# thowell/CALIPSO.jl

Hardware: AMD Instinct MI355X
Metric: Newton steps/sec (n~5k KKT) (higher is better)
Workload: dtype f64; 1 GPU; C3 synthetic dense conic QP: nx=2500 ne=1500 nc=1000 (400 R+ + 200 x SOC3), n=5000 condensed, N=8500 unreduced; ONE system per GPU stepped sequentially (replicas at N > 1); 1 LDL^T factorisation, 6 refinement round(s) per step; refinement_rounds=6

## Files before the change

calipso.jl_amd/__init__.py:

```python
import ctypes as C

import numpy as np

from ._lib import CALLBACK_FN, EVAL_FN, CalipsoHipError, lib

__all__ = ["Solver", "Group", "LDLSolver", "SmallBatch", "Comm", "ordering", "symbolic", "Options", "initialize_b", "solve_b", "CalipsoHipError", "FLAGS", "splitmix_uniform",
           "mfma_f64_peak"]

FLAGS = dict(
    objective=1 << 0, objective_gradient_variables=1 << 1, objective_jacobian_variables_variables=1 << 2,
    equality_constraint=1 << 3, equality_jacobian_variables=1 << 4, equality_dual_jacobian_variables=1 << 5,
    equality_dual_jacobian_variables_variables=1 << 6, cone_constraint=1 << 7, cone_jacobian_variables=1 << 8,
    cone_dual_jacobian_variables=1 << 9, cone_dual_jacobian_variables_variables=1 << 10,
    objective_jacobian_variables_parameters=1 << 11, equality_jacobian_parameters=1 << 12,
    equality_dual_jacobian_variables_parameters=1 << 13, cone_jacobian_parameters=1 << 14,
    cone_dual_jacobian_variables_parameters=1 << 15)
CONE_BARRIER, CONE_BARRIER_GRADIENT, CONE_PRODUCT, CONE_JACOBIAN, CONE_TARGET = 1, 2, 4, 8, 16

STATUS_TEXT = {-1: "inertia correction failure", -2: "cone search failure", -3: "evaluation callback failed",
               -4: "bad argument", -5: "HIP error", -6: "cone layout not supported"}


def _pd(a):
    return a.ctypes.data_as(C.POINTER(C.c_double))
# ... 373 lines not shown
    def set_callbacks(self, inner=None, outer=None):
        self._cbi = CALLBACK_FN(lambda u, h: inner(self)) if inner else None
        self._cbo = CALLBACK_FN(lambda u, h: outer(self)) if outer else None
        ci = C.cast(self._cbi, C.c_void_p) if self._cbi else None
        co = C.cast(self._cbo, C.c_void_p) if self._cbo else None
        self._check(self._L.calipso_hip_set_callbacks(self._h, ci, co, None), "set_callbacks")

    def stats(self):
        out = np.zeros(8, dtype=np.int64)
        self._L.calipso_hip_stats(self._h, _pi(out))
        return dict(total_iterations=int(out[0]), outer=int(out[1]), factorizations=int(out[2]), refinement_failures=int(out[3]),
                    max_refinement_rounds=int(out[4]), fallbacks=int(out[5]), last_refinement_rounds=int(out[6]), newton_steps=int(out[7]))

    def qp_attach(self, P, q, A, b, G, h, objective_scale=0.5):
        f = lambda M: np.ascontiguousarray(np.asarray(M, dtype=np.float64).T).reshape(-1)
        v = lambda a: np.ascontiguousarray(np.asarray(a, dtype=np.float64))
        Pc, Ac, Gc = f(P), f(A) if self.ne else np.zeros(1), f(G) if self.nc else np.zeros(1)
        qv, bv, hv = v(q), v(b) if self.ne else np.zeros(1), v(h) if self.nc else np.zeros(1)
        self._check(self._L.calipso_hip_qp_attach(self._h, _pd(Pc), _pd(qv), _pd(Ac), _pd(bv), _pd(Gc), _pd(hv), objective_scale), "qp_attach")

    def qp_evaluate(self, flags, which=0):
        self._check(self._L.calipso_hip_qp_evaluate(self._h, which, int(flags)), "qp_evaluate")

    def newton_step(self, advance=False):
        info = np.zeros(6)
        rc = self._check(self._L.calipso_hip_newton_step(self._h, int(advance), _pd(info)), "newton_step")
        return dict(status=rc, step_size=info[0], step_size_cone_slack_dual=info[1], refinement_rounds=int(info[2]),
                    factorizations=int(info[3]), merit_candidate=info[4], violation_candidate=info[5])

    def newton_steps(self, count, advance=False):
        info = np.zeros(6 * max(int(count), 1))
        status = np.zeros(max(int(count), 1), dtype=np.int32)
        self._check(self._L.calipso_hip_newton_steps(self._h, int(count), int(advance), _pd(info), status.ctypes.data_as(C.POINTER(C.c_int32))), "newton_steps")
        I = info.reshape(-1, 6)
        return [dict(status=int(status[k]), step_size=I[k, 0], step_size_cone_slack_dual=I[k, 1], refinement_rounds=int(I[k, 2]), factorizations=int(I[k, 3]),
                     merit_candidate=I[k, 4], violation_candidate=I[k, 5]) for k in range(int(count))]

    def phase_times(self):
        out = np.zeros(9)
        self._L.calipso_hip_phase_times(self._h, _pd(out))
        return out

    def kernel_times(self):
        out = np.zeros(8)
        self._L.calipso_hip_kernel_times(self._h, _pd(out))
        return out

    def structure_work(self):
        out = np.zeros(8)
        self._check(self._L.calipso_hip_structure_work(self._h, _pd(out)), "structure_work")
        return dict(schur_flops=out[0], packed_doubles=out[1], segment_pairs=int(out[2]), factor_flops=out[3], factor_nnz=out[4], order=int(out[5]), structured=bool(out[6]))

    def schedule_info(self):
        out = np.zeros(4)
        self._check(self._L.calipso_hip_schedule_info(self._h, _pd(out)), "schedule_info")
        return dict(prologue_ahead_steps=int(out[0]), last_prologue_mode=int(out[1]), ahead_undone=int(out[2]))

    def padded_nx(self):
        return int(self.kernel_times()[2])

    def device_bytes(self):
        return int(self.kernel_times()[3])

    def analyze_structure(self):
        out = np.zeros(4, dtype=np.int64)
        self._check(self._L.calipso_hip_analyze_structure(self._h, _pi(out)), "analyze_structure")
        return dict(half_bandwidth=int(out[0]), band_blocks=int(out[1]), equality_rows_per_group=int(out[2]), cone_rows_per_group=int(out[3]))

    def clear_structure(self):
        self._check(self._L.calipso_hip_clear_structure(self._h), "clear_structure")

    def set_stage_parallel(self, on=True, batch=1):
        out = np.zeros(4, dtype=np.int64)
        self._check(self._L.calipso_hip_set_stage_parallel(self._h, 1 if on else 0, int(batch), _pi(out)), "set_stage_parallel")
        return dict(levels=int(out[0]), largest_front=int(out[1]), nnz_upper=int(out[2]))

    def set_stage_blocks(self, on=True):
        out = np.zeros(4, dtype=np.int64)
        self._check(self._L.calipso_hip_set_stage_blocks(self._h, 1 if on else 0, _pi(out)), "set_stage_blocks")
        return dict(z_blocks=int(out[0]), hessian_blocks=int(out[1]), segments=int(out[2]), packed_doubles=int(out[3]))

    def synchronize(self):
        self._check(self._L.calipso_hip_synchronize(self._h), "synchronize")

    def streams_concurrent(self, other):
        out = np.zeros(6)
        self._check(self._L.calipso_hip_streams_concurrent(self._h, other._h, _pd(out)), "streams_concurrent")
        return bool(out[0]), float(out[1]), float(out[2]), float(out[3]), float(out[4]), float(out[5])

    def rebind_stream(self, priority_class=-1):
        self._check(self._L.calipso_hip_rebind_stream(self._h, int(priority_class)), "rebind_stream")


class Group:

    def __init__(self, solvers):
        import ctypes as C
        self.solvers = list(solvers)
        self._L = self.solvers[0]._L
        arr = (C.c_void_p * len(self.solvers))(*[s._h for s in self.solvers])
        h = C.c_void_p()
        rc = self._L.calipso_hip_group_create(arr, len(self.solvers), C.byref(h))
        if rc != 0:
            raise CalipsoHipError("group_create failed (%d): %s" % (rc, self._L.calipso_hip_last_error(self.solvers[0]._h).decode()))
        self._g = h

    def newton_step(self, advance=False):
        import ctypes as C
        B = len(self.solvers)
# ... 782 lines not shown
```

calipso.jl_amd/csrc/api.hip:

```cpp
#include <algorithm>
#include <array>
#include <atomic>
#include <cmath>
#include <mutex>
#include <cstdio>
#include <cstdlib>
#include <cstring>

#include "internal.hpp"
#include "device_utils.hpp"
#include "host_logic.hpp"

using namespace calipso;

namespace calipso {
int check(H* s, hipError_t e, const char* what) {
    char buf[512];
    snprintf(buf, sizeof buf, "%s: %s", what, hipGetErrorString(e));
    if (s) s->err = buf;
    return CALIPSO_ERR_HIP;
}
bool lds_attribute(const void* kernel, int bytes) {
    static std::mutex mu;
    static std::map<std::pair<const void*, int>, std::pair<int, int>> done;
// ... 560 lines not shown

}

__global__ __launch_bounds__(128) void k_publish_words(const unsigned* __restrict__ src, int words, unsigned* __restrict__ hdst, unsigned long long* __restrict__ hseq,
                                                        unsigned long long seq) {
    if ((int)threadIdx.x < words) hdst[threadIdx.x] = src[threadIdx.x];
    __threadfence_system();
    __syncthreads();
    if (threadIdx.x == 0) __hip_atomic_store(hseq, seq, __ATOMIC_RELEASE, __HIP_MEMORY_SCOPE_SYSTEM);
}
static int wait_published(H* s, unsigned long long seq);
static int publish_and_wait(H* s, const void* dsrc, void* hdst_dev, int words) {
    const unsigned long long seq = ++s->pub_seq;
    hipLaunchKernelGGL(k_publish_words, dim3(1), dim3(128), 0, s->stream, static_cast<const unsigned*>(dsrc), words, static_cast<unsigned*>(hdst_dev), s->hseq_dev, seq);
    return wait_published(s, seq);
}
static int wait_published(H* s, unsigned long long seq) {
    if (launch_errors(s, "a kernel launch of this phase was refused")) return CALIPSO_ERR_HIP;
    hipError_t q = hipSuccess;
    const bool ok = host_wait([&] { return __atomic_load_n(s->hseq, __ATOMIC_ACQUIRE) >= seq; },
                              [&] { q = hipStreamQuery(s->stream); return q == hipErrorNotReady; });
    if (ok) return 0;
    if (q != hipSuccess && q != hipErrorNotReady) return calipso::check(s, q, "publish_and_wait");
    s->err = "scalar read-back did not arrive";
    return CALIPSO_ERR_HIP;
}
static int wait_published_side(H* s, unsigned long long seq) {
    hipError_t q = hipSuccess;
    const bool ok = host_wait([&] { return __atomic_load_n(s->hseq + 1, __ATOMIC_ACQUIRE) >= seq; },
                              [&] { q = hipStreamQuery(s->stream2); return q == hipErrorNotReady; });
    if (ok) return 0;
    if (q != hipSuccess && q != hipErrorNotReady) return calipso::check(s, q, "wait_published_side");
    s->err = "scalar read-back of the second stream did not arrive";
    return CALIPSO_ERR_HIP;
}
static int read_scalars(H* s, int first, int count) { return publish_and_wait(s, s->dscal + first, s->hscal_dev + first, 2 * count); }
static int read_icount(H* s, int first, int count) { return publish_and_wait(s, s->icount + first, s->hicount_dev + first, count); }
static double* point_of(H* s, int which) { return which == 0 ? s->solution : s->candidate; }

static void factor_times(H* s) {
    if (!s->factor_times_pending) return;
    s->factor_times_pending = false;
    if (hipEventSynchronize(s->ev[13]) != hipSuccess) return;
    float ms = 0.f;
    (void)hipEventElapsedTime(&ms, s->ev[10], s->ev[11]); s->phase_ms[1] = ms;
    (void)hipEventElapsedTime(&ms, s->ev[11], s->ev[12]); s->phase_ms[7] = ms;
    (void)hipEventElapsedTime(&ms, s->ev[12], s->ev[13]); s->phase_ms[3] = ms;
    s->kernel_ms[0] = hipEventElapsedTime(&ms, s->ev[12], s->ev[14]) == hipSuccess ? ms : 0.0;
}

static int do_factorize(H* s, int64_t inertia[3], bool rhs_ahead_ok = false) {
    factor_times(s);
    (void)hipEventRecord(s->ev[10], s->stream);
    launch_cone_weights(s);
    s->rhs_ahead = false; s->rhs_joined = false;
    if (rhs_ahead_ok) {
        hipStream_t st2 = calipso::ldl_rhs_stream(s);
        if (st2 && s->side_work) s->rhs_ahead = true;
        else if (st2) {
            (void)hipEventRecord(s->ev_side[6], s->stream);
            (void)hipStreamWaitEvent(st2, s->ev_side[6], 0);
            hipStream_t keep = s->stream;
            s->stream = st2;
            launch_residual_symmetric(s, s->residual);
            if (s->d.m) calipso::gemv_t(s, s->d.m, s->d.nx, s->Z, s->d.m, s->t1, s->xbuf, 1.0, 1.0, calipso::SP_Z);
            s->stream = keep;
            s->rhs_ahead = true;
        }
    }
    launch_scale_rows(s);
    calipso::inject_refused_launch(s->stream);
    (void)hipEventRecord(s->ev[11], s->stream);
    launch_schur(s);
    (void)hipEventRecord(s->ev[12], s->stream);
    s->side_ran = false;
    launch_ldl(s);
    if (s->side_work && s->rhs_ahead && !s->side_ran) s->side_work(s);
    (void)hipEventRecord(s->ev[13], s->stream);
    s->factor_times_pending = true;
    if (s->ldl_failed) { s->ldl_failed = false; SYNC(); return CALIPSO_ERR_HIP; }
    if (s->ldl_pub_seq) {
        if (wait_published(s, s->ldl_pub_seq)) return CALIPSO_ERR_HIP;
    } else {
        if (launch_errors(s, "a kernel launch of the factorisation was refused")) return CALIPSO_ERR_HIP;
        CK(hipMemcpyAsync(s->hicount, s->icount, sizeof(int) * 6, hipMemcpyDeviceToHost, s->stream));
        SYNC();
        factor_times(s);
    }
    s->stats.factorizations += 1;
    s->phase_ms[8] += 1.0;
    const int64_t pos = s->hicount[0] + s->hicount[3], nonpos = s->hicount[1] + s->hicount[4], zero = s->hicount[2] + s->hicount[5];
    inertia[0] = pos; inertia[1] = nonpos; inertia[2] = zero;
    if (zero > 0) { inertia[0] = -1; return CALIPSO_WARN_ZERO_PIVOT; }
    return CALIPSO_OK;
}

static int do_inertia_correction(H* s, int64_t* nfact, bool rhs_ahead_ok = false, const int64_t* first_in = nullptr, int first_rc = 0) {
    const Options& o = s->opt; const Dims& d = s->d;
    int64_t in[3];
    ic_begin(o, s->sc);
    int rc;
    if (first_in) { in[0] = first_in[0]; in[1] = first_in[1]; in[2] = first_in[2]; rc = first_rc; }
    else rc = do_factorize(s, in, rhs_ahead_ok);
    for (int64_t count = 1;; ++count) {
        if (rc < 0) return rc;
        const IcVerdict v = ic_after(o, s->sc, in, d.nx, d.ne + d.nc, count == 1);
        if (v != IC_AGAIN) {
            if (nfact) *nfact = count;
            if (v == IC_DONE) return CALIPSO_OK;
            s->err = "inertia correction failure";
            return CALIPSO_ERR_INERTIA;
        }
        rc = do_factorize(s, in, rhs_ahead_ok);
    }
}

static void do_sds(H* s, int which, double* accumulate = nullptr, bool refine_follows = false, bool use_ahead = false) {
    const double* res = which == 0 ? s->residual : s->residual_error;
    double* st = which == 0 ? s->step : s->step_correction;
    if (which == 0 && s->rhs_ahead && !s->rhs_joined && s->stream2 && s->ev_side[7]) {
        (void)hipEventRecord(s->ev_side[7], s->stream2);
        (void)hipStreamWaitEvent(s->stream, s->ev_side[7], 0);
        s->rhs_joined = true;
    }
    const bool ready = use_ahead && which == 0 && s->rhs_ahead && s->rhs_joined;
    s->rhs_ahead = false;
    if (!ready) launch_residual_symmetric(s, res);
    const bool tail = which == 0 && !accumulate && s->d.m > 0;
    linear_solve_device(s, !tail, ready);
    if (tail && launch_solve_tail(s, 0, false, refine_follows)) return;
    if (tail) gemv_n(s, s->d.m, s->d.nx, s->Z, s->d.m, s->xbuf, s->t2, 1.0, 0.0, SP_Z);
    launch_recover(s, st, res, accumulate, which == 0 ? 1 : 0);
}

static void refine_residual(H* s, bool publish = false) {
    const Dims& d = s->d;
    launch_refine_local(s);
    const int nchunk = gemv_refine_pair(s, s->step + d.oy(), s->t1, s->w1, s->w2, s->step, s->lxv, true);
    if (nchunk > 0) launch_refine_x_fused(s, publish, nchunk); else launch_refine_x(s, publish);
}
static void refine_solve(H* s) {
    const Dims& d = s->d;
    launch_trsv(s, s->xbuf);
    if (d.m && launch_solve_tail(s, 1, true, true)) return;
    if (d.m) gemv_n(s, d.m, d.nx, s->Z, d.m, s->xbuf, s->t2, 1.0, 0.0, SP_Z);
    launch_recover(s, s->step_correction, s->residual_error, s->step, 2);
}

static bool spec_refinement_ok(H* s) {
    static const bool env = [] { const char* e = getenv("CALIPSO_HIP_SPEC_REFINE"); return !e || atoi(e) != 0; }();
    return env && !s->cur && s->gate && s->d.m > 0 && !s->compact && !s->blocks.on && !(s->stage_parallel && s->spS) && wform_on(s) && solve_tail_available(s) &&
           s->opt.max_iterative_refinement >= 1;
}
static int refinement_loop(H* s, double norm, double norm0, int it, int* rounds, double* final_norm, bool* ran_more);
static int do_refinement(H* s, int* rounds, double* final_norm, bool zsx_valid = false) {
    const Options& o = s->opt; const Dims& d = s->d;
    if (!zsx_valid && d.m) gemv_n(s, d.m, d.nx, s->Z, d.m, s->step, s->zsx, 1.0, 0.0, SP_Z);
    double norm, norm0;
    int it = 0;
    if (spec_refinement_ok(s)) {
        const int spec = (int)std::min<calipso::i64>(o.max_iterative_refinement, std::max<calipso::i64>(1, s->stats.last_refine > 0 ? s->stats.last_refine : o.min_iterative_refinement));
        if (++s->gate_counter == 0) s->gate_counter = 1;
        s->gate_epoch = s->gate_counter;
        for (int k = 0; k <= spec; ++k) {
            if (k > 0) {
                launch_trsv_direct(s, s->xbuf);
                (void)launch_solve_tail(s, 1, true, true);
            }
            launch_refine_local(s);
            const int nchunk = gemv_refine_pair(s, s->step + d.oy(), s->t1, s->w1, s->w2, s->step, s->lxv, true);
            launch_refine_x_fused(s, true, nchunk, k, k == spec);
        }
        s->gate_epoch = 0;
        if (s->refine_defer) { s->refine_pending = true; if (rounds) *rounds = -1; return CALIPSO_OK; }
        if (wait_published(s, s->pub_seq)) return CALIPSO_ERR_HIP;
        norm = s->hscal[7]; norm0 = s->hscal[20]; it = (int)s->hscal[21];
    } else {
        refine_residual(s, true);
        if (wait_published(s, s->pub_seq)) return CALIPSO_ERR_HIP;
        norm = s->hscal[7];
        norm0 = norm;
    }
// ... 648 lines not shown
    EV(8);
    int rc = inner_iteration(s, nullptr, nullptr, ev, cv, info, &ev, &cv, !last);
    EV(9);
    if (rc < 0) return rc;
    if (!advance) {
        copy_step_state(s, false);
        launch_cone(s, s->solution, CALIPSO_CONE_PRODUCT);
        s->filter_theta = ft; s->filter_merit = fm; s->filter_index = fi;
        restore_scalars_keeping_regularization(s->sc, saved_sc);
    }
    if (info_out) {
        info_out[0] = info.step_size; info_out[1] = info.step_size_t; info_out[2] = info.rounds; info_out[3] = (double)info.nfact;
        info_out[4] = info.Mh; info_out[5] = info.thetah;
    }
    if (!last) return rc;
    SYNC();
    float ms = 0.f;
    if (info.exit_kind == 0) {
        (void)hipEventElapsedTime(&ms, s->ev[0], s->ev[1]); s->phase_ms[0] = ms;
        (void)hipEventElapsedTime(&ms, s->ev[2], s->ev[3]); s->phase_ms[2] = ms;
        (void)hipEventElapsedTime(&ms, s->ev[3], s->ev[4]); s->phase_ms[5] = ms;
    }
    (void)hipEventElapsedTime(&ms, s->ev[8], s->ev[9]); s->phase_ms[6] = ms;
    return rc;
}

}

extern "C" {

int32_t calipso_hip_phase_times(H* s, double out[9]) {
    if (!s || !out) return CALIPSO_ERR_ARGUMENT;
    factor_times(s);
    for (int i = 0; i < 9; ++i) out[i] = s->phase_ms[i];
    return CALIPSO_OK;
}

int32_t calipso_hip_kernel_times(H* s, double out[8]) {
    if (!s || !out) return CALIPSO_ERR_ARGUMENT;
    for (int i = 0; i < 8; ++i) out[i] = 0.0;
    factor_times(s);
    out[0] = s->kernel_ms[0];
    out[1] = (double)s->ldl_step_launches;
    out[2] = (double)s->d.NP;
    out[3] = (double)(s->slab_doubles * sizeof(double) + s->scratch_bytes);
    { double lf[8]; calipso::lfac_describe(s, lf); out[6] = s->lfac_last ? 1.0 : (s->lfac_failed ? -1.0 : 0.0); out[7] = lf[5]; }
    if (s->matvec_timed && hipEventSynchronize(s->ev[6]) == hipSuccess) {
        float ms = 0.f;
        if (hipEventElapsedTime(&ms, s->ev[5], s->ev[6]) == hipSuccess) { out[4] = ms; out[5] = 8.0 * ((double)s->d.m * s->d.nx + (double)s->d.nx * s->d.nx); }
    }
    return CALIPSO_OK;
}

int32_t calipso_hip_schedule_info(H* s, double out[4]) {
    if (!s || !out) return CALIPSO_ERR_ARGUMENT;
    out[0] = (double)s->prologue_ahead_steps; out[1] = (double)s->last_prologue_mode; out[2] = (double)s->ahead_undone; out[3] = 0.0;
    return CALIPSO_OK;
}

int32_t calipso_hip_structure_work(H* s, double out[8]) {
    if (!s || !out) return CALIPSO_ERR_ARGUMENT;
    for (int i = 0; i < 8; ++i) out[i] = 0.0;
    if (s->blocks.on) { out[0] = s->blocks.schur_flops; out[1] = (double)s->blocks.packed; out[2] = (double)s->blocks.npairs; }
    if (s->stage_parallel && s->spS) { double w[3]; calipso::sparse_work(s->spS, w); out[3] = w[0]; out[4] = w[1]; out[5] = w[2]; }
    out[6] = s->compact ? 1.0 : 0.0;
    return CALIPSO_OK;
}

int32_t calipso_hip_splitmix_uniform(uint64_t problem_id, uint64_t stream_id, double lo, double hi, int64_t count, double* out) {
    if (!out && count > 0) return CALIPSO_ERR_ARGUMENT;
    uint64_t state = 0xCA11B50000000000ULL + 4096ULL * problem_id + stream_id;
    for (int64_t i = 0; i < count; ++i) {
        state += 0x9E3779B97F4A7C15ULL;
        uint64_t z = state;
        z = (z ^ (z >> 30)) * 0xBF58476D1CE4E5B9ULL;
        z = (z ^ (z >> 27)) * 0x94D049BB133111EBULL;
        z = z ^ (z >> 31);
        out[i] = lo + (hi - lo) * ((double)(z >> 11) * (1.0 / 9007199254740992.0));
    }
    return CALIPSO_OK;
}

}
```

calipso.jl_amd/csrc/device_utils.hpp:

```cpp
#pragma once
#include <hip/hip_runtime.h>

#include "../../include/calipso_wave.hpp"

namespace calipso {

template <typename... P> __device__ __forceinline__ void inst_shift(const Batch& b, P&... p) {
    const long long o = b.delta[blockIdx.z];
    ((p += o), ...);
}
template <typename... P> __device__ __forceinline__ void inst_shift_i(const Batch& b, P&... p) {
    const long long o = 2 * b.delta[blockIdx.z];
    ((p += o), ...);
}

__device__ __forceinline__ size_t column_shift(const Batch& b, size_t per_member) { return (size_t)b.slot[blockIdx.z] * per_member; }

__device__ __forceinline__ double from_lane63(double v) {
    return __hiloint2double(__builtin_amdgcn_readlane(__double2hiint(v), 63), __builtin_amdgcn_readlane(__double2loint(v), 63));
}
__device__ __forceinline__ double wave_sum(double v) { return from_lane63(wave_sum_l63(v)); }
__device__ __forceinline__ double wave_max(double v) { return from_lane63(wave_max_l63(v)); }
__device__ __forceinline__ int wave_sum_i(int v) {
#pragma unroll
    for (int off = 32; off > 0; off >>= 1) v += __shfl_down(v, off, 64);
    return v;
}

__device__ __forceinline__ double block_sum(double v, double* sm) {
    const int lane = threadIdx.x & 63, w = threadIdx.x >> 6, nw = (blockDim.x + 63) >> 6;
    v = wave_sum(v);
    __syncthreads();
    if (lane == 0) sm[w] = v;
    __syncthreads();
    double r = 0.0;
    if (threadIdx.x == 0) for (int i = 0; i < nw; ++i) r += sm[i];
    return r;
}
__device__ __forceinline__ double block_max(double v, double* sm) {
    const int lane = threadIdx.x & 63, w = threadIdx.x >> 6, nw = (blockDim.x + 63) >> 6;
    v = wave_max(v);
    __syncthreads();
    if (lane == 0) sm[w] = v;
    __syncthreads();
    double r = 0.0;
    if (threadIdx.x == 0) for (int i = 0; i < nw; ++i) r = fmax(r, sm[i]);
    return r;
}

__device__ __forceinline__ void arrow_inverse(int n, const double* u, const double* x, double* out) {
    double uu = 0.0;
    for (int i = 1; i < n; ++i) uu += u[i] * u[i];
    const double alpha = -1.0 / (u[0] * u[0]) * uu;
    const double beta = 1.0 / (1.0 + alpha);
    double d0 = 0.0;
    for (int i = 1; i < n; ++i) d0 += (u[i] / u[0]) * x[i];
    const double x0_1 = x[0] - d0;
    double d1 = 0.0;
    for (int i = 1; i < n; ++i) {
        const double v = x[i] - beta * ((u[i] / u[0]) * x0_1);
        out[i] = v;
        d1 += (u[i] / u[0]) * v;
    }
    const double x2_1 = x[0] - d1;
    out[0] = 1.0 / u[0] * x2_1;
    for (int i = 1; i < n; ++i) out[i] = 1.0 / u[0] * out[i];
}


template <int MAXD>
__device__ __forceinline__ void arrow_inverse_small(int n, const double (&u)[MAXD], const double (&x)[MAXD], double (&out)[MAXD]) {
    double uu = 0.0;
#pragma unroll
    for (int i = 1; i < MAXD; ++i) if (i < n) uu += u[i] * u[i];
    const double alpha = -1.0 / (u[0] * u[0]) * uu;
    const double beta = 1.0 / (1.0 + alpha);
    double d0 = 0.0;
#pragma unroll
    for (int i = 1; i < MAXD; ++i) if (i < n) d0 += (u[i] / u[0]) * x[i];
    const double x0_1 = x[0] - d0;
    double d1 = 0.0;
#pragma unroll
    for (int i = 1; i < MAXD; ++i) if (i < n) {
        const double v = x[i] - beta * ((u[i] / u[0]) * x0_1);
        out[i] = v;
        d1 += (u[i] / u[0]) * v;
    }
    const double x2_1 = x[0] - d1;
    out[0] = 1.0 / u[0] * x2_1;
#pragma unroll
    for (int i = 1; i < MAXD; ++i) if (i < n) out[i] = 1.0 / u[0] * out[i];
}

template <int MAXD>
__device__ __forceinline__ void arrow_inverse_t_small(int n, const double (&u)[MAXD], const double (&y)[MAXD], double (&out)[MAXD]) {
    double uu = 0.0;
#pragma unroll
    for (int i = 1; i < MAXD; ++i) if (i < n) uu += u[i] * u[i];
    const double alpha = -1.0 / (u[0] * u[0]) * uu;
    const double beta = 1.0 / (1.0 + alpha);
// ... 16 lines not shown
```

calipso.jl_amd/csrc/gemv.hip:

```cpp
#include "internal.hpp"
#include "device_utils.hpp"

namespace calipso {

struct BlockRanges { int b0, b1, b2, b3; };
__device__ __forceinline__ BlockRanges column_blocks(const Sparsity& sp, int col, int rows) {
    BlockRanges r = {0, (rows + 63) / 64, 0, 0};
    if (sp.kind == SP_DENSE) return r;
    if (sp.kind == SP_LXX) { r.b0 = max(0, col - sp.hb) / 64; r.b1 = (min(rows, col + sp.hb + 1) + 63) / 64; return r; }
    const int* k = sp.kr + 4 * (col / 16);
    const int elo = k[0], ehi = k[1], clo = k[2], chi = k[3];
    if (sp.kind == SP_GX) { r.b0 = elo / 64; r.b1 = ehi > elo ? (ehi + 63) / 64 : r.b0; return r; }
    if (sp.kind == SP_HX) { r.b0 = clo / 64; r.b1 = chi > clo ? (chi + 63) / 64 : r.b0; return r; }
    r.b0 = elo / 64; r.b1 = ehi > elo ? (ehi + 63) / 64 : r.b0;
    r.b2 = (sp.ne + clo) / 64; r.b3 = chi > clo ? (sp.ne + chi + 63) / 64 : r.b2;
    return r;
}
__device__ __forceinline__ bool block_active(const BlockRanges& r, int b) { return (b >= r.b0 && b < r.b1) || (b >= r.b2 && b < r.b3); }

template <int NV>
__device__ __forceinline__ void structured_column(const BlockRanges& br, int rows, int lane, const double* __restrict__ a, const double* const (&x)[NV],
                                                  double (&acc0)[NV], double (&acc1)[NV]) {
#pragma unroll
    for (int pass = 0; pass < 2; ++pass) {
        const int lo = pass ? max(br.b2, br.b1) : br.b0, hi = pass ? br.b3 : br.b1;
        for (int w0 = lo; w0 < hi; w0 += 16) {
            double v[16];
#pragma unroll
            for (int q = 0; q < 16; ++q) { const int b = w0 + q, i = b * 64 + lane; v[q] = (b < hi && i < rows) ? a[i] : 0.0; }
#pragma unroll
            for (int q = 0; q < 16; ++q) {
                const int b = w0 + q, i = b * 64 + lane;
                const bool in = b < hi && i < rows;
                const bool odd = ((b % 24) & 1) != 0;
#pragma unroll
                for (int n = 0; n < NV; ++n) {
                    const double xv = in ? x[n][i] : 0.0;
                    acc0[n] = odd ? acc0[n] : fma(v[q], xv, acc0[n]);
                    acc1[n] = odd ? fma(v[q], xv, acc1[n]) : acc1[n];
                }
            }
        }
    }
}

__global__ __launch_bounds__(256) void k_gemv_t(Batch bt, Sparsity sp, int rows, int cols, const double* __restrict__ A, int ld, const double* __restrict__ x,
                                                 double* __restrict__ y, double alpha, double beta, const double* __restrict__ add = nullptr) {
    inst_shift(bt, A, x, y);
    if (add) inst_shift(bt, add);
    if (sp.kr) inst_shift_i(bt, sp.kr);
    const int lane = threadIdx.x & 63;
    const int col = blockIdx.x * 4 + (threadIdx.x >> 6);
    if (col >= cols) return;
    const double* a = A + (size_t)col * ld;
    const BlockRanges br = column_blocks(sp, col, rows);
    double acc0 = 0.0, acc1 = 0.0;
    if (sp.kind != SP_DENSE) {
        const double* const xs[1] = {x};
        double a0[1] = {0.0}, a1[1] = {0.0};
        structured_column<1>(br, rows, lane, a, xs, a0, a1);
        acc0 = a0[0]; acc1 = a1[0];
    } else
    for (int base = 0; base < rows; base += 64 * 24) {
        if (sp.kind != SP_DENSE && !(base / 64 < max(br.b1, br.b3) && base / 64 + 24 > min(br.b0, br.b2 < br.b3 ? br.b2 : br.b0))) continue;
        double v[24];
#pragma unroll
        for (int q = 0; q < 24; ++q) { const int i = base + lane + 64 * q; v[q] = (i < rows && block_active(br, base / 64 + q)) ? a[i] : 0.0; }
#pragma unroll
        for (int q = 0; q < 24; q += 2) {
            const int i = base + lane + 64 * q;
            acc0 = fma(v[q], i < rows ? x[i] : 0.0, acc0);
            acc1 = fma(v[q + 1], i + 64 < rows ? x[i + 64] : 0.0, acc1);
        }
    }
    const double r = wave_sum(acc0 + acc1);
    if (lane == 0) y[col] = add ? alpha * r + add[col] : ((beta == 0.0) ? alpha * r : alpha * r + beta * y[col]);
}

__device__ __forceinline__ void gemv_t2_body(Batch bt, Sparsity sp, int bx, int rows, int cols, const double* __restrict__ A, int ld, const double* __restrict__ x1,
                                             const double* __restrict__ x2, double* __restrict__ y1, double* __restrict__ y2) {
    inst_shift(bt, A, x1, x2, y1, y2);
    if (sp.kr) inst_shift_i(bt, sp.kr);
    const int lane = threadIdx.x & 63;
    const int col = bx * 4 + (threadIdx.x >> 6);
    if (col >= cols) return;
    const double* a = A + (size_t)col * ld;
    const BlockRanges br = column_blocks(sp, col, rows);
    double p0 = 0.0, p1 = 0.0, q0 = 0.0, q1 = 0.0;
    if (sp.kind != SP_DENSE) {
        const double* const xs[2] = {x1, x2};
        double a0[2] = {0.0, 0.0}, a1[2] = {0.0, 0.0};
        structured_column<2>(br, rows, lane, a, xs, a0, a1);
        p0 = a0[0]; p1 = a1[0]; q0 = a0[1]; q1 = a1[1];
    } else
    for (int base = 0; base < rows; base += 64 * 24) {
        if (sp.kind != SP_DENSE && !(base / 64 < max(br.b1, br.b3) && base / 64 + 24 > min(br.b0, br.b2 < br.b3 ? br.b2 : br.b0))) continue;
        double v[24];
#pragma unroll
        for (int q = 0; q < 24; ++q) { const int i = base + lane + 64 * q; v[q] = (i < rows && block_active(br, base / 64 + q)) ? a[i] : 0.0; }
#pragma unroll
        for (int q = 0; q < 24; q += 2) {
            const int i = base + lane + 64 * q;
            const bool in0 = i < rows, in1 = i + 64 < rows;
            p0 = fma(v[q], in0 ? x1[i] : 0.0, p0); p1 = fma(v[q + 1], in1 ? x1[i + 64] : 0.0, p1);
            q0 = fma(v[q], in0 ? x2[i] : 0.0, q0); q1 = fma(v[q + 1], in1 ? x2[i + 64] : 0.0, q1);
        }
    }
    const double r1 = wave_sum(p0 + p1), r2 = wave_sum(q0 + q1);
    if (lane == 0) { y1[col] = r1; y2[col] = r2; }
}
__device__ __forceinline__ void gemv_t2_dense_lds(Batch bt, int bx, int rows, int cols, const double* __restrict__ A, int ld, const double* __restrict__ x1,
                                                  const double* __restrict__ x2, double* __restrict__ y1, double* __restrict__ y2, double* __restrict__ xs) {
    inst_shift(bt, A, x1, x2, y1, y2);
    const int lane = threadIdx.x & 63;
    const int col = bx * 4 + (threadIdx.x >> 6);
    const bool valid = col < cols;
    const double* a = A + (size_t)(valid ? col : 0) * ld;
    double v[24];
#pragma unroll
    for (int q = 0; q < 24; ++q) { const int i = lane + 64 * q; v[q] = (valid && i < rows) ? a[i] : 0.0; }
    for (int i = threadIdx.x; i < rows; i += 256) { xs[i] = x1[i]; xs[rows + i] = x2[i]; }
    __syncthreads();
    if (!valid) return;
    double p0 = 0.0, p1 = 0.0, q0 = 0.0, q1 = 0.0;
    for (int base = 0; base < rows; base += 64 * 24) {
        if (base) {
#pragma unroll
            for (int q = 0; q < 24; ++q) { const int i = base + lane + 64 * q; v[q] = i < rows ? a[i] : 0.0; }
        }
// ... 52 lines not shown
    const int i = bx * GN_ROWS + threadIdx.x;
    const int c0 = by * chunk;
    const int c1 = min(cols, c0 + chunk);
    const bool xb = c1 - c0 <= 64;
    const int ln = threadIdx.x & 63;
    double xr = (xb && c0 + ln < c1) ? x[c0 + ln] : 0.0;
    asm volatile("" : "+v"(xr));
    const bool inrow = i < rows;
    int jlo = 0, jhi = cols;
    if (inrow) {
        if (sp.kind == SP_LXX) { jlo = i - sp.hb; jhi = i + sp.hb + 1; }
        else if (sp.kind != SP_DENSE) { jlo = sp.rowrange[2 * (row_off + i)]; jhi = sp.rowrange[2 * (row_off + i) + 1]; }
    } else { jlo = 0; jhi = 0; }
    const bool any = inrow && !(sp.kind != SP_DENSE && (c1 <= jlo || c0 >= jhi));
    double acc0 = 0.0, acc1 = 0.0;
    auto xat = [&](int j) -> double {
        if (!xb) return x[j];
        const int l = j - c0;
        return __hiloint2double(__builtin_amdgcn_readlane(__double2hiint(xr), l), __builtin_amdgcn_readlane(__double2loint(xr), l));
    };
    for (int j0 = c0; j0 < c1; j0 += 24) {
        const bool batch_in = any && (sp.kind == SP_DENSE || !(j0 + 24 <= jlo || j0 >= jhi));
        double v[24];
#pragma unroll
        for (int q = 0; q < 24; ++q) { const int j = j0 + q; v[q] = (batch_in && j < c1 && j >= jlo && j < jhi) ? A[i + (size_t)j * ld] : 0.0; }
#pragma unroll
        for (int q = 0; q < 24; q += 2) {
            const double x0 = j0 + q < c1 ? xat(j0 + q) : 0.0, x1 = j0 + q + 1 < c1 ? xat(j0 + q + 1) : 0.0;
            if (batch_in) { acc0 += v[q] * x0; acc1 += v[q + 1] * x1; }
        }
    }
    if (inrow) partial[(size_t)by * rows + i] = acc0 + acc1;
}
__global__ __launch_bounds__(GN_ROWS) void k_gemv_n_partial(Batch bt, Sparsity sp, int row_off, int rows, int cols, int chunk, const double* __restrict__ A, int ld,
                                                             const double* __restrict__ x, double* __restrict__ partial) {
    gemv_n_partial_body(bt, sp, blockIdx.x, blockIdx.y, row_off, rows, cols, chunk, A, ld, x, partial);
}
__global__ __launch_bounds__(256) void k_gemv_t2_and_n(Batch bt, Sparsity spz, int rowsz, int colsz, const double* __restrict__ Z, int ldz, const double* __restrict__ x1,
                                                        const double* __restrict__ x2, double* __restrict__ y1, double* __restrict__ y2, int nt2, Sparsity spl, int rb,
                                                        int rowsl, int colsl, int chunk, const double* __restrict__ L, int ldl, const double* __restrict__ xl,
                                                        double* __restrict__ partial, const int* __restrict__ gate = nullptr, int gate_epoch = 0, int lds_x = 0) {
    static_assert(GN_ROWS == 256, "one block size for both bodies");
    if (gate && gate[0] == gate_epoch) return;
    extern __shared__ __attribute__((aligned(16))) double t2_lds[];
    const int b = blockIdx.x;
    if (b < nt2 && lds_x && spz.kind == SP_DENSE) {
        gemv_t2_dense_lds(bt, b, rowsz, colsz, Z, ldz, x1, x2, y1, y2, t2_lds);
        return;
    }
    if (b < nt2) gemv_t2_body(bt, spz, b, rowsz, colsz, Z, ldz, x1, x2, y1, y2);
    else gemv_n_partial_body(bt, spl, (b - nt2) % rb, (b - nt2) / rb, 0, rowsl, colsl, chunk, L, ldl, xl, partial);
}

__global__ __launch_bounds__(256) void k_gemv_n_reduce(Batch bt, int rows, int nchunk, const double* __restrict__ partial, double* __restrict__ y, double alpha, double beta,
                                                       const double* __restrict__ add = nullptr) {
    __shared__ double part[4][64];
    inst_shift(bt, partial, y);
    if (add) inst_shift(bt, add);
    const int r = threadIdx.x & 63, p = threadIdx.x >> 6;
    const int i = blockIdx.x * 64 + r;
    double acc = 0.0;
    if (i < rows) {
        static_assert(GN_MAXCHUNK <= 64, "16 partials per thread");
        for (int c0 = p; c0 < nchunk; c0 += 64) {
            double v[16];
#pragma unroll
            for (int u = 0; u < 16; ++u) { const int c = c0 + 4 * u; v[u] = c < nchunk ? partial[(size_t)c * rows + i] : 0.0; }
#pragma unroll
            for (int u = 0; u < 16; ++u) if (c0 + 4 * u < nchunk) acc += v[u];
        }
    }
    part[p][r] = acc;
    __syncthreads();
    if (threadIdx.x < 64 && i < rows) {
        const double v = (part[0][r] + part[1][r]) + (part[2][r] + part[3][r]);
        y[i] = add ? alpha * v + add[i] : ((beta == 0.0) ? alpha * v : alpha * v + beta * y[i]);
    }
}

constexpr int BOTH_RQ = 16;
constexpr int BOTH_CW = 16;
__global__ __launch_bounds__(256) void k_gemv_both(Batch bt, Sparsity sp, int rows, int cols, int cw, const double* __restrict__ A, int ld, const double* __restrict__ x,
                                                    const double* __restrict__ u, double* __restrict__ part_n, double* __restrict__ part_t) {
    inst_shift(bt, A, x, u, part_n, part_t);
    if (sp.kr) inst_shift_i(bt, sp.kr);
    const int lane = threadIdx.x & 63;
    const int cg = blockIdx.x * 4 + (threadIdx.x >> 6);
    const int c0 = cg * cw;
    if (c0 >= cols) return;
    const int r0 = blockIdx.y * 64 * BOTH_RQ;
    double uu[BOTH_RQ], acc[BOTH_RQ];
#pragma unroll
    for (int q = 0; q < BOTH_RQ; ++q) { const int i = r0 + lane + 64 * q; uu[q] = i < rows ? u[i] : 0.0; acc[q] = 0.0; }
    const int c1 = min(cols, c0 + cw);
    const BlockRanges br = column_blocks(sp, c0, rows);
    unsigned active = 0;
#pragma unroll
    for (int q = 0; q < BOTH_RQ; ++q) if (block_active(br, r0 / 64 + q)) active |= 1u << q;
    for (int j = c0; j < c1; ++j) {
        const double* a = A + (size_t)j * ld;
        double z[BOTH_RQ];
#pragma unroll
        for (int q = 0; q < BOTH_RQ; ++q) { const int i = r0 + lane + 64 * q; z[q] = (i < rows && ((active >> q) & 1u)) ? a[i] : 0.0; }
        const double xj = x[j];
        double t0 = 0.0, t1 = 0.0;
#pragma unroll
        for (int q = 0; q < BOTH_RQ; q += 2) {
            t0 += z[q] * uu[q]; t1 += z[q + 1] * uu[q + 1];
            acc[q] += z[q] * xj; acc[q + 1] += z[q + 1] * xj;
        }
        const double t = wave_sum(t0 + t1);
        if (lane == 0) part_t[(size_t)blockIdx.y * cols + j] = t;
    }
#pragma unroll
    for (int q = 0; q < BOTH_RQ; ++q) { const int i = r0 + lane + 64 * q; if (i < rows) part_n[(size_t)cg * rows + i] = acc[q]; }
}

void gemv_both(calipso_hip_solver* s, int rows, int cols, const double* A, int ld, const double* x, const double* u, double* yn, double* yt, double beta_t, int kind) {
    if (rows == 0 || cols == 0) return;
    if (s->compact) { s->err = "internal: a dense mat-vec was requested on a structured handle"; s->ldl_failed = true; return; }
    const BatchSc B = batch_of(s);
    const int cw = BOTH_CW;
    const int ncg = (cols + cw - 1) / cw, nrr = (rows + 64 * BOTH_RQ - 1) / (64 * BOTH_RQ);
    double* part_n = s->gemv_partial;
    double* part_t = s->gemv_partial + (size_t)ncg * rows;
    hipLaunchKernelGGL(k_gemv_both, dim3((ncg + 3) / 4, nrr, B.b.n), dim3(256), 0, s->stream, B.b, sparsity_of(s, kind), rows, cols, cw, A, ld, x, u, part_n, part_t);
    hipLaunchKernelGGL(k_gemv_n_reduce, dim3((rows + 63) / 64, 1, B.b.n), dim3(256), 0, s->stream, B.b, rows, ncg, part_n, yn, 1.0, 0.0);
    hipLaunchKernelGGL(k_gemv_n_reduce, dim3((cols + 63) / 64, 1, B.b.n), dim3(256), 0, s->stream, B.b, cols, nrr, part_t, yt, 1.0, beta_t);
}

static void gemv_n_chunks(int rows, int cols, int& rb, int& nchunk, int& chunk) {
    rb = (rows + GN_ROWS - 1) / GN_ROWS;
    nchunk = (768 + rb - 1) / rb;
    if (nchunk > GN_MAXCHUNK) nchunk = GN_MAXCHUNK;
    if (nchunk > (cols + 15) / 16) nchunk = (cols + 15) / 16;
    if (nchunk < 1) nchunk = 1;
    chunk = (cols + nchunk - 1) / nchunk;
    nchunk = (cols + chunk - 1) / chunk;
    if (cols == 0) nchunk = 0;
}

int gemv_refine_pair(calipso_hip_solver* s, const double* x1, const double* x2, double* y1, double* y2, const double* xl, double* yl, bool defer_reduce) {
    const Dims& d = s->d;
    if (d.m == 0 || s->blocks.on || s->compact) {
        if (d.m) gemv_t2(s, d.m, d.nx, s->Z, d.m, x1, x2, y1, y2, SP_Z);
        gemv_n(s, d.nx, d.nx, s->Lxx, d.nx, xl, yl, 1.0, 0.0, SP_LXX);
        return 0;
    }
    int rb, nchunk, chunk;
    gemv_n_chunks(d.nx, d.nx, rb, nchunk, chunk);
    const int nt2 = (d.nx + 3) / 4;
    const BatchSc B = batch_of(s);
    const bool timed = s->time_matvec && !s->cur;
    if (timed) (void)hipEventRecord(s->ev[5], s->stream);
    const size_t xbytes = 2 * sizeof(double) * (size_t)d.m;
    const int lds_x = gemv_lds_x(xbytes);
    hipLaunchKernelGGL(k_gemv_t2_and_n, dim3(nt2 + rb * nchunk, 1, B.b.n), dim3(256), lds_x ? xbytes : 0, s->stream, B.b, sparsity_of(s, SP_Z), d.m, d.nx, s->Z, d.m, x1, x2, y1, y2, nt2,
                       sparsity_of(s, SP_LXX), rb, d.nx, d.nx, chunk, s->Lxx, d.nx, xl, s->gemv_partial, s->gate_epoch ? s->gate : (const int*)nullptr, s->gate_epoch, lds_x);
    if (timed) { (void)hipEventRecord(s->ev[6], s->stream); s->time_matvec = false; s->matvec_timed = true; }
    if (defer_reduce) return nchunk;
    hipLaunchKernelGGL(k_gemv_n_reduce, dim3((d.nx + 63) / 64, 1, B.b.n), dim3(256), 0, s->stream, B.b, d.nx, nchunk, s->gemv_partial, yl, 1.0, 0.0);
    return 0;
}

void gemv_n(calipso_hip_solver* s, int rows, int cols, const double* A, int ld, const double* x, double* y, double alpha, double beta, int kind, const double* add) {
    if (rows == 0) return;
    if (blocks_gemv_n(s, kind, x, y, alpha, beta)) { if (add) launch_add(s, y, add, rows); return; }
    if (s->compact) { s->err = "internal: a dense mat-vec was requested on a structured handle"; s->ldl_failed = true; return; }
    int rb, nchunk, chunk;
    gemv_n_chunks(rows, cols, rb, nchunk, chunk);
    const BatchSc B = batch_of(s);
    if (nchunk > 0)
        hipLaunchKernelGGL(k_gemv_n_partial, dim3(rb, nchunk, B.b.n), dim3(GN_ROWS), 0, s->stream, B.b, sparsity_of(s, kind), kind == SP_HX ? s->d.ne : 0, rows, cols, chunk, A, ld,
                           x, s->gemv_partial);
    hipLaunchKernelGGL(k_gemv_n_reduce, dim3((rows + 63) / 64, 1, B.b.n), dim3(256), 0, s->stream, B.b, rows, nchunk, s->gemv_partial, y, alpha, beta, add);
}

}
```

calipso.jl_amd/csrc/internal.hpp:

```cpp
#pragma once
#include <hip/hip_runtime.h>
#include <stdint.h>

#include <map>
#include <string>
#include <vector>

#include "../../include/calipso_hip.h"
#include "../../include/calipso_options.hpp"
#include "step_decisions.hpp"
#include "sensitivity_columns.hpp"

namespace calipso {

constexpr int TILE = 128;
constexpr int NB = 64;
constexpr int MAX_SOC_DIM = 1024;
constexpr int TRSV_BLOCK = 2048;
inline int trsv_block(int NP, int limit = TRSV_BLOCK) {
    if (NP <= 512) return NP;
    int tb = 512;
    while (2 * tb <= limit && 2 * tb <= NP) tb *= 2;
    for (;; tb /= 2) { const int rem = NP % tb; if (tb == 512 || (rem & (rem - 1)) == 0) return tb; }
}
inline size_t tinv_doubles(int NP) {
    size_t most = 0;
    for (int limit : {512, 1024, 2048}) { const size_t tb = (size_t)trsv_block(NP, limit); const size_t n = ((size_t)NP + tb - 1) / tb * tb * tb; most = n > most ? n : most; }
    return most;
}
inline bool wform_layout_ok(int NP, int tb) { return NP > tb && NP <= 4096; }
inline size_t wform_offset(int NP, int tb, int kb) {
    size_t off = 0;
    for (int b = 0; b < kb; ++b) { const int k0 = b * tb, w = tb < NP - k0 ? tb : NP - k0; off += (size_t)(NP - k0 - w) * (size_t)w; }
    return off;
}
constexpr int MAX_BATCH = 128;
struct Batch {
    int n = 1;
    long long delta[MAX_BATCH] = {0};
    int slot[MAX_BATCH] = {0};
};
struct BatchSc {
    Batch b;
    const Scalars* sctab = nullptr;
    Scalars sc1;
    __host__ __device__ const Scalars& scal(int z) const { return sctab ? sctab[z] : sc1; }
};

enum { SP_DENSE = 0, SP_Z = 1 , SP_GX = 2 , SP_HX = 3 , SP_LXX = 4  };
struct Sparsity {
    int kind = SP_DENSE;
    int hb = 0;
    int ne = 0;
    const int* kr = nullptr;
    const int* rowrange = nullptr;
};

struct Dims {
    int nx, np, ne, nc, n, N, m;
    int q;
    int n_soc;
    int max_dim;
    int n_wide;
    int NP;
    __host__ __device__ int orr() const { return nx; }
    __host__ __device__ int os() const { return nx + ne; }
    __host__ __device__ int oy() const { return nx + ne + nc; }
    __host__ __device__ int oz() const { return nx + ne + nc + ne; }
    __host__ __device__ int ot() const { return nx + ne + nc + ne + nc; }
};

struct ConeDev {
    int* soc_start = nullptr;
    int* soc_dim = nullptr;
    int* soc_woff = nullptr;
    int* entry_soc = nullptr;
    int* wide = nullptr;
};

struct ZBlock { int row0, nrows, col0, ncols; long long off_c, off_r; };
struct LBlock { int c0, n; long long off_c, off_r; };
struct Segment { int c0, nc, first, count; };
struct SegPair { int a, b, first, count, lblock; long long soff; };
struct StageBlocks {
    bool on = false;
    int nblk = 0, nlb = 0, nseg = 0, npairs = 0, max_lb = 0;
    size_t packed = 0;
    unsigned long long signature = 0;
    ZBlock* d_blk = nullptr; LBlock* d_lblk = nullptr; Segment* d_seg = nullptr; int* d_segblk = nullptr; SegPair* d_pairs = nullptr; int* d_pairblk = nullptr;
    int* d_colrange = nullptr;
    std::vector<calipso_device_block> h_jdesc, h_hdesc;
    calipso_device_block *d_jdesc = nullptr, *d_hdesc = nullptr;
    int* d_rowcov = nullptr;
    double schur_flops = 0.0;
    std::vector<ZBlock> h_blk; std::vector<LBlock> h_lblk; std::vector<SegPair> h_pairs; std::vector<Segment> h_seg; std::vector<int> h_seg_of_col;
};
struct BlockPlan {
    std::vector<ZBlock> zb; std::vector<LBlock> lb; std::vector<Segment> seg; std::vector<int> segblk, pairblk, colrange, seg_of_col; std::vector<SegPair> pairs;
    size_t packed = 0, spacked = 0; int max_lb = 0; unsigned long long signature = 0;
};

struct QpEval {
    bool attached = false;
    double scale = 0.5;
    double *q = nullptr, *bh = nullptr;
};

struct ColumnWorkspace {
    double* d = nullptr; size_t doubles = 0;
    int* active = nullptr; size_t ints = 0;
    std::vector<double> norms;
    SensitivityColumns cols;
    double info[4] = {0, 0, 0, 0};
};

struct Stats {
    i64 total_iterations = 0, outer = 0, factorizations = 0, refine_fail = 0, refine_max = 0, fallbacks = 0, last_refine = 0, newton_steps = 0;
};

}

struct calipso_hip_solver {
    calipso::Dims d;
    calipso::Options opt;
    calipso::Scalars sc;
    calipso::ConeDev cone;
    calipso::QpEval qp;
    calipso::Stats stats;
    struct calipso_hip_group* owner = nullptr;
    const calipso::BatchSc* cur = nullptr;
    double* slab = nullptr; size_t slab_doubles = 0;
    int device = 0;
    hipStream_t stream = nullptr;
    std::string err;
    calipso_callback_fn cb_inner = nullptr, cb_outer = nullptr;
    void* cb_user = nullptr;
    calipso_device_eval_fn dev_eval = nullptr;
    void* dev_eval_user = nullptr;
    calipso_device_block_eval_fn dev_block_eval = nullptr;
    void* dev_block_eval_user = nullptr;
    size_t scratch_bytes = 0;
    int last_prologue_mode = 0;
    bool prologue_pending = false, side_ran = false;
    int prologue_rc = 0;
    void (*side_work)(calipso_hip_solver*) = nullptr;
    unsigned long long pub_seq2 = 0;
    long long prologue_ahead_steps = 0;
    long long ahead_undone = 0;
    bool rhs_ahead = false, rhs_joined = false;
    double *evalL = nullptr, *evalZ = nullptr;
    std::map<std::string, double*> optd;
    std::vector<int> h_soc_start, h_soc_dim, h_soc_woff;
    std::vector<int64_t> h_nonneg, h_soc_ptr, h_soc_idx;
    double* Lxx = nullptr;
    double* Z = nullptr;
    double *gx = nullptr, *hx = nullptr;
    double* Lsym = nullptr;
    bool hessian_dirty = true;
    double *fx = nullptr, *gyx = nullptr, *hzx = nullptr;
    double* gh = nullptr;
    double *g = nullptr, *hc = nullptr;
    double *cone_product = nullptr, *cone_target = nullptr, *barrier_gradient = nullptr;
    double* dscal = nullptr;
    double* hscal = nullptr;
    double* hscal_dev = nullptr;
    unsigned long long* hseq = nullptr;
    unsigned long long* hseq_dev = nullptr;
    unsigned long long pub_seq = 0;
    double *jacobian_parameters = nullptr, *solution_sensitivity = nullptr;
    double *solution = nullptr, *candidate = nullptr, *lambda = nullptr, *parameters = nullptr;
    double *residual = nullptr, *residual_error = nullptr, *step = nullptr, *step_correction = nullptr, *saved_point = nullptr;
    double *residual_symmetric = nullptr, *step_symmetric = nullptr, *merit_gradient = nullptr;
    bool pad_done = false;
    double* Kdense = nullptr;
    double* S = nullptr;
    double* Dx = nullptr;
    double* refpart = nullptr;
    int refparts = 0;
    int* zgrp = nullptr; int n_zgrp = 0;
    int* gate = nullptr; int gate_epoch = 0; int gate_counter = 0;
    bool refine_defer = false, refine_pending = false;
    bool spec_ahead_ok = false;
    bool refine_local_done = false;
    double* Ypanel = nullptr;
    double* Tinv = nullptr;
    double* Ttmp = nullptr;
    double* zf2 = nullptr;
    double* Wfac = nullptr;
    double* WH = nullptr;
    double* wz = nullptr;
    double* kzz = nullptr;
    double* Wsoc = nullptr;
    double* Bsoc = nullptr;
    double* socwork = nullptr;
    int schur_nj = 8;
    int half_bandwidth = 0, band64 = 0;
    std::vector<int> h_reach;
    std::vector<int> h_zrow, h_lreach;
    calipso::StageBlocks blocks;
    bool blocks_effective = true;
    size_t blocks_zero_cell = 0;
    bool compact = false;
    calipso_hip_sparse* spS = nullptr;
    long long* spS_src = nullptr;
    bool spS_values_current = false;
    int* spS_inv = nullptr;
    int* d_reach = nullptr;
    bool stage_parallel = false;
    calipso::i64 structure_resets = 0;
    int* krange = nullptr;
    int* zrow = nullptr;
    int* icount = nullptr;
    int* hicount = nullptr;
    int* hicount_dev = nullptr;
    double* gemv_partial = nullptr;
    double* vtmp = nullptr;
    double *xbuf = nullptr, *zf = nullptr, *t1 = nullptr, *t2 = nullptr;
    double *zsx = nullptr;
    double *w1 = nullptr, *w2 = nullptr, *lxv = nullptr;
    double *saved_g = nullptr, *saved_h = nullptr;
    double *lgp = nullptr, *gp = nullptr, *hp = nullptr;
    std::vector<double> hparams;
    calipso::ColumnWorkspace fwd, rev;
    bool group_columns = false;
    int group_tile = 0;
// ... 26 lines not shown
    bool graph_ldl_tried = false, graph_ldl_fin_tried = false, graph_trsv_tried = false, use_graphs = true;
    calipso::i64 solve_block = 1024;
    calipso::i64 solve_wform = 1;
    bool time_matvec = false, matvec_timed = false;
    double kernel_ms[4] = {0};
    double phase_ms[9] = {0};
    std::vector<double> filter_theta, filter_merit, cache_theta, cache_merit;
    calipso::i64 filter_index = 0;
    std::vector<double> hpoint, hstage;
};

namespace calipso {

void launch_cone(calipso_hip_solver* s, const double* point, int flags);
void launch_cone_search(calipso_hip_solver* s, unsigned long long publish_seq = 0);
void launch_cone_candidate(calipso_hip_solver* s, double a_s, double a_t);
void launch_cone_candidate_batch(calipso_hip_solver* s, const double* a_s, const double* a_t);
void launch_cone_violation_host(calipso_hip_solver* s, const double* xhat_dev, const double* x_dev, double tau);
void launch_residual(calipso_hip_solver* s);
void launch_violations(calipso_hip_solver* s, int pub_first = 0, int pub_count = 0);
void launch_residual_symmetric(calipso_hip_solver* s, const double* res);
void launch_recover(calipso_hip_solver* s, double* step, const double* res, double* accumulate, int zsx_mode = 0);
void launch_refine_local(calipso_hip_solver* s);
bool launch_solve_tail(calipso_hip_solver* s, int which, bool accumulate, bool with_refine);
bool solve_tail_available(const calipso_hip_solver* s);
void solve_tail_plan(const Dims& d, const std::vector<int>& soc_start, const std::vector<int>& soc_dim, std::vector<int>& grp);
void launch_refine_x(calipso_hip_solver* s, bool publish = false);
void launch_refine_x_fused(calipso_hip_solver* s, bool publish, int nchunk, int it = -1, bool last_queued = false);
void launch_trsv_direct(calipso_hip_solver* s, double* x);
void launch_axpy_points(calipso_hip_solver* s, double step_size, int with_s);
void launch_accept(calipso_hip_solver* s, double step_size);
void launch_axpy_points_batch(calipso_hip_solver* s, const double* step_size, int with_s);
void launch_accept_batch(calipso_hip_solver* s, const double* step_size);
void launch_merit(calipso_hip_solver* s, const double* point);
void launch_merit_gradient(calipso_hip_solver* s);
void launch_merit_and_gradient(calipso_hip_solver* s);
void launch_first_candidate(calipso_hip_solver* s, double a_s, double a_t);
void launch_first_candidate_batch(calipso_hip_solver* s, const double* a_s, const double* a_t);
void launch_first_candidate_from_masks(calipso_hip_solver* s);
void launch_constraint_violation(calipso_hip_solver* s, const double* point, int pub_first = 0, int pub_count = 0);
void launch_merit_and_constraint(calipso_hip_solver* s, const double* point, int pub_first, int pub_count);
void launch_violations_and_constraint(calipso_hip_solver* s, int pub_first = 0, int pub_count = 0, bool side = false);
void launch_dot_merit(calipso_hip_solver* s);
void launch_Hmul(calipso_hip_solver* s, const double* v, double* out);
void launch_residual_error(calipso_hip_solver* s, const double* step);
void launch_add(calipso_hip_solver* s, double* y, const double* x, int len);
void launch_assemble_K(calipso_hip_solver* s);
void gemv_n(calipso_hip_solver* s, int rows, int cols, const double* A, int ld, const double* x, double* y, double alpha, double beta, int kind = SP_DENSE,
            const double* add = nullptr);
void gemv_t(calipso_hip_solver* s, int rows, int cols, const double* A, int ld, const double* x, double* y, double alpha, double beta, int kind = SP_DENSE,
            const double* add = nullptr);
void gemv_t2(calipso_hip_solver* s, int rows, int cols, const double* A, int ld, const double* x1, const double* x2, double* y1, double* y2, int kind = SP_DENSE);
int gemv_refine_pair(calipso_hip_solver* s, const double* x1, const double* x2, double* y1, double* y2, const double* xl, double* yl, bool defer_reduce = false);
void gemv_both(calipso_hip_solver* s, int rows, int cols, const double* A, int ld, const double* x, const double* u, double* yn, double* yt, double beta_t,
               int kind = SP_DENSE);
void launch_cone_weights(calipso_hip_solver* s);
void launch_cone_weights_wide(calipso_hip_solver* s);
void launch_residual_symmetric_wide(calipso_hip_solver* s, const double* res, int p, double* rsym, double* t1, bool regions);
void launch_recover_wide(calipso_hip_solver* s, const double* res, int p, const double* rsym, const double* t2, double* dsym, double* step, double* accumulate, int zsx_mode, bool regions);
void launch_refine_local_wide(calipso_hip_solver* s, int part0);
void launch_scale_rows(calipso_hip_solver* s);
void launch_schur(calipso_hip_solver* s);
void launch_symmetrize(calipso_hip_solver* s);
void schur_plan(calipso_hip_solver* s);
void launch_pad_identity(calipso_hip_solver* s);
void blocks_release(calipso_hip_solver* s);
void blocks_pack(calipso_hip_solver* s, bool z, bool l);
int blocks_pack_from(calipso_hip_solver* s, const double* L, const double* Z, bool l, bool zg, bool zh);
int blocks_descriptors(calipso_hip_solver* s);
void blocks_mirror(calipso_hip_solver* s, bool l, bool zg, bool zh);
bool blocks_gemv_n(calipso_hip_solver* s, int kind, const double* x, double* y, double alpha, double beta);
bool blocks_gemv_t(calipso_hip_solver* s, int kind, const double* u1, const double* u2, double* y1, double* y2, double alpha, double beta);
bool blocks_schur(calipso_hip_solver* s);
bool blocks_gemm_l(calipso_hip_solver* s, const double* X, long long ldx, double* Y, long long ldy, int p, bool transposed = false);
bool blocks_gemm_n(calipso_hip_solver* s, const double* X, long long ldx, double* Y, long long ldy, int p);
bool blocks_gemm_t(calipso_hip_solver* s, const double* U, long long ldu, double* Y, long long ldy, int p, double beta);
bool blocks_plan(const Dims& d, const std::vector<int>& zrow, const std::vector<int>& lreach, BlockPlan& P, std::string& err);
int blocks_install(calipso_hip_solver* s, const BlockPlan& P);
int blocks_unpack_dense(calipso_hip_solver* s, double** Lxx, double** Z);
int blocks_upload_dense(calipso_hip_solver* s, int which, const double* data, double scale);
int blocks_download_dense(calipso_hip_solver* s, int which, double* data);
bool blocks_entry_offsets(const calipso_hip_solver* s, int which, int row, int col, long long* off_c, long long* off_r);
void launch_ldl(calipso_hip_solver* s);
void ldl_drop_graphs(calipso_hip_solver* s);
void launch_trsv(calipso_hip_solver* s, double* x);
bool lastblock_sym_on(const calipso_hip_solver* s);
bool wform_on(const calipso_hip_solver* s);
bool lfac_on(const calipso_hip_solver* s);
bool lfac_ready(calipso_hip_solver* s);
int lfac_enqueue(calipso_hip_solver* s, unsigned long long* hprog, unsigned long long epoch);
double* lfac_factor_buffer(calipso_hip_solver* s);
void lfac_release(calipso_hip_solver* s);
void lfac_describe(calipso_hip_solver* s, double out[8]);
void launch_copy_pad(calipso_hip_solver* s, const double* src, int n, double* dst, int npad);
void launch_init_point(calipso_hip_solver* s);
void launch_lambda_update(calipso_hip_solver* s);
void launch_jacobian_parameters(calipso_hip_solver* s);
void launch_negate_copy(calipso_hip_solver* s, const double* src, double* dst, int n);
void linear_solve_device(calipso_hip_solver* s, bool with_t2 = true, bool rhs_ready = false);
hipStream_t ldl_rhs_stream(calipso_hip_solver* s);
void launch_solve_from_b(calipso_hip_solver* s);
void gemm(calipso_hip_solver* s, int M, int N, int K, double alpha, const double* A, int lda, bool transA, const double* B, int ldb, double beta,
          double* C, int ldc);
void gemm_columns(calipso_hip_solver* s, int M, int N, int K, double alpha, const double* A, int lda, bool transA, const double* B, int ldb, double beta,
                  double* C, int ldc);
void trsm_multi(calipso_hip_solver* s, double* X, int p, double* U, double* Zm);
void launch_residual_symmetric_multi(calipso_hip_solver* s, const double* res, int p, double* rsym, double* xbuf, double* t1);
void launch_recover_multi(calipso_hip_solver* s, const double* res, int p, const double* rsym, const double* xbuf, const double* t2, double* dsym, double* step, double scale);
int refine_multi_parts(const calipso_hip_solver* s);
void launch_refine_rows_multi(calipso_hip_solver* s, const double* X, const double* R, const double* zx, int p, double* E, double* part, bool transposed = false);
void launch_refine_x_multi(calipso_hip_solver* s, const double* X, const double* R, const double* hx, long long ldh, int p, double* E, const double* part, double* norms);
void launch_accumulate_masked(calipso_hip_solver* s, const int* active, const double* C, int p, double* X, double* Xsave);
void launch_restore_masked(calipso_hip_solver* s, const int* restore, const double* Xsave, int p, double* X);
void launch_scale_into(calipso_hip_solver* s, const double* x, double* y, size_t n, double a);
int differentiate_columns(calipso_hip_solver* s);
int differentiate_columns_group(calipso_hip_solver* s, ColumnWorkspace& ws, int count, int tile);
int differentiate_columns_t(calipso_hip_solver* s, int p, const double* cotangent, bool with_theta, const double** lam, const double** grad_theta);
int differentiate_columns_t_group(calipso_hip_solver* s, ColumnWorkspace& ws, int count, int p, const double* cotangent, bool with_theta, const double** lam, const double** grad_theta);
int reserve_device(calipso_hip_solver* s, void** buf, size_t* have, size_t want, size_t elem, size_t uncounted, const char* caller, const char* what);
void launch_recover_t_multi(calipso_hip_solver* s, const double* V, int p, double* lam, double* g, double* xbuf);
void launch_residual_symmetric_t_multi(calipso_hip_solver* s, int p, const double* g, const double* xbuf, const double* t1, double* lam);
void launch_recover_t_wide(calipso_hip_solver* s, const double* V, int p, double* lam, double* g);
void launch_residual_symmetric_t_wide(calipso_hip_solver* s, int p, const double* g, const double* t1, double* lam);
void launch_qp_data_gradients(calipso_hip_solver* s, const double* lam, int p, double* const out[6], double scale);
int nonsymmetric_solve(calipso_hip_solver* s, const double* res, double* step);
void nonsymmetric_release(calipso_hip_solver* s);
void group_member_destroyed(struct calipso_hip_group* g, calipso_hip_solver* s);
void scatter_release(calipso_hip_solver* s);
void ldlsolver_release(calipso_hip_solver* s);
int structure_validate(calipso_hip_solver* s, int which);
bool csc_pattern_ok(i64 n, const i64* colptr, const i64* rowval);
inline bool structure_active(const calipso_hip_solver* s) { return s->band64 > 0 || s->stage_parallel || s->blocks.on; }
constexpr uint32_t PARAMETER_JACOBIANS = CALIPSO_EVAL_OBJECTIVE_JACOBIAN_PARAMETERS | CALIPSO_EVAL_EQUALITY_JACOBIAN_PARAMETERS | CALIPSO_EVAL_EQUALITY_DUAL_JACOBIAN_PARAMETERS |
                                         CALIPSO_EVAL_CONE_JACOBIAN_PARAMETERS | CALIPSO_EVAL_CONE_DUAL_JACOBIAN_PARAMETERS;
void launch_qp_evaluate(calipso_hip_solver* s, const double* point, uint32_t flags);

int check(calipso_hip_solver* s, hipError_t e, const char* what);
void inject_refused_launch(hipStream_t stream);
bool lds_attribute(const void* kernel, int bytes);
int evaluate_point(calipso_hip_solver* s, calipso_eval_fn eval, void* user, int which, uint32_t flags);
inline BatchSc batch_of(const calipso_hip_solver* s) {
    if (s->cur) return *s->cur;
    BatchSc b;
    b.b.n = 1; b.b.delta[0] = 0; b.sctab = nullptr; b.sc1 = s->sc;
    return b;
}
bool sparse_is_multifrontal(const calipso_hip_sparse* sp);
void sparse_borrow_stream(calipso_hip_sparse* sp, hipStream_t st);
int sparse_batch(const calipso_hip_sparse* sp);
int sparse_factor_from_dense(calipso_hip_sparse* sp, hipStream_t st, const Batch& bt, const double* S, const long long* src, int* icount, bool values_in_place = false);
void sparse_values(calipso_hip_sparse* sp, double** values, long long* stride);
int sparse_solve_inplace(calipso_hip_sparse* sp, hipStream_t st, const Batch& bt, double* x);
// ... 18 lines not shown
```

calipso.jl_amd/csrc/ldl.hip:

```cpp
#include "internal.hpp"
#define LDL_TRACE_OWNER
#include "ldl_device.hpp"
#include "host_logic.hpp"

#include <algorithm>
#include <array>
#include <chrono>
#include <mutex>

namespace calipso {


__global__ __launch_bounds__(DIAG_THREADS) void k_ldl_diag(Batch bt, int NP, int nx, int k0, int tb, double* __restrict__ S, double* __restrict__ Dx,
                                                            double* __restrict__ Tinv, double* __restrict__ Minv, int* __restrict__ icount) {
    __shared__ double smem[DIAG_LDS_DOUBLES];
    inst_shift(bt, S, Dx, Tinv, Minv);
    inst_shift_i(bt, icount);
    const int lane = threadIdx.x & 63, w = threadIdx.x >> 6, R = w >> 2, C = w & 3, fr = lane & 15, fk = lane >> 4;
    v4d acc = (v4d){0.0, 0.0, 0.0, 0.0};
    if (R >= C) {
#pragma unroll
        for (int q = 0; q < 4; ++q) acc[q] = S[(k0 + 16 * R + fr) + (size_t)(k0 + 16 * C + fk + 4 * q) * NP];
    }
    diag_block(smem, acc, NP, nx, k0, tb, S, Dx, Tinv, Minv, icount);
// ... 388 lines not shown
}
static bool side_stream(calipso_hip_solver* s) {
    if (s->stream2) return s->hprog_dev != nullptr && s->ev_side[7] != nullptr;
    int least = 0, greatest = 0;
    if (hipDeviceGetStreamPriorityRange(&least, &greatest) != hipSuccess) return false;
    hipStream_t st = nullptr;
    if (hipStreamCreateWithPriority(&st, hipStreamNonBlocking, least) != hipSuccess) return false;
    bool ok = true;
    if (!s->hprog) {
        if (hipHostMalloc((void**)&s->hprog, 4 * sizeof(unsigned long long), hipHostMallocMapped) != hipSuccess) { s->hprog = nullptr; ok = false; }
        else {
            s->hprog[0] = 0; s->hprog[1] = 0;
            if (hipHostGetDevicePointer((void**)&s->hprog_dev, s->hprog, 0) != hipSuccess) { s->hprog_dev = nullptr; ok = false; }
        }
    }
    for (auto& e : s->ev_side)
        if (ok && !e && hipEventCreateWithFlags(&e, hipEventDisableTiming) != hipSuccess) { e = nullptr; ok = false; }
    if (!ok) { (void)hipStreamDestroy(st); return false; }
    s->stream2 = st;
    return true;
}
static void enqueue_finish_feed(calipso_hip_solver* s, hipStream_t stream, int f);
static void enqueue_wform(calipso_hip_solver* s, hipStream_t stream, int kb);
static void enqueue_feed(calipso_hip_solver* s, hipStream_t stream, int i, bool beside);
static int wform_rows(const calipso_hip_solver* s, int rb);
static void enqueue_lastblock_sym(calipso_hip_solver* s, hipStream_t stream);
static void ldl_plan_ranges(calipso_hip_solver* s);
static bool ldl_overlap(calipso_hip_solver* s) {
    static const int env = [] { const char* e = getenv("CALIPSO_HIP_LDL_OVERLAP"); return e ? atoi(e) : 1; }();
    if (!env || graph_ldl_requested() || s->cur || s->band64 > 0) return false;
    const int NP = s->d.NP, tb = trsv_block(NP, (int)s->solve_block);
    if (NP < 1024 || NP > 8192 || tb < 256) return false;
    return true;
}

static void enqueue_ldl_steps(calipso_hip_solver* s) {
    const int NP = s->d.NP, nblk = NP / NB, tb = trsv_block(NP, (int)s->solve_block);
    const Batch bt = batch_of(s).b;
    const unsigned nz = bt.n;
    double* Minv = s->Ypanel;
    const bool lfac = lfac_ready(s);
    if (!lfac) hipLaunchKernelGGL(k_ldl_diag, dim3(1, 1, nz), dim3(DIAG_THREADS), 0, s->stream, bt, NP, s->d.nx, 0, tb, s->S, s->Dx, s->Tinv, Minv, s->icount);
    const int band = s->band64 > 0 ? s->band64 : nblk;
    const int resident = std::max(2, 248 / (int)nz);
    const bool pairs = s->band64 == 0 && nz >= 4;
    auto grid = [&](int tiles) { const int workers = std::min(std::max(tiles - 1, 0), resident) * (int)nz; return dim3(nz + (workers ? (workers + 7) / 8 * 8 + 7 : 0)); };
    const bool overlap = ldl_overlap(s) && side_stream(s);
    s->ldl_overlap_on = overlap;
    if (overlap) ldl_plan_ranges(s);
    int launches = 1;
    unsigned long long* const hprog = overlap ? s->hprog_dev : (unsigned long long*)nullptr;
    const unsigned long long epoch = s->ldl_epoch << 16;
    s->lfac_last = lfac;
    if (lfac) launches = lfac_enqueue(s, hprog, epoch);
    for (int kb = 0; !lfac && kb + 1 < nblk;) {
        const int k0 = kb * NB;
        const int rows = std::min(NP - k0 - NB, band * NB);
        const int ntr = rows / TT;
        if (pairs && kb + 2 < nblk) {
            hipLaunchKernelGGL((k_ldl_step<1>), grid(ntr), dim3(TR_THREADS), 0, s->stream, bt, NP, s->d.nx, k0, ntr, tb, s->S, Minv, s->Dx,
                               s->Tinv, s->icount, hprog, epoch | (unsigned long long)kb);
            const int ntr2 = ntr - 1, ntiles2 = ntr2 * (ntr2 + 1) / 2;
            hipLaunchKernelGGL((k_ldl_step<2>), grid(ntiles2), dim3(TR_THREADS), 0, s->stream, bt, NP, s->d.nx, k0, ntiles2, tb, s->S, Minv,
                               s->Dx, s->Tinv, s->icount);
            kb += 2; launches += 2;
        } else {
            const int ntiles = ntr * (ntr + 1) / 2;
            hipLaunchKernelGGL((k_ldl_step<0>), grid(ntiles), dim3(TR_THREADS), 0, s->stream, bt, NP, s->d.nx, k0, ntiles, tb, s->S, Minv, s->Dx, s->Tinv, s->icount,
                               hprog, epoch | (unsigned long long)kb);
            kb += 1; launches += 1;
        }
    }
    s->ldl_step_launches = launches;
    int forks = 0;
    if (overlap) while (3 * forks < (int)s->ldl_feeds.size() && s->ldl_feeds[3 * forks] <= nblk - 2) ++forks;
    s->ldl_forks = forks;
    if (s->ldl_publish && nz == 1) {
        s->ldl_pub_seq = ++s->pub_seq;
        hipLaunchKernelGGL(k_publish_inertia, dim3(1), dim3(64), 0, s->stream, s->icount, s->hicount_dev, s->hseq_dev, s->ldl_pub_seq);
    }
}

static void enqueue_ldl_finish(calipso_hip_solver* s) {
    const int NP = s->d.NP, nblk = NP / NB, tb = trsv_block(NP, (int)s->solve_block);
    const Batch bt = batch_of(s).b;
    const unsigned nz = bt.n;
    const int band = s->band64 > 0 ? s->band64 : nblk;
    {
        if (s->ldl_overlap_on) {
            if (s->ldl_forks || s->rhs_ahead) {
                (void)hipEventRecord(s->ev_side[7], s->stream2);
                (void)hipStreamWaitEvent(s->stream, s->ev_side[7], 0);
                s->rhs_joined = true;
            }
            for (int f = s->ldl_forks; 3 * f < (int)s->ldl_feeds.size(); ++f) enqueue_feed(s, s->stream, f, false);
            enqueue_lastblock_sym(s, s->stream);
            return;
        }
    }
    if (nblk > 1) {
        const int maxrows = std::min(NP - NB, band * NB);
        hipLaunchKernelGGL(k_ldl_scale, dim3(maxrows / 64, nblk - 1, nz), dim3(1024), 0, s->stream, bt, NP, tb, band * NB, 0, s->S, s->Lf, s->Dx, s->Tinv);
    }
    for (int level = 1; level <= 5; ++level) {
        const int half = 32 << level, tiles = half / 64, pairs = NP / (2 * half);
        if (2 * half > tb) break;
        for (int phase = 0; phase < 2; ++phase)
            hipLaunchKernelGGL(k_tinv_merge32, dim3(pairs * tiles * tiles * 4, 1, nz), dim3(256), 0, s->stream, bt, NP, tb, half, phase, 0, s->Lf, s->Tinv, s->Ttmp);
    }
    if (wform_on(s)) for (int kb = 0; kb * tb < NP; ++kb) enqueue_wform(s, s->stream, kb);
    enqueue_lastblock_sym(s, s->stream);
}

constexpr int FEED = 256;
static size_t merge_scratch(int NP, int half) { return (size_t)NP * (size_t)(half - 64) / 2; }
static void enqueue_merge(calipso_hip_solver* s, hipStream_t stream, int half, int phase, int pair0, int pairs) {
    const int NP = s->d.NP, tb = trsv_block(NP, (int)s->solve_block), tiles = half / 32;
    const Batch bt = batch_of(s).b;
    hipLaunchKernelGGL(k_tinv_merge32, dim3(pairs * tiles * tiles, 1, bt.n), dim3(256), 0, stream, bt, NP, tb, half, phase, pair0, s->Lf, s->Tinv, s->Ttmp + merge_scratch(NP, half));
}
constexpr int WFORM_WGS = 128;
static void ldl_plan_ranges(calipso_hip_solver* s) {
    const int NP = s->d.NP, nblk = NP / NB, tb = trsv_block(NP, (int)s->solve_block);
    s->ldl_ranges.clear();
    s->ldl_feeds.clear();
    const bool wf = wform_on(s);
    std::vector<std::array<int, 3>> feeds;
    for (int b0 = 0; b0 < NP; b0 += tb) {
        const int wblk = std::min(tb, NP - b0), wr = std::min(FEED, wblk);
        for (int c = b0; c < b0 + wblk; c += wr) {
            feeds.push_back({(c + wr) / NB, 0, (int)s->ldl_ranges.size() / 2});
            s->ldl_ranges.push_back(c); s->ldl_ranges.push_back(wr);
        }
// ... 251 lines not shown
    const int tid = threadIdx.x, r = tid % ROWS, p = tid / ROWS;
    const int row = blockIdx.x * ROWS + r;
    const double* M = Msym + row;
    double acc = 0.0;
    for (int c0 = 0; c0 < w; c0 += W) {
        double v[CPT];
#pragma unroll
        for (int q = 0; q < CPT; ++q) { const int c = c0 + p + PARTS * q; v[q] = (c < w) ? M[(size_t)c * w] : 0.0; }
        if (c0) __syncthreads();
        for (int i = tid; i < W; i += ROWS * PARTS) bs[i] = c0 + i < w ? in[k0 + c0 + i] : 0.0;
        __syncthreads();
#pragma unroll
        for (int q = 0; q < CPT; ++q) acc += v[q] * bs[p + PARTS * q];
    }
    part[p][r] = acc;
    __syncthreads();
    if (tid < ROWS) {
        double s = 0.0;
#pragma unroll
        for (int q = 0; q < PARTS; ++q) s += part[q][tid];
        x[k0 + blockIdx.x * ROWS + tid] = s;
    }
}

bool wform_on(const calipso_hip_solver* s) {
    const int NP = s->d.NP, tb = trsv_block(NP, (int)s->solve_block);
    return s->solve_wform != 0 && !s->compact && !(s->stage_parallel && s->spS) && wform_layout_ok(NP, tb);
}
static const int LASTSYM = [] { const char* e = getenv("CALIPSO_HIP_LASTBLOCK_SYM"); return e ? atoi(e) : 1; }();
bool lastblock_sym_on(const calipso_hip_solver* s) {
    if (!LASTSYM || !wform_on(s)) return false;
    const int NP = s->d.NP, tb = trsv_block(NP, (int)s->solve_block), nb = (NP + tb - 1) / tb;
    return nb >= 2;
}
static void enqueue_lastblock_sym(calipso_hip_solver* s, hipStream_t stream) {
    if (!lastblock_sym_on(s)) return;
    const int NP = s->d.NP, tb = trsv_block(NP, (int)s->solve_block), nb = (NP + tb - 1) / tb;
    const int k0 = (nb - 1) * tb, w = NP - k0;
    const Batch bt = batch_of(s).b;
    hipLaunchKernelGGL(k_lastblock_sym, dim3((w / 32) * (w / 32), 1, bt.n), dim3(256), 0, stream, bt, tb, nb - 1, w, s->Tinv, s->Dx, s->Wfac + wform_offset(NP, tb, nb - 1));
}
static int wform_rows(const calipso_hip_solver* s, int rb) {
    if (s->band64 <= 0) return rb;
    return std::min(rb, ((s->half_bandwidth + 63) / 64) * 64);
}
static void enqueue_wform(calipso_hip_solver* s, hipStream_t stream, int kb) {
    const int NP = s->d.NP, tb = trsv_block(NP, (int)s->solve_block);
    const int k0 = kb * tb, w = std::min(tb, NP - k0), rb = NP - k0 - w;
    if (rb <= 0) return;
    const Batch bt = batch_of(s).b;
    const int rows = wform_rows(s, rb);
    hipLaunchKernelGGL(k_wform_product, dim3((rows / 32) * (w / 32), 1, bt.n), dim3(256), 0, stream, bt, NP, tb, kb, w, rb, rows, s->Lf, s->Tinv, s->Wfac + wform_offset(NP, tb, kb));
}
static void enqueue_trsv_wform(calipso_hip_solver* s, double* x) {
    const int NP = s->d.NP, tb = trsv_block(NP, (int)s->solve_block), nb = (NP + tb - 1) / tb;
    double* u = s->zf;
    double* z = s->zf2;
    const Batch bt = batch_of(s).b;
    const unsigned nz = bt.n;
    const int* gate = s->gate_epoch ? s->gate : (const int*)nullptr;
    const int ge = s->gate_epoch;
    const bool sym = lastblock_sym_on(s);
    for (int kb = 0; kb < nb - (sym ? 1 : 0); ++kb) {
        const int k0 = kb * tb, w = std::min(tb, NP - k0), rb = NP - k0 - w;
        const double* Wb = s->Wfac + wform_offset(NP, tb, kb);
        const int rows = wform_rows(s, rb);
        const int snap = (sym && kb == nb - 2) ? 1 + rows : 0;
        const int grows = snap ? rb : rows;
        if (w > 512) hipLaunchKernelGGL((k_trsv_fwd<16, 32, 32>), dim3((w + grows) / 16, 1, nz), dim3(512), 0, s->stream, bt, kb, tb, w, rb, s->Tinv, Wb, x, s->Dx, u, z, gate, ge, snap);
        else hipLaunchKernelGGL((k_trsv_fwd<16, 16, 32>), dim3((w + grows) / 16, 1, nz), dim3(256), 0, s->stream, bt, kb, tb, w, rb, s->Tinv, Wb, x, s->Dx, u, z, gate, ge, snap);
    }
    if (sym) {
        const int k0 = (nb - 1) * tb, w = NP - k0;
        const double* Msym = s->Wfac + wform_offset(NP, tb, nb - 1);
        if (w > 512) hipLaunchKernelGGL((k_block_sym<16, 32, 32>), dim3(w / 16, 1, nz), dim3(512), 0, s->stream, bt, k0, w, Msym, u, x, gate, ge);
        else hipLaunchKernelGGL((k_block_sym<16, 16, 32>), dim3(w / 16, 1, nz), dim3(256), 0, s->stream, bt, k0, w, Msym, u, x, gate, ge);
    }
    for (int kb = nb - 1 - (sym ? 1 : 0); kb >= 0; --kb) {
        const int k0 = kb * tb, w = std::min(tb, NP - k0), rb = NP - k0 - w;
        const double* Wb = s->Wfac + wform_offset(NP, tb, kb);
        const int rows = wform_rows(s, rb), nch = (w + rows + 63) / 64;
        if (nch <= 8) launch_trsv_bwd<8>(s->stream, nz, bt, kb, tb, w, rb, rows, s->Tinv, Wb, z, x, gate, ge);
        else if (nch <= 16) launch_trsv_bwd<16>(s->stream, nz, bt, kb, tb, w, rb, rows, s->Tinv, Wb, z, x, gate, ge);
        else if (nch <= 24) launch_trsv_bwd<24>(s->stream, nz, bt, kb, tb, w, rb, rows, s->Tinv, Wb, z, x, gate, ge);
        else if (nch <= 32) launch_trsv_bwd<32>(s->stream, nz, bt, kb, tb, w, rb, rows, s->Tinv, Wb, z, x, gate, ge);
        else if (nch <= 40) launch_trsv_bwd<40>(s->stream, nz, bt, kb, tb, w, rb, rows, s->Tinv, Wb, z, x, gate, ge);
        else if (nch <= 48) launch_trsv_bwd<48>(s->stream, nz, bt, kb, tb, w, rb, rows, s->Tinv, Wb, z, x, gate, ge);
        else launch_trsv_bwd<64>(s->stream, nz, bt, kb, tb, w, rb, rows, s->Tinv, Wb, z, x, gate, ge);
    }
}

static void enqueue_trsv(calipso_hip_solver* s, double* x) {
    if (wform_on(s)) { enqueue_trsv_wform(s, x); return; }
    const int NP = s->d.NP, tb = trsv_block(NP, (int)s->solve_block), nb = (NP + tb - 1) / tb;
    double* u = s->zf;
    double* z = s->zf2;
    const Batch bt = batch_of(s).b;
    const unsigned nz = bt.n;
    for (int kb = 0; kb < nb; ++kb) {
        const int k0 = kb * tb, w = std::min(tb, NP - k0);
        int rest = NP - (k0 + w);
        if (s->band64 > 0) rest = std::min(rest, ((s->half_bandwidth + 31) / 32) * 32);
        if (w > 512) {
            hipLaunchKernelGGL((k_trsv_block_n<16, 32, 32>), dim3(w / 16, 1, nz), dim3(512), 0, s->stream, bt, kb, tb, w, s->Tinv, x, s->Dx, u, z);
            if (rest > 0) hipLaunchKernelGGL((k_trsv_update_n<16, 32, 32>), dim3(rest / 16, 1, nz), dim3(512), 0, s->stream, bt, NP, k0, w, s->Lf, u, x);
        } else {
            hipLaunchKernelGGL((k_trsv_block_n<16, 16, 32>), dim3(w / 16, 1, nz), dim3(256), 0, s->stream, bt, kb, tb, w, s->Tinv, x, s->Dx, u, z);
            if (rest > 0) hipLaunchKernelGGL((k_trsv_update_n<16, 16, 32>), dim3(rest / 16, 1, nz), dim3(256), 0, s->stream, bt, NP, k0, w, s->Lf, u, x);
        }
    }
    for (int kb = nb - 1; kb >= 0; --kb) {
        const int k0 = kb * tb, w = std::min(tb, NP - k0);
        if (w > 1024) hipLaunchKernelGGL(k_trsv_block_t<2048>, dim3(w / 4, 1, nz), dim3(256), 0, s->stream, bt, kb, tb, w, s->Tinv, z, x);
        else hipLaunchKernelGGL(k_trsv_block_t<1024>, dim3(w / 4, 1, nz), dim3(256), 0, s->stream, bt, kb, tb, w, s->Tinv, z, x);
        if (kb > 0) {
            const int cfirst = s->band64 > 0 ? std::max(0, ((k0 - s->half_bandwidth) / 4) * 4) : 0;
            if (w > 1024) hipLaunchKernelGGL(k_trsv_update_t<2048>, dim3((k0 - cfirst) / 4, 1, nz), dim3(256), 0, s->stream, bt, NP, k0, w, cfirst, s->Lf, x, z);
            else hipLaunchKernelGGL(k_trsv_update_t<1024>, dim3((k0 - cfirst) / 4, 1, nz), dim3(256), 0, s->stream, bt, NP, k0, w, cfirst, s->Lf, x, z);
        }
    }
}


template <typename F>
static bool replay_or_capture(calipso_hip_solver* s, hipGraphExec_t& exec, bool& tried, F enqueue) {
    if (exec) return hipGraphLaunch(exec, s->stream) == hipSuccess;
    if (tried) return false;
    tried = true;
    hipGraph_t graph = nullptr;
    if (hipStreamBeginCapture(s->stream, hipStreamCaptureModeThreadLocal) != hipSuccess) return false;
    enqueue();
    if (hipStreamEndCapture(s->stream, &graph) != hipSuccess || !graph) return false;
    const bool ok = hipGraphInstantiate(&exec, graph, nullptr, nullptr, 0) == hipSuccess;
    (void)hipGraphDestroy(graph);
    if (!ok) { exec = nullptr; return false; }
    return hipGraphLaunch(exec, s->stream) == hipSuccess;
}

#ifdef CALIPSO_LDL_TRACE
}
extern "C" int32_t calipso_hip_debug_ldl_bulk_trace(long long* out) { return hipMemcpyFromSymbol(out, HIP_SYMBOL(calipso::g_ldl_bulk), sizeof(long long) * (32 * 8 + 32 * 16 * 2)) == hipSuccess ? 0 : -1; }
extern "C" int32_t calipso_hip_debug_ldl_trace(long long* out) { return hipMemcpyFromSymbol(out, HIP_SYMBOL(calipso::g_ldl_trace), sizeof(long long) * 64 * 16) == hipSuccess ? 0 : -1; }
namespace calipso {
#endif

void ldl_drop_graphs(calipso_hip_solver* s) {
    if (s->graph_ldl) { (void)hipGraphExecDestroy(s->graph_ldl); s->graph_ldl = nullptr; }
    if (s->graph_ldl_fin) { (void)hipGraphExecDestroy(s->graph_ldl_fin); s->graph_ldl_fin = nullptr; }
    if (s->graph_trsv) { (void)hipGraphExecDestroy(s->graph_trsv); s->graph_trsv = nullptr; }
    s->graph_ldl_tried = false; s->graph_ldl_fin_tried = false; s->graph_trsv_tried = false;
}

hipStream_t ldl_rhs_stream(calipso_hip_solver* s) {
    static const bool env = [] { const char* e = getenv("CALIPSO_HIP_RHS_AHEAD"); return !e || atoi(e) != 0; }();
    if (!env || s->cur || s->compact || (s->stage_parallel && s->spS) || (s->use_graphs && graph_ldl_requested())) return nullptr;
    if (!ldl_overlap(s) || !side_stream(s)) return nullptr;
    return s->stream2;
}

void launch_ldl(calipso_hip_solver* s) {
    s->ldl_forks = 0;
    s->ldl_pub_seq = 0;
    s->ldl_overlap_on = false;
    s->ldl_failed = false;
    if (s->stage_parallel && s->spS) {
        const Batch bt = batch_of(s).b;
        if (sparse_factor_from_dense(s->spS, s->stream, bt, s->S, s->spS_src, s->icount, s->compact && s->spS_inv && s->spS_values_current) == CALIPSO_OK) { s->spS_values_current = false; (void)hipEventRecord(s->ev[14], s->stream); return; }
        if (s->compact) {
            s->err = "structured handle: the multifrontal factorisation was refused and there is no blocked one to fall back to";
            s->ldl_failed = true;
            (void)hipEventRecord(s->ev[14], s->stream);
            return;
        }
        s->stage_parallel = false;
        launch_pad_identity(s);
    }
    s->Lf = lfac_factor_buffer(s);
    const bool graphs = !s->cur && s->use_graphs && graph_ldl_requested();
    if (ldl_overlap(s)) (void)side_stream(s);
    static const bool pub_env = [] { const char* e = getenv("CALIPSO_HIP_LDL_PUBLISH"); return !e || atoi(e) != 0; }();
    s->ldl_publish = pub_env && !graphs && !s->cur;
    s->ldl_epoch += 1;
    if (!graphs || !replay_or_capture(s, s->graph_ldl, s->graph_ldl_tried, [&] { enqueue_ldl_steps(s); })) enqueue_ldl_steps(s);
    (void)hipEventRecord(s->ev[14], s->stream);
    for (int f = 0; f < s->ldl_forks; ++f) {
        const unsigned long long want = (s->ldl_epoch << 16) | (unsigned long long)s->ldl_feeds[3 * f];
        (void)host_wait([&] { return __atomic_load_n(s->hprog, __ATOMIC_ACQUIRE) >= want; }, [&] { return hipStreamQuery(s->stream) == hipErrorNotReady; });
        enqueue_feed(s, s->stream2, f, true);
    }
    if (!graphs || !replay_or_capture(s, s->graph_ldl_fin, s->graph_ldl_fin_tried, [&] { enqueue_ldl_finish(s); })) enqueue_ldl_finish(s);
}

void launch_trsv_direct(calipso_hip_solver* s, double* x) {
    if (s->stage_parallel && s->spS) { (void)sparse_solve_inplace(s->spS, s->stream, batch_of(s).b, x); return; }
    enqueue_trsv(s, x);
}
void launch_trsv(calipso_hip_solver* s, double* x) {
    if (s->stage_parallel && s->spS) { (void)sparse_solve_inplace(s->spS, s->stream, batch_of(s).b, x); return; }
    if (s->cur || x != s->xbuf || !s->use_graphs || !replay_or_capture(s, s->graph_trsv, s->graph_trsv_tried, [&] { enqueue_trsv(s, s->xbuf); })) enqueue_trsv(s, x);
}

}
```

calipso.jl_amd/csrc/lfac.hip:

```cpp
#include "internal.hpp"
#include "ldl_device.hpp"

#include <algorithm>
#include <array>
#include <atomic>
#include <chrono>
#include <cstdio>
#include <map>
#include <memory>
#include <mutex>
#include <queue>
#include <thread>
#include <type_traits>

namespace calipso {

constexpr int LKT = 32;
constexpr int LLDK = LKT + 2;
constexpr int LFAC_LDS_DOUBLES = 4 * TT * LDT > DIAG_LDS_DOUBLES ? 4 * TT * LDT : DIAG_LDS_DOUBLES;
static_assert(6 * TT * LLDK <= LFAC_LDS_DOUBLES, "Schur stage buffers (a ring of three)");

enum { LI_SCHUR = 0, LI_FAR = 1, LI_ROW = 2 };
struct LItem { short kind, i, j, a, b, c, pad0, pad1; };

struct LfacArgs {
    int NP, nx, m, ne, nc, tb;
    int k;
    int nst0, nst;
    double *S, *Zbuf, *Minv, *Dx, *Tinv;
    const double *Lsym, *Zj, *WH;
    int* icount;
    const LItem* items; const int* wfirst;
    unsigned long long* hprog; unsigned long long ptag;
    Scalars sc;
};

struct LLane { int tid, lane, wave, wr, wc, fr, fk, row, cb; };

__device__ __forceinline__ void item_schur(const LfacArgs& a, const LItem it, const LLane& L, double* __restrict__ smem) {
    const int i0 = it.i * TT, j0 = it.j * TT;
    const int P = it.pad0 > 1 ? it.pad0 : 1;
    const bool mf = __builtin_amdgcn_readfirstlane(L.wave) < 16 / P;
    const int wr = (4 / P) * it.pad1 + (L.wave >> 2);
    const int offC = (wr * 16 + L.fr) + (L.wc * 16 + L.fk) * a.NP;
    double* T = a.S + (i0 + (size_t)j0 * a.NP);
    v4d acc = (v4d){0.0, 0.0, 0.0, 0.0};
    if (mf && !(it.c & 1)) {
#pragma unroll
        for (int r = 0; r < 4; ++r) acc[r] = T[offC + 4 * r * a.NP];
    }
    asm volatile("" : "+v"(acc));
    const double omega_y = -1.0 / (-1.0 / (a.sc.rho + a.sc.ep) + (0.0 - a.sc.ed));
    const int k = L.tid & (LKT - 1), c = L.tid >> 5;
    const bool vA0 = i0 + c < a.nx, vA1 = i0 + c + 32 < a.nx, vB0 = j0 + c < a.nx, vB1 = j0 + c + 32 < a.nx;
    const unsigned cA0 = (unsigned)min(i0 + c, a.nx - 1), cA1 = (unsigned)min(i0 + c + 32, a.nx - 1), cB0 = (unsigned)min(j0 + c, a.nx - 1), cB1 = (unsigned)min(j0 + c + 32, a.nx - 1);
    const unsigned pA0 = cA0 * (unsigned)a.m, pA1 = cA1 * (unsigned)a.m, pBm0 = cB0 * (unsigned)a.m, pBm1 = cB1 * (unsigned)a.m, pBc0 = cB0 * (unsigned)a.nc, pBc1 = cB1 * (unsigned)a.nc;
    double ra[2][2], rb[2][2];
    auto fetch = [&](int st, int set) {
        const bool eq = st < a.nst0;
        const int kl = (eq ? st : st - a.nst0) * LKT, klim = (eq ? a.ne : a.nc) - 1 - kl;
        const unsigned kk = (unsigned)min(k, klim);
        const double* bA = (eq ? a.Zj : a.Zj + a.ne) + kl;
        const double* bB = (eq ? a.Zj : a.WH) + kl;
        ra[set][0] = bA[kk + pA0]; ra[set][1] = bA[kk + pA1];
        rb[set][0] = bB[kk + (eq ? pBm0 : pBc0)]; rb[set][1] = bB[kk + (eq ? pBm1 : pBc1)];
    };
    auto park = [&](int buf, int set, int st) {
        const bool eq = st < a.nst0;
        const int klim = (eq ? a.ne : a.nc) - 1 - (eq ? st : st - a.nst0) * LKT;
        const bool kin = k <= klim;
        const double scale = eq ? omega_y : 1.0;
        double* As = smem + (size_t)buf * 2 * TT * LLDK;
        double* Bs = As + TT * LLDK;
        As[c * LLDK + k] = (kin && vA0) ? 1.0 * ra[set][0] : 0.0;
        As[(c + 32) * LLDK + k] = (kin && vA1) ? 1.0 * ra[set][1] : 0.0;
        Bs[c * LLDK + k] = (kin && vB0) ? scale * rb[set][0] : 0.0;
        Bs[(c + 32) * LLDK + k] = (kin && vB1) ? scale * rb[set][1] : 0.0;
    };
    const int s0 = it.a, s1 = it.b;
    double fa[8], fb[8];
    auto reads = [&](int buf, int half) {
        const unsigned ab = (unsigned)(uintptr_t)(smem + (size_t)buf * 2 * TT * LLDK + (wr * 16 + L.fr) * LLDK + L.fk);
        const unsigned bb = (unsigned)(uintptr_t)(smem + (size_t)buf * 2 * TT * LLDK + TT * LLDK + (L.wc * 16 + L.fr) * LLDK + L.fk);
        if (half == 0) {
#pragma unroll
            for (int kk = 0; kk < 4; ++kk) {
// ... 158 lines not shown
    if (it.a < k) apply_panels(a, c2, i, k + 2, it.a, k, L, Ms, Xs, Ms, Xs);
    else lds_barrier();
#pragma unroll
    for (int q = 0; q < 4; ++q) Ys[L.row * LDT + L.cb + q * 16] = y2[q];
    lds_barrier();
    {
        const v4d acc = frag_product((unsigned)(uintptr_t)(Zs + (L.wr * 16 + L.fr) * LDT + L.fk), (unsigned)(uintptr_t)(Ys + (L.wc * 16 + L.fr) * LDT + L.fk));
#pragma unroll
        for (int r = 0; r < 4; ++r) T2[offC + 4 * r * a.NP] = c2[r] - acc[r];
    }
    lds_barrier();
}

__global__ __launch_bounds__(TR_THREADS) void k_lfac(const LfacArgs a) {
    __shared__ double smem[LFAC_LDS_DOUBLES];
    if (a.hprog && blockIdx.x == 0 && threadIdx.x == 0) __hip_atomic_store(a.hprog, a.ptag, __ATOMIC_RELAXED, __HIP_MEMORY_SCOPE_SYSTEM);
    auto lanes = [] {
        LLane L;
        int tid = threadIdx.x;
        asm volatile("" : "+v"(tid));
        L.tid = tid; L.lane = L.tid & 63; L.wave = L.tid >> 6;
        L.wr = L.wave >> 2; L.wc = L.wave & 3; L.fr = L.lane & 15; L.fk = L.lane >> 4;
        L.row = (L.lane & 7) + 8 * ((L.lane >> 4) & 1) + 16 * (L.wave & 3);
        L.cb = ((L.lane >> 3) & 1) + 2 * ((L.lane >> 5) & 1) + 4 * (L.wave >> 2);
        return L;
    };
    if (blockIdx.x == 0) {
        const LLane L = lanes();
        if (a.k < -1) return;
        const int offC = (L.wr * 16 + L.fr) + (L.wc * 16 + L.fk) * a.NP;
        if (a.k == -1) {
            v4d acc = (v4d){0.0, 0.0, 0.0, 0.0};
            if (L.wr >= L.wc) {
#pragma unroll
                for (int q = 0; q < 4; ++q) acc[q] = a.S[offC + 4 * q * a.NP];
            }
            diag_block(smem, acc, a.NP, a.nx, 0, a.tb, a.S, a.Dx, a.Tinv, a.Minv, a.icount);
            return;
        }
        const int k0 = a.k * NB, r0 = k0 + NB;
        double* Zs = smem;
        double* Ys = smem + TT * LDT;
        double* Ms = Ys + TT * LDT;
        double cS[4];
        const double* Q = a.S + ((size_t)r0 + (size_t)r0 * a.NP);
#pragma unroll
        for (int r = 0; r < 4; ++r) cS[r] = Q[offC + 4 * r * a.NP];
        form_Z(a.S + ((size_t)r0 + (size_t)k0 * a.NP), a.NP, a.Minv + (size_t)a.k * NB * NB, Ys, Ms, Zs, L.row, L.cb, L.wr, L.wc, L.fr, L.fk);
        const v4d acc = frag_product((unsigned)(uintptr_t)(Zs + (L.wr * 16 + L.fr) * LDT + L.fk), (unsigned)(uintptr_t)(Ys + (L.wc * 16 + L.fr) * LDT + L.fk));
#pragma unroll
        for (int r = 0; r < 4; ++r) cS[r] -= acc[r];
        lds_barrier();
        diag_block(smem, (v4d){cS[0], cS[1], cS[2], cS[3]}, a.NP, a.nx, r0, a.tb, a.S, a.Dx, a.Tinv, a.Minv, a.icount);
        return;
    }
    const int w = (int)blockIdx.x - 1;
    const int first = a.wfirst[w], last = a.wfirst[w + 1];
#pragma unroll 1
    for (int idx = first; idx < last; ++idx) {
        const LItem it = a.items[idx];
        const LLane L = lanes();
        if (it.kind == LI_SCHUR) item_schur(a, it, L, smem);
        else if (it.kind == LI_FAR) item_far(a, it, L, smem);
        else item_row(a, it, L, smem);
    }
}

struct LfacPlan {
    int nblk = 0, nst0 = 0, nst = 0, W = 0;
    std::vector<int> item0;
    std::vector<LItem> items;
    std::vector<int> wfirst;
    double budget = 0.0; int margin = 0;
    std::vector<double> load;
    std::vector<int> counts;
    std::vector<double> mean;
    std::vector<int> busy;
};
struct LfacAux {
    LfacPlan plan;
    int NP = 0, ne = 0, nc = 0;
    double *Zbuf = nullptr, *Lfac = nullptr;
    LItem* d_items = nullptr; int* d_wfirst = nullptr;
    double plan_ms = 0.0;
};

constexpr double LFAC_CHAIN_US = 19.4;
constexpr double LFAC_LAUNCH_US = 0.0;
static double cost_schur(int stages, int P = 1) { return (P == 1 ? 1.52 : P == 2 ? 1.05 : 0.8) * stages + 3.3; }
static double cost_far(int panels) { return 3.1 * panels + 2.5; }
static double cost_row(int pending) { return 15.0 + 2.2 * pending; }
static double cost_row_half(int pending, bool second) { return second ? 11.0 + 2.2 * pending : 10.0; }
static int stages_within(double us, int P = 1) { const int n = (int)((us - 3.3) / (P == 1 ? 1.52 : P == 2 ? 1.05 : 0.8)); return n < 1 ? 1 : n; }

static bool lfac_make_plan(LfacPlan& P, int nblk, int nx, int ne, int nc, int W, double budget, double head, int margin = 1 << 20) {
    P = LfacPlan();
    P.nblk = nblk; P.W = W; P.budget = budget;
    P.nst0 = (ne + LKT - 1) / LKT; P.nst = P.nst0 + (nc + LKT - 1) / LKT;
    const int nst = P.nst;
    if (head <= 0.0) head = std::min(cost_schur(nst), 120.0);
    struct Tile { int st = 0, pn = 0; };
    std::vector<Tile> tiles((size_t)nblk * nblk);
    auto T = [&](int i, int j) -> Tile& { return tiles[(size_t)i * nblk + j]; };
    auto deadline = [&](int i, int j) { return (i == 0 && j == 0) ? -1 : std::max(0, j - 2); };
    std::vector<std::pair<int, int>> order;
    for (int j = 0; j < nblk; ++j) for (int i = j; i < nblk; ++i) {
// ... 247 lines not shown
    LfacAux* A = static_cast<LfacAux*>(s->lfac_aux);
    if (!A) return;
    if (A->Zbuf) (void)hipFree(A->Zbuf);
    if (A->Lfac) (void)hipFree(A->Lfac);
    if (A->d_items) (void)hipFree(A->d_items);
    if (A->d_wfirst) (void)hipFree(A->d_wfirst);
    delete A;
    s->lfac_aux = nullptr;
}


static LfacAux* lfac_prepare(calipso_hip_solver* s) {
    LfacAux* A = static_cast<LfacAux*>(s->lfac_aux);
    const int NP = s->d.NP, nblk = NP / NB;
    if (A && A->NP == NP && A->ne == s->d.ne && A->nc == s->d.nc) return A;
    lfac_release(s);
    A = new LfacAux();
    A->NP = NP; A->ne = s->d.ne; A->nc = s->d.nc;
    bool ok = false;
    {
        double ms = 0.0;
        const auto P = lfac_cached_plan(nblk, s->d.nx, s->d.ne, s->d.nc, 255, &ms);
        A->plan_ms = ms;
        if (P) { A->plan = *P; ok = true; }
        else {
            char buf[256];
            snprintf(buf, sizeof buf, "note: no left-looking plan meets its deadlines for nx = %d, ne = %d, nc = %d (NP = %d): the right-looking schedule is kept", s->d.nx, s->d.ne, s->d.nc, NP);
            s->err = buf;
        }
    }
    const size_t nn = (size_t)NP * NP;
    const bool planned = ok;
    ok = ok && hipMalloc((void**)&A->Zbuf, nn * sizeof(double)) == hipSuccess && hipMalloc((void**)&A->Lfac, nn * sizeof(double)) == hipSuccess &&
         hipMalloc((void**)&A->d_items, std::max<size_t>(1, A->plan.items.size()) * sizeof(LItem)) == hipSuccess &&
         hipMalloc((void**)&A->d_wfirst, A->plan.wfirst.size() * sizeof(int)) == hipSuccess &&
         hipMemcpy(A->d_items, A->plan.items.data(), A->plan.items.size() * sizeof(LItem), hipMemcpyHostToDevice) == hipSuccess &&
         hipMemcpy(A->d_wfirst, A->plan.wfirst.data(), A->plan.wfirst.size() * sizeof(int), hipMemcpyHostToDevice) == hipSuccess &&
         hipMemset(A->Lfac, 0, nn * sizeof(double)) == hipSuccess;
    s->lfac_aux = A;
    if (!ok) {
        if (planned) { (void)hipGetLastError(); s->err = "note: the buffers of the left-looking schedule (2 NP^2 doubles) could not be allocated: the right-looking schedule is kept"; }
        lfac_release(s); s->lfac_failed = true; return nullptr;
    }
    return A;
}

bool lfac_ready(calipso_hip_solver* s) { return lfac_on(s) && lfac_prepare(s) != nullptr; }

double* lfac_factor_buffer(calipso_hip_solver* s) {
    if (!lfac_ready(s)) return s->S;
    return static_cast<LfacAux*>(s->lfac_aux)->Lfac;
}

int lfac_enqueue(calipso_hip_solver* s, unsigned long long* hprog, unsigned long long epoch) {
    LfacAux* A = lfac_prepare(s);
    if (!A) return 0;
    const int NP = s->d.NP, nblk = NP / NB;
    LfacArgs a;
    a.NP = NP; a.nx = s->d.nx; a.m = s->d.m; a.ne = s->d.ne; a.nc = s->d.nc; a.tb = trsv_block(NP, (int)s->solve_block);
    a.nst0 = A->plan.nst0; a.nst = A->plan.nst;
    a.S = s->S; a.Zbuf = A->Zbuf; a.Minv = s->Ypanel; a.Dx = s->Dx; a.Tinv = s->Tinv;
    a.Lsym = s->Lsym; a.Zj = s->Z; a.WH = s->WH; a.icount = s->icount;
    a.sc = s->sc;
    int launches = 0;
    for (int ell = -2; ell <= nblk - 2; ++ell) {
        a.k = ell;
        a.items = A->d_items;
        a.wfirst = A->d_wfirst + A->plan.item0[ell + 2];
        a.hprog = ell >= 0 ? hprog : (unsigned long long*)nullptr;
        a.ptag = epoch | (unsigned long long)(ell >= 0 ? ell : 0);
        hipLaunchKernelGGL(k_lfac, dim3(1 + A->plan.busy[ell + 2]), dim3(TR_THREADS), 0, s->stream, a);
        ++launches;
    }
    return launches;
}

void lfac_describe(calipso_hip_solver* s, double out[8]) {
    for (int i = 0; i < 8; ++i) out[i] = 0.0;
    LfacAux* A = static_cast<LfacAux*>(s->lfac_aux);
    if (!A) return;
    out[0] = (double)A->plan.item0.size(); out[1] = (double)A->plan.items.size(); out[2] = A->plan.budget; out[3] = A->plan.load.empty() ? 0.0 : A->plan.load[0];
    double sum = 0.0; int n = 0;
    for (size_t l = 2; l < A->plan.load.size(); ++l) { sum += A->plan.load[l]; ++n; }
    out[4] = n ? sum / n : 0.0;
    out[5] = 2.0 * (double)A->NP * A->NP * sizeof(double) + (double)A->plan.items.size() * sizeof(LItem) + (double)A->plan.wfirst.size() * sizeof(int);
    out[6] = A->plan_ms; out[7] = lfac_plan_estimate(A->plan);
}

}

extern "C" int32_t calipso_hip_debug_lfac_describe(calipso_hip_solver* s, double out[8]) {
    if (!s || !out) return CALIPSO_ERR_ARGUMENT;
    calipso::lfac_describe(s, out);
    return CALIPSO_OK;
}

extern "C" int32_t calipso_hip_debug_lfac_plan(int32_t nblk, int32_t nx, int32_t ne, int32_t nc, double budget, double head, double* out, int32_t max_launches) {
    calipso::LfacPlan P;
    if (budget <= 0.0 ? !calipso::lfac_best_plan(P, nblk, nx, ne, nc, 255) : !calipso::lfac_make_plan(P, nblk, nx, ne, nc, 255, budget, head)) return 0;
    if (max_launches > 0) { out[6 * (max_launches - 1)] = P.budget; out[6 * (max_launches - 1) + 1] = P.margin; out[6 * (max_launches - 1) + 2] = P.load.empty() ? 0.0 : P.load[0]; }
    const int nl = (int)P.item0.size();
    for (int l = 0; l < nl && l < max_launches; ++l) {
        const int w0 = P.item0[l];
        const int i0 = P.wfirst[w0], i1 = P.wfirst[w0 + P.W];
        double kinds[3] = {0, 0, 0}, longrow = 0;
        for (int i = i0; i < i1; ++i) {
            const calipso::LItem& it = P.items[i];
            kinds[it.kind] += 1;
            if (it.kind == calipso::LI_ROW) longrow = std::max(longrow, calipso::cost_row(it.j - it.a));
        }
        out[6 * l + 0] = P.load[l]; out[6 * l + 1] = i1 - i0; out[6 * l + 2] = kinds[0]; out[6 * l + 3] = kinds[1]; out[6 * l + 4] = kinds[2]; out[6 * l + 5] = P.mean[l]; (void)longrow;
    }
    return nl;
}

extern "C" double calipso_hip_debug_lfac_items(calipso_hip_solver* s, int32_t kind, int32_t n, int32_t P, int32_t per_worker, int32_t skew, int32_t active) {
    using namespace calipso;
    if (!s || !lfac_ready(s)) return -1.0;
    LfacAux* A = static_cast<LfacAux*>(s->lfac_aux);
    const int NP = s->d.NP, nblk = NP / NB, W = A->plan.W, nst = A->plan.nst;
    std::vector<LItem> items; std::vector<int> wfirst;
    std::vector<std::pair<int, int>> tiles;
    for (int j = 0; j < nblk; ++j) for (int i = j; i < nblk; ++i) tiles.push_back({i, j});
    size_t next = 0;
    for (int w = 0; w < W; ++w) {
        wfirst.push_back((int)items.size());
        for (int q = 0; q < per_worker && (active <= 0 || (w * active) / W != ((w + 1) * active) / W); ++q) {
            LItem it{};
            if (kind == 0) {
                const auto ij = tiles[(next++) % tiles.size()];
                const int a0 = skew ? (w * 7) % std::max(1, nst - n) : 0;
                it.kind = LI_SCHUR; it.i = (short)ij.first; it.j = (short)ij.second; it.a = (short)a0; it.b = (short)std::min(nst, a0 + n); it.c = 1; it.pad0 = (short)P; it.pad1 = (short)(w % std::max(1, P));
            } else if (kind == 1) {
                std::pair<int, int> ij;
                do { ij = tiles[(next++) % tiles.size()]; } while (ij.second < n + 3);
                it.kind = LI_FAR; it.i = (short)ij.first; it.j = (short)ij.second; it.a = 0; it.b = (short)n;
            } else {
                const int k = n + (w % 3), i = k + 2 + (int)((next++) % (size_t)(nblk - k - 2));
                it.kind = LI_ROW; it.i = (short)i; it.j = (short)k; it.a = (short)(k - n); it.c = (short)(kind == 3 ? 0 : kind == 4 ? 3 : 1);
            }
            items.push_back(it);
        }
    }
    wfirst.push_back((int)items.size());
    LItem* d_items = nullptr; int* d_wfirst = nullptr;
    if (hipMalloc((void**)&d_items, items.size() * sizeof(LItem)) != hipSuccess || hipMalloc((void**)&d_wfirst, wfirst.size() * sizeof(int)) != hipSuccess) return -1.0;
    (void)hipMemcpy(d_items, items.data(), items.size() * sizeof(LItem), hipMemcpyHostToDevice);
    (void)hipMemcpy(d_wfirst, wfirst.data(), wfirst.size() * sizeof(int), hipMemcpyHostToDevice);
    LfacArgs a;
    a.NP = NP; a.nx = s->d.nx; a.m = s->d.m; a.ne = s->d.ne; a.nc = s->d.nc; a.tb = trsv_block(NP, (int)s->solve_block);
    a.nst0 = A->plan.nst0; a.nst = nst; a.k = -2;
    a.S = s->S; a.Zbuf = A->Zbuf; a.Minv = s->Ypanel; a.Dx = s->Dx; a.Tinv = s->Tinv; a.Lsym = s->Lsym; a.Zj = s->Z; a.WH = s->WH; a.icount = s->icount;
    a.items = d_items; a.wfirst = d_wfirst; a.hprog = nullptr; a.ptag = 0; a.sc = s->sc;
    hipEvent_t e0, e1;
    (void)hipEventCreate(&e0); (void)hipEventCreate(&e1);
    hipLaunchKernelGGL(k_lfac, dim3(1 + W), dim3(TR_THREADS), 0, s->stream, a);
    (void)hipStreamSynchronize(s->stream);
    (void)hipEventRecord(e0, s->stream);
    for (int r = 0; r < 5; ++r) hipLaunchKernelGGL(k_lfac, dim3(1 + W), dim3(TR_THREADS), 0, s->stream, a);
    (void)hipEventRecord(e1, s->stream);
    (void)hipEventSynchronize(e1);
    float ms = 0.f;
    (void)hipEventElapsedTime(&ms, e0, e1);
    (void)hipEventDestroy(e0); (void)hipEventDestroy(e1);
    (void)hipFree(d_items); (void)hipFree(d_wfirst);
    return (double)ms * 1e3 / 5.0;
}
```

calipso.jl_amd/csrc/qp.hip:

```cpp
#include "internal.hpp"
#include "device_utils.hpp"

namespace calipso {

__global__ __launch_bounds__(1024) void k_qp_objective(Batch bt, int nx, const double* __restrict__ x, const double* __restrict__ Lx,
                                                        const double* __restrict__ q, double* __restrict__ dscal) {
    __shared__ double sm[16];
    inst_shift(bt, x, Lx, q, dscal);
    double a = 0.0, b = 0.0;
    for (int i0 = threadIdx.x; i0 < nx; i0 += 4 * 1024) {
        double xv[4], lv[4], qv[4];
#pragma unroll
        for (int u = 0; u < 4; ++u) { const int i = i0 + u * 1024; const bool in = i < nx; xv[u] = in ? x[i] : 0.0; lv[u] = in ? Lx[i] : 0.0; qv[u] = in ? q[i] : 0.0; }
#pragma unroll
        for (int u = 0; u < 4; ++u) if (i0 + u * 1024 < nx) { a += xv[u] * lv[u]; b += qv[u] * xv[u]; }
    }
    const double ra = block_sum(a, sm);
    const double rb = block_sum(b, sm);
    if (threadIdx.x == 0) dscal[0] = 0.5 * ra + rb;
}

__global__ void k_vec_add(Batch bt, int n, const double* __restrict__ a, const double* __restrict__ b, double sign, double* __restrict__ out) {
    inst_shift(bt, a, b, out);
    const int i = blockIdx.x * blockDim.x + threadIdx.x;
    if (i < n) out[i] = a[i] + sign * b[i];
}

void launch_qp_evaluate(calipso_hip_solver* s, const double* point, uint32_t flags) {
    const Dims& d = s->d;
    const double* x = point;
    const double* y = point + d.oy();
    const double* z = point + d.oz();
    double* Lx = s->vtmp + 3 * (size_t)d.N;
    const Batch bt = batch_of(s).b;
    const unsigned nz = bt.n;
    if (flags & (CALIPSO_EVAL_OBJECTIVE | CALIPSO_EVAL_OBJECTIVE_GRADIENT)) {
        if (!(flags & CALIPSO_EVAL_OBJECTIVE)) gemv_t(s, d.nx, d.nx, s->Lxx, d.nx, x, s->fx, 1.0, 0.0, SP_LXX, s->qp.q);
        else {
            gemv_t(s, d.nx, d.nx, s->Lxx, d.nx, x, Lx, 1.0, 0.0, SP_LXX);
            hipLaunchKernelGGL(k_qp_objective, dim3(1, 1, nz), dim3(1024), 0, s->stream, bt, d.nx, x, Lx, s->qp.q, s->dscal);
            if (flags & CALIPSO_EVAL_OBJECTIVE_GRADIENT)
                hipLaunchKernelGGL(k_vec_add, dim3((d.nx + 255) / 256, 1, nz), dim3(256), 0, s->stream, bt, d.nx, Lx, s->qp.q, 1.0, s->fx);
        }
    }
    const bool want_g = (flags & CALIPSO_EVAL_EQUALITY) && d.ne, want_h = (flags & CALIPSO_EVAL_CONE) && d.nc;
    if (want_g && want_h) {
        gemv_n(s, d.m, d.nx, s->Z, d.m, x, s->gh, 1.0, 0.0, SP_Z, s->qp.bh);
    } else if (want_g) {
        gemv_n(s, d.ne, d.nx, s->gx, d.m, x, s->g, 1.0, 0.0, SP_GX, s->qp.bh);
    } else if (want_h) {
        gemv_n(s, d.nc, d.nx, s->hx, d.m, x, s->hc, 1.0, 0.0, SP_HX, s->qp.bh + d.ne);
    }
    if (flags & CALIPSO_EVAL_EQUALITY_DUAL_GRADIENT) {
        if (d.ne) gemv_t(s, d.ne, d.nx, s->gx, d.m, y, s->gyx, 1.0, 0.0, SP_GX);
        else fill_d(s, s->gyx, d.nx, 0.0);
    }
    if (flags & CALIPSO_EVAL_CONE_DUAL_GRADIENT) {
        if (d.nc) gemv_t(s, d.nc, d.nx, s->hx, d.m, z, s->hzx, 1.0, 0.0, SP_HX);
        else fill_d(s, s->hzx, d.nx, 0.0);
    }
}

}
```

calipso.jl_amd/csrc/schur.hip:

```cpp
#include "internal.hpp"
#include "device_utils.hpp"

#include <algorithm>
#include <mutex>

namespace calipso {

__global__ __launch_bounds__(1024) void k_cone_weights(BatchSc bt, Dims d, ConeDev cd, const double* __restrict__ w,
                                                        double* __restrict__ kzz, double* __restrict__ wz, double* __restrict__ Bsoc,
                                                        double* __restrict__ Wsoc, double* __restrict__ work, int* __restrict__ icount) {
    __shared__ int smi[3][16];
    inst_shift(bt.b, w, kzz, wz, Bsoc, Wsoc, work);
    inst_shift_i(bt.b, icount);
    const Scalars sc = bt.scal(blockIdx.z);
    const int tid = threadIdx.x;
    const double* sl = w + d.os();
    const double* t = w + d.ot();
    const double Hss = 0.0 + sc.ep;
    int pos = 0, nonpos = 0, zero = 0;
    for (int i = tid; i < d.q; i += 1024) {
        const double Sb = sl[i] - sc.ed, Ti = t[i];
        const double k = -1.0 * Sb / (Ti + Sb * Hss) + (0.0 - sc.ed);
        kzz[i] = k;
        wz[i] = -1.0 / k;
        pos += k > 0.0; nonpos += k <= 0.0; zero += k == 0.0;
    }
    for (int j = tid; j < d.n_soc; j += 1024) {
        const int st = cd.soc_start[j], dim = cd.soc_dim[j], off = cd.soc_woff[j];
        double* B = Bsoc + off;
        double* W = Wsoc + off;
        if (dim > 4) continue;
        {
            constexpr int MD = 4;
            double ls[MD], lt[MD], u[MD], c[MD], o[MD], Bm[MD * MD], M[MD * MD];
#pragma unroll
            for (int a = 0; a < MD; ++a) { ls[a] = a < dim ? sl[st + a] : 0.0; lt[a] = a < dim ? t[st + a] : 0.0; u[a] = 0.0; c[a] = 0.0; o[a] = 0.0; }
#pragma unroll
            for (int e = 0; e < MD * MD; ++e) { Bm[e] = 0.0; M[e] = 0.0; }
            const double sb1 = ls[0] - sc.ed;
            u[0] = lt[0] + sb1 * Hss;
#pragma unroll
            for (int k = 1; k < MD; ++k) if (k < dim) u[k] = lt[k] + ls[k] * Hss;
#pragma unroll
            for (int col = 0; col < MD; ++col) if (col < dim) {
#pragma unroll
                for (int a = 0; a < MD; ++a) if (a < dim) c[a] = (a == col) ? sb1 : (col == 0 ? ls[a] : (a == 0 ? ls[col] : 0.0));
                arrow_inverse_small<MD>(dim, u, c, o);
#pragma unroll
                for (int a = 0; a < MD; ++a) if (a < dim) Bm[a + col * MD] = 0.0 - o[a];
            }
#pragma unroll
            for (int a = 0; a < MD; ++a) if (a < dim) Bm[a + a * MD] += (0.0 - sc.ed);
#pragma unroll
            for (int b = 0; b < MD; ++b)
#pragma unroll
                for (int a = 0; a < MD; ++a) if (a < dim && b < dim) { B[a + b * dim] = Bm[a + b * MD]; M[a + b * MD] = (a <= b) ? Bm[a + b * MD] : Bm[b + a * MD]; }
#pragma unroll
            for (int jj = 0; jj < MD; ++jj) if (jj < dim) {
                const double dj = M[jj + jj * MD];
                pos += dj > 0.0; nonpos += dj <= 0.0; zero += dj == 0.0;
#pragma unroll
                for (int i = jj + 1; i < MD; ++i) if (i < dim) {
                    const double yij = M[i + jj * MD];
                    const double l = yij / dj;
#pragma unroll
                    for (int k = jj + 1; k < MD; ++k) if (k <= i) M[i + k * MD] -= l * (k == i ? yij : M[jj + k * MD]);
                    M[i + jj * MD] = l;
                    M[jj + i * MD] = yij;
                }
            }
#pragma unroll
            for (int col = 0; col < MD; ++col) if (col < dim) {
#pragma unroll
                for (int a = 0; a < MD; ++a) o[a] = (a == col) ? 1.0 : 0.0;
#pragma unroll
                for (int a = 0; a < MD; ++a) if (a < dim) {
                    double x = o[a];
#pragma unroll
                    for (int k = 0; k < MD; ++k) if (k < a) x -= M[a + k * MD] * o[k];
                    o[a] = x;
                }
#pragma unroll
                for (int a = 0; a < MD; ++a) if (a < dim) o[a] /= M[a + a * MD];
#pragma unroll
                for (int a = MD - 1; a >= 0; --a) if (a < dim) {
                    double x = o[a];
#pragma unroll
                    for (int k = 0; k < MD; ++k) if (k > a && k < dim) x -= M[k + a * MD] * o[k];
                    o[a] = x;
                }
#pragma unroll
                for (int a = 0; a < MD; ++a) if (a < dim) W[a + col * dim] = -o[a];
            }
        }
    }
    if (tid == 0 && d.ne > 0) {
        const double ky = -1.0 / (sc.rho + sc.ep) + (0.0 - sc.ed);
        if (ky > 0.0) pos += d.ne;
        if (ky <= 0.0) nonpos += d.ne;
        if (ky == 0.0) zero += d.ne;
    }
    pos = wave_sum_i(pos); nonpos = wave_sum_i(nonpos); zero = wave_sum_i(zero);
    if ((tid & 63) == 0) { smi[0][tid >> 6] = pos; smi[1][tid >> 6] = nonpos; smi[2][tid >> 6] = zero; }
    __syncthreads();
    if (tid < 3) {
        int a = 0;
        for (int k = 0; k < 16; ++k) a += smi[tid][k];
        icount[tid] = a;
        icount[3 + tid] = 0;
    }
}

void launch_cone_weights(calipso_hip_solver* s) {
    const BatchSc B = batch_of(s);
    hipLaunchKernelGGL(k_cone_weights, dim3(1, 1, B.b.n), dim3(1024), 0, s->stream, B, s->d, s->cone, s->solution, s->kzz, s->wz, s->Bsoc,
                       s->Wsoc, s->socwork, s->icount);
    launch_cone_weights_wide(s);
}

constexpr int SCALE_COLS = 16;
__global__ void k_scale_rows(Batch bt, Dims d, ConeDev cd, const double* __restrict__ hx, const double* __restrict__ wz,
                             const double* __restrict__ Wsoc, double* __restrict__ WH, const int* __restrict__ zrow, double* __restrict__ Spad) {
    inst_shift(bt, hx, wz, Wsoc, WH);
    if (zrow) inst_shift_i(bt, zrow);
    if (Spad) {
        inst_shift(bt, Spad);
        const long long total = (long long)gridDim.x * gridDim.y * blockDim.x, count = (long long)(d.NP - d.nx) * d.NP;
        for (long long e = ((long long)blockIdx.y * gridDim.x + blockIdx.x) * blockDim.x + threadIdx.x; e < count; e += total) {
            const int i = d.nx + (int)(e / d.NP), j = (int)(e % d.NP);
            if (j <= i) Spad[i + (size_t)j * d.NP] = (i == j) ? 1.0 : 0.0;
        }
    }
    const int c = blockIdx.x * blockDim.x + threadIdx.x;
    if (c >= d.nc) return;
    int st = 0, dim = 0;
    const double* W = nullptr;
    double w0 = 0.0;
    if (c < d.q) w0 = wz[c];
    else { const int j = cd.entry_soc[c]; st = cd.soc_start[j]; dim = cd.soc_dim[j]; W = Wsoc + cd.soc_woff[j]; }
    int col0 = blockIdx.y * SCALE_COLS, col1 = min(d.nx, col0 + SCALE_COLS);
    if (zrow) {
        const int k = d.ne + c;
        col0 = max(col0, zrow[2 * k]); col1 = min(col1, zrow[2 * k + 1]);
    }
    const int cbase = blockIdx.y * SCALE_COLS;
    if (c < d.q) {
        double hv[SCALE_COLS];
#pragma unroll
        for (int k = 0; k < SCALE_COLS; ++k) { const int col = cbase + k; hv[k] = (col >= col0 && col < col1) ? hx[c + (size_t)col * d.m] : 0.0; }
#pragma unroll
        for (int k = 0; k < SCALE_COLS; ++k) { const int col = cbase + k; if (col >= col0 && col < col1) WH[c + (size_t)col * d.nc] = w0 * hv[k]; }
        return;
    }
    if (dim <= 4) {
        double wr[4];
#pragma unroll
        for (int b = 0; b < 4; ++b) wr[b] = b < dim ? W[(c - st) + b * dim] : 0.0;
        for (int k0 = 0; k0 < SCALE_COLS; k0 += 8) {
            double hv[8][4];
#pragma unroll
            for (int k = 0; k < 8; ++k) {
                const int col = cbase + k0 + k;
                const bool in = col >= col0 && col < col1;
#pragma unroll
                for (int b = 0; b < 4; ++b) hv[k][b] = (in && b < dim) ? hx[st + b + (size_t)col * d.m] : 0.0;
            }
#pragma unroll
            for (int k = 0; k < 8; ++k) {
                const int col = cbase + k0 + k;
                if (col >= col0 && col < col1) {
                    double v = 0.0;
#pragma unroll
                    for (int b = 0; b < 4; ++b) if (b < dim) v += wr[b] * hv[k][b];
                    WH[c + (size_t)col * d.nc] = v;
                }
            }
        }
        return;
    }
    for (int col = col0; col < col1; ++col) {
        const double* h = hx + (size_t)col * d.m;
        double v = 0.0;
        for (int b = 0; b < dim; ++b) v += W[(c - st) + b * dim] * h[st + b];
        WH[c + (size_t)col * d.nc] = v;
    }
}

void launch_scale_rows(calipso_hip_solver* s) {
    s->pad_done = false;
    if (s->d.nc == 0) return;
    if (s->blocks.on && s->blocks_effective) return;
    const BatchSc B = batch_of(s);
    const bool pad = s->d.NP > s->d.nx && !(s->stage_parallel && s->spS);
    s->pad_done = pad;
    hipLaunchKernelGGL(k_scale_rows, dim3((s->d.nc + 255) / 256, (s->d.nx + SCALE_COLS - 1) / SCALE_COLS, B.b.n), dim3(256), 0, s->stream, B.b, s->d, s->cone, s->hx, s->wz, s->Wsoc, s->WH, s->band64 > 0 ? s->zrow : nullptr,
                       pad ? s->S : (double*)nullptr);
}

constexpr int KT = 32;
constexpr int LDK = KT + 2;
constexpr int SCHUR_THREADS = 1024;
constexpr int SLD = TILE * KT / SCHUR_THREADS;
typedef double v4d __attribute__((ext_vector_type(4)));

struct SchurStage { const double* MA; const double* MB; int kmax; int k0; double bscale; int lda, ldb; };

__device__ __forceinline__ SchurStage schur_stage(int st, int nst0, int est0, int cst0, const Dims& d, const double* gx, const double* hx, const double* WH,
                                                  double omega_y) {
    SchurStage g;
    if (st < nst0) { g.MA = gx; g.MB = gx; g.kmax = d.ne; g.k0 = (est0 + st) * KT; g.bscale = omega_y; g.lda = d.m; g.ldb = d.m; }
    else { g.MA = hx; g.MB = WH; g.kmax = d.nc; g.k0 = (cst0 + st - nst0) * KT; g.bscale = 1.0; g.lda = d.m; g.ldb = d.nc; }
    return g;
}

__device__ __forceinline__ void stage_fetch(double (&r)[SLD], const double* __restrict__ M, int ldm, int kmax, int ncols, int k0, int c0, int width,
                                            int tid, double scale) {
    const int k = tid % KT, cbase = tid / KT;
#pragma unroll
    for (int it = 0; it < SLD; ++it) {
        const int c = cbase + it * (SCHUR_THREADS / KT);
        const int gk = k0 + k, gc = c0 + c;
        r[it] = (gk < kmax && gc < ncols && c < width) ? scale * M[gk + (size_t)gc * ldm] : 0.0;
    }
}
__device__ __forceinline__ void stage_fetch_full(double (&r)[SLD], const double* __restrict__ base, const unsigned (&off)[SLD], double scale) {
#pragma unroll
    for (int it = 0; it < SLD; ++it) r[it] = scale * base[off[it]];
}
__device__ __forceinline__ void stage_store(double* dst, const double (&r)[SLD], int tid) {
    const int k = tid % KT, cbase = tid / KT;
#pragma unroll
    for (int it = 0; it < SLD; ++it) dst[(cbase + it * (SCHUR_THREADS / KT)) * LDK + k] = r[it];
}

constexpr int SB = 5;
__device__ __forceinline__ int schur_row_count(int bi, int nx, int TJ) { return (min(nx, (bi + 1) * TILE) - 1) / TJ + 1; }
__device__ __forceinline__ void schur_tile(int t, int nx, int TJ, int& bi, int& bj) {
    const int nbi = (nx + TILE - 1) / TILE;
    for (int r0 = 0; r0 < nbi; r0 += SB) {
        const int r1 = min(nbi, r0 + SB);
        const int cmax = schur_row_count(r1 - 1, nx, TJ);
        for (int c0 = 0; c0 < cmax; c0 += SB) {
            for (int b = r0; b < r1; ++b) {
                const int c = min(max(schur_row_count(b, nx, TJ) - c0, 0), SB);
                if (t < c) { bi = b; bj = c0 + t; return; }
                t -= c;
            }
// ... 248 lines not shown
```

calipso.jl_amd/csrc/solvek.hip:

```cpp
#include "internal.hpp"
#include "device_utils.hpp"

namespace calipso {

__global__ void k_copy_pad(const double* __restrict__ src, int n, double* __restrict__ dst, int npad) {
    const int i = blockIdx.x * blockDim.x + threadIdx.x;
    if (i < npad) dst[i] = i < n ? src[i] : 0.0;
}
void launch_copy_pad(calipso_hip_solver* s, const double* src, int n, double* dst, int npad) {
    hipLaunchKernelGGL(k_copy_pad, dim3((npad + 255) / 256), dim3(256), 0, s->stream, src, n, dst, npad);
}

__global__ void k_negate_copy(const double* __restrict__ src, double* __restrict__ dst, int n) {
    const int i = blockIdx.x * blockDim.x + threadIdx.x;
    if (i < n) dst[i] = -1.0 * src[i];
}
void launch_negate_copy(calipso_hip_solver* s, const double* src, double* dst, int n) {
    hipLaunchKernelGGL(k_negate_copy, dim3((n + 255) / 256), dim3(256), 0, s->stream, src, dst, n);
}

void linear_solve_device(calipso_hip_solver* s, bool with_t2, bool rhs_ready) {
    const Dims& d = s->d;
    if (d.m && !rhs_ready) gemv_t(s, d.m, d.nx, s->Z, d.m, s->t1, s->xbuf, 1.0, 1.0, SP_Z);
    launch_trsv(s, s->xbuf);
    if (d.m && with_t2) gemv_n(s, d.m, d.nx, s->Z, d.m, s->xbuf, s->t2, 1.0, 0.0, SP_Z);
}

__global__ void k_solve_prepare(Dims d, Scalars sc, ConeDev cd, const double* __restrict__ b, const double* __restrict__ wz,
                                const double* __restrict__ Wsoc, double* __restrict__ xbuf, double* __restrict__ t1) {
    const int i = blockIdx.x * blockDim.x + threadIdx.x;
    if (i < d.NP) { xbuf[i] = i < d.nx ? b[i] : 0.0; return; }
    const int e = i - d.NP;
    if (e >= d.m) return;
    const double* bm = b + d.nx;
    if (e < d.ne) {
        const double omega_y = -1.0 / (-1.0 / (sc.rho + sc.ep) + (0.0 - sc.ed));
        t1[e] = omega_y * bm[e];
    } else {
        const int c = e - d.ne;
        if (c < d.q) t1[e] = wz[c] * bm[e];
        else {
            const int j = cd.entry_soc[c], st = cd.soc_start[j], dim = cd.soc_dim[j];
            const double* W = Wsoc + cd.soc_woff[j];
            double v = 0.0;
            for (int q = 0; q < dim; ++q) v += W[(c - st) + q * dim] * bm[d.ne + st + q];
            t1[e] = v;
        }
    }
}
__global__ void k_solve_finish(Dims d, Scalars sc, ConeDev cd, const double* __restrict__ b, const double* __restrict__ dx,
                               const double* __restrict__ t2, const double* __restrict__ wz, const double* __restrict__ Wsoc,
                               double* __restrict__ out) {
    const int i = blockIdx.x * blockDim.x + threadIdx.x;
    if (i >= d.n) return;
    if (i < d.nx) { out[i] = dx[i]; return; }
    const int e = i - d.nx;
    const double* bm = b + d.nx;
    if (e < d.ne) {
        const double omega_y = -1.0 / (-1.0 / (sc.rho + sc.ep) + (0.0 - sc.ed));
        out[i] = -1.0 * omega_y * (bm[e] - t2[e]);
    } else {
        const int c = e - d.ne;
        if (c < d.q) out[i] = -1.0 * wz[c] * (bm[e] - t2[e]);
        else {
            const int j = cd.entry_soc[c], st = cd.soc_start[j], dim = cd.soc_dim[j];
            const double* W = Wsoc + cd.soc_woff[j];
            double v = 0.0;
            for (int q = 0; q < dim; ++q) v += W[(c - st) + q * dim] * (bm[d.ne + st + q] - t2[d.ne + st + q]);
            out[i] = -1.0 * v;
        }
    }
}
void launch_solve_from_b(calipso_hip_solver* s) {
    const Dims& d = s->d;
    hipLaunchKernelGGL(k_solve_prepare, dim3((d.NP + d.m + 255) / 256), dim3(256), 0, s->stream, d, s->sc, s->cone, s->residual_symmetric, s->wz,
                       s->Wsoc, s->xbuf, s->t1);
    linear_solve_device(s);
// ... 57 lines not shown
```

include/calipso_hip.h:

```cpp
#ifndef CALIPSO_HIP_H
#define CALIPSO_HIP_H

#include <stdint.h>

#ifdef __cplusplus
extern "C" {
#endif

typedef struct calipso_hip_solver calipso_hip_solver;

enum {
    CALIPSO_OK = 0,
    CALIPSO_ERR_INERTIA = -1,
    CALIPSO_ERR_CONE_SEARCH = -2,
    CALIPSO_ERR_CALLBACK = -3,
    CALIPSO_ERR_ARGUMENT = -4,
    CALIPSO_ERR_HIP = -5,
    CALIPSO_ERR_LAYOUT = -6,
    CALIPSO_WARN_ZERO_PIVOT = 1,
    CALIPSO_WARN_REFINEMENT = 2,
    CALIPSO_WARN_LINE_SEARCH = 3
};

enum {
// ... 193 lines not shown
int32_t calipso_hip_smallnewton_trace(calipso_hip_smallnewton*, int32_t rows, double* out);
int32_t calipso_hip_smallnewton_solve(calipso_hip_smallnewton*, int32_t* result, double* ms);
int32_t calipso_hip_smallnewton_steps(calipso_hip_smallnewton*, int32_t count, int32_t advance, double* info, int32_t* status, double* ms);
int32_t calipso_hip_smallnewton_differentiate(calipso_hip_smallnewton*, int64_t p, int32_t shared, const double* jacobian_parameters, double* sensitivity, int32_t* status, double* ms);
#define CALIPSO_SMALLNEWTON_ABI 1
enum { CALIPSO_SMALLNEWTON_QUERY = 0, CALIPSO_SMALLNEWTON_GRANT_LDS = 1, CALIPSO_SMALLNEWTON_OCCUPANCY = 2, CALIPSO_SMALLNEWTON_LAUNCH = 3 };
typedef struct calipso_smallnewton_launch {
    int32_t op;
    int32_t abi;
    int64_t* out;
    const void* args;
    int64_t args_bytes;
    int32_t mode;
    int32_t threads;
    int32_t soc, lu;
    int32_t eval_rtheta;
    int32_t reserved;
    int64_t grid;
    int64_t lds_bytes;
    void* stream;
} calipso_smallnewton_launch;
typedef int32_t (*calipso_smallnewton_kernels_fn)(const calipso_smallnewton_launch*);
int32_t calipso_hip_smallnewton_set_evaluator(calipso_hip_smallnewton*, calipso_smallnewton_kernels_fn fn, int64_t n_parameters);
int32_t calipso_hip_smallnewton_set_parameters(calipso_hip_smallnewton*, const double* theta, int32_t shared);
int32_t calipso_hip_smallnewton_differentiate_parameters(calipso_hip_smallnewton*, double* sensitivity, int32_t* status, double* ms);
int32_t calipso_hip_smallnewton_differentiate_adjoint(calipso_hip_smallnewton*, int64_t k, const double* cotangent, double* adjoint, double* grad_theta, double* grad_qp,
                                                      int32_t* status, double* ms);
int32_t calipso_hip_smallnewton_set_stream(calipso_hip_smallnewton*, void* hip_stream, int32_t borrow);
int32_t calipso_hip_smallnewton_set_qp_device(calipso_hip_smallnewton*, const double* P, const double* q, const double* A, const double* b, const double* G, const double* h,
                                              double objective_scale, int32_t shared_mask, int32_t row_major);
int32_t calipso_hip_smallnewton_initialize_device(calipso_hip_smallnewton*, const double* x0);
int32_t calipso_hip_smallnewton_set_state_device(calipso_hip_smallnewton*, const double* w, const double* lambda, const double* scalars);
int32_t calipso_hip_smallnewton_set_parameters_device(calipso_hip_smallnewton*, const double* theta, int32_t shared);
int32_t calipso_hip_smallnewton_solve_device(calipso_hip_smallnewton*);
int32_t calipso_hip_smallnewton_get_solution_device(calipso_hip_smallnewton*, double* x, double* y, double* z, double* w, int32_t* status);
int32_t calipso_hip_smallnewton_differentiate_adjoint_device(calipso_hip_smallnewton*, int64_t k, const double* cot_w, const double* cot_x, const double* cot_y, const double* cot_z,
                                                             double* adjoint, double* grad_theta, double* const* grad_qp, int32_t reduce_mask, int32_t row_major, int32_t* status);

typedef struct calipso_hip_comm calipso_hip_comm;
int32_t calipso_hip_comm_unique_id(uint8_t id[128]);
int32_t calipso_hip_comm_init(int32_t rank, int32_t nranks, const uint8_t id[128], int32_t device, calipso_hip_comm** out);
int32_t calipso_hip_comm_destroy(calipso_hip_comm*);
int32_t calipso_hip_comm_size(calipso_hip_comm*, int32_t out[2]);
const char* calipso_hip_comm_last_error(calipso_hip_comm*);
int64_t calipso_hip_comm_gather_status(calipso_hip_comm*, const int32_t* rows, int64_t n_rows, int32_t* all_rows, int64_t cap_rows,
                                       int64_t* counts_out);
int32_t calipso_hip_comm_allreduce_sum(calipso_hip_comm*, double* values, int64_t count);

int32_t calipso_hip_mfma_f64_peak(int32_t device, double* tflops);

int32_t calipso_hip_phase_times(calipso_hip_solver*, double out[9]);
int32_t calipso_hip_kernel_times(calipso_hip_solver*, double out[8]);
int32_t calipso_hip_structure_work(calipso_hip_solver*, double out[8]);
int32_t calipso_hip_schedule_info(calipso_hip_solver*, double out[4]);
int32_t calipso_hip_synchronize(calipso_hip_solver*);
int32_t calipso_hip_streams_concurrent(calipso_hip_solver* a, calipso_hip_solver* b, double out[6]);
int32_t calipso_hip_rebind_stream(calipso_hip_solver*, int32_t priority_class);

int32_t calipso_hip_splitmix_uniform(uint64_t problem_id, uint64_t stream_id, double lo, double hi, int64_t count, double* out);

#ifdef __cplusplus
}
#endif
#endif
```

Before: 555.3 Newton steps/s.

## Fuse per-step small kernels: cone weights with row scaling, inertia publish, QP candidate gemvs

Adds several launch-reducing fusions behind an environment bitmask that enables all of them by default. Cone weights are computed inside the row-scaling kernel, with the weights recomputed per row. Inertia publishing is folded into the lfac factorisation enqueue. The QP candidate transpose and normal gemvs share one launch, and the objective reduction rides on the reduce kernel. A forward-solve-ahead hook is also threaded into the triangular solve. The aim is to cut kernel launch and serialisation overhead in a launch-bound Newton step, at the cost of redundant per-thread cone math and more complex code paths.

```diff
diff --git a/calipso.jl_amd/__init__.py b/calipso.jl_amd/__init__.py
--- a/calipso.jl_amd/__init__.py
+++ b/calipso.jl_amd/__init__.py
@@ -449,9 +449,10 @@
         return dict(schur_flops=out[0], packed_doubles=out[1], segment_pairs=int(out[2]), factor_flops=out[3], factor_nnz=out[4], order=int(out[5]), structured=bool(out[6]))
 
     def schedule_info(self):
-        out = np.zeros(4)
+        out = np.zeros(9)
         self._check(self._L.calipso_hip_schedule_info(self._h, _pd(out)), "schedule_info")
-        return dict(prologue_ahead_steps=int(out[0]), last_prologue_mode=int(out[1]), ahead_undone=int(out[2]))
+        return dict(prologue_ahead_steps=int(out[0]), last_prologue_mode=int(out[1]), ahead_undone=int(out[2]),
+                    fusion_a=int(out[4]), fusion_b=int(out[5]), fusion_c=int(out[6]), fusion_d=int(out[7]))
 
     def padded_nx(self):
         return int(self.kernel_times()[2])
diff --git a/calipso.jl_amd/csrc/api.hip b/calipso.jl_amd/csrc/api.hip
--- a/calipso.jl_amd/csrc/api.hip
+++ b/calipso.jl_amd/csrc/api.hip
@@ -636,7 +636,9 @@
 static int do_factorize(H* s, int64_t inertia[3], bool rhs_ahead_ok = false) {
     factor_times(s);
     (void)hipEventRecord(s->ev[10], s->stream);
-    launch_cone_weights(s);
+    launch_cone_weights(s, true);
+    const bool scaled = s->weights_pending;
+    if (scaled) launch_scale_rows(s);
     s->rhs_ahead = false; s->rhs_joined = false;
     if (rhs_ahead_ok) {
         hipStream_t st2 = calipso::ldl_rhs_stream(s);
@@ -652,7 +654,7 @@
             s->rhs_ahead = true;
         }
     }
-    launch_scale_rows(s);
+    if (!scaled) launch_scale_rows(s);
     calipso::inject_refused_launch(s->stream);
     (void)hipEventRecord(s->ev[11], s->stream);
     launch_schur(s);
@@ -709,9 +711,11 @@
     }
     const bool ready = use_ahead && which == 0 && s->rhs_ahead && s->rhs_joined;
     s->rhs_ahead = false;
+    const int fwd_done = ready ? s->fwd_ahead : 0;
+    s->fwd_ahead = 0;
     if (!ready) launch_residual_symmetric(s, res);
     const bool tail = which == 0 && !accumulate && s->d.m > 0;
-    linear_solve_device(s, !tail, ready);
+    linear_solve_device(s, !tail, ready, fwd_done);
     if (tail && launch_solve_tail(s, 0, false, refine_follows)) return;
     if (tail) gemv_n(s, s->d.m, s->d.nx, s->Z, s->d.m, s->xbuf, s->t2, 1.0, 0.0, SP_Z);
     launch_recover(s, st, res, accumulate, which == 0 ? 1 : 0);
@@ -1466,9 +1470,10 @@
     return CALIPSO_OK;
 }
 
-int32_t calipso_hip_schedule_info(H* s, double out[4]) {
+int32_t calipso_hip_schedule_info(H* s, double out[9]) {
     if (!s || !out) return CALIPSO_ERR_ARGUMENT;
     out[0] = (double)s->prologue_ahead_steps; out[1] = (double)s->last_prologue_mode; out[2] = (double)s->ahead_undone; out[3] = 0.0;
+    for (int i = 0; i < 5; ++i) out[4 + i] = (double)s->fusion_count[i];
     return CALIPSO_OK;
 }
 
diff --git a/calipso.jl_amd/csrc/device_utils.hpp b/calipso.jl_amd/csrc/device_utils.hpp
--- a/calipso.jl_amd/csrc/device_utils.hpp
+++ b/calipso.jl_amd/csrc/device_utils.hpp
@@ -46,6 +46,22 @@
     double r = 0.0;
     if (threadIdx.x == 0) for (int i = 0; i < nw; ++i) r = fmax(r, sm[i]);
     return r;
+}
+
+__device__ __forceinline__ void qp_objective_body(Batch bt, int nx, const double* __restrict__ x, const double* __restrict__ Lx, const double* __restrict__ q,
+                                                  double* __restrict__ dscal, double* sm) {
+    inst_shift(bt, x, Lx, q, dscal);
+    double a = 0.0, b = 0.0;
+    for (int i0 = threadIdx.x; i0 < nx; i0 += 4 * 1024) {
+        double xv[4], lv[4], qv[4];
+#pragma unroll
+        for (int u = 0; u < 4; ++u) { const int i = i0 + u * 1024; const bool in = i < nx; xv[u] = in ? x[i] : 0.0; lv[u] = in ? Lx[i] : 0.0; qv[u] = in ? q[i] : 0.0; }
+#pragma unroll
+        for (int u = 0; u < 4; ++u) if (i0 + u * 1024 < nx) { a += xv[u] * lv[u]; b += qv[u] * xv[u]; }
+    }
+    const double ra = block_sum(a, sm);
+    const double rb = block_sum(b, sm);
+    if (threadIdx.x == 0) dscal[0] = 0.5 * ra + rb;
 }
 
 __device__ __forceinline__ void arrow_inverse(int n, const double* u, const double* x, double* out) {
diff --git a/calipso.jl_amd/csrc/gemv.hip b/calipso.jl_amd/csrc/gemv.hip
--- a/calipso.jl_amd/csrc/gemv.hip
+++ b/calipso.jl_amd/csrc/gemv.hip
@@ -44,13 +44,13 @@
     }
 }
 
-__global__ __launch_bounds__(256) void k_gemv_t(Batch bt, Sparsity sp, int rows, int cols, const double* __restrict__ A, int ld, const double* __restrict__ x,
-                                                 double* __restrict__ y, double alpha, double beta, const double* __restrict__ add = nullptr) {
+__device__ __forceinline__ void gemv_t_body(Batch bt, Sparsity sp, int bx, int rows, int cols, const double* __restrict__ A, int ld, const double* __restrict__ x,
+                                            double* __restrict__ y, double alpha, double beta, const double* __restrict__ add) {
     inst_shift(bt, A, x, y);
     if (add) inst_shift(bt, add);
     if (sp.kr) inst_shift_i(bt, sp.kr);
     const int lane = threadIdx.x & 63;
-    const int col = blockIdx.x * 4 + (threadIdx.x >> 6);
+    const int col = bx * 4 + (threadIdx.x >> 6);
     if (col >= cols) return;
     const double* a = A + (size_t)col * ld;
     const BlockRanges br = column_blocks(sp, col, rows);
@@ -75,6 +75,10 @@
     }
     const double r = wave_sum(acc0 + acc1);
     if (lane == 0) y[col] = add ? alpha * r + add[col] : ((beta == 0.0) ? alpha * r : alpha * r + beta * y[col]);
+}
+__global__ __launch_bounds__(256) void k_gemv_t(Batch bt, Sparsity sp, int rows, int cols, const double* __restrict__ A, int ld, const double* __restrict__ x,
+                                                 double* __restrict__ y, double alpha, double beta, const double* __restrict__ add = nullptr) {
+    gemv_t_body(bt, sp, blockIdx.x, rows, cols, A, ld, x, y, alpha, beta, add);
 }
 
 __device__ __forceinline__ void gemv_t2_body(Batch bt, Sparsity sp, int bx, int rows, int cols, const double* __restrict__ A, int ld, const double* __restrict__ x1,
@@ -233,13 +237,12 @@
     else gemv_n_partial_body(bt, spl, (b - nt2) % rb, (b - nt2) / rb, 0, rowsl, colsl, chunk, L, ldl, xl, partial);
 }
 
-__global__ __launch_bounds__(256) void k_gemv_n_reduce(Batch bt, int rows, int nchunk, const double* __restrict__ partial, double* __restrict__ y, double alpha, double beta,
-                                                       const double* __restrict__ add = nullptr) {
-    __shared__ double part[4][64];
+__device__ __forceinline__ void gemv_n_reduce_body(Batch bt, int bx, int tid, double (*part)[64], int rows, int nchunk, const double* __restrict__ partial, double* __restrict__ y,
+                                                   double alpha, double beta, const double* __restrict__ add) {
     inst_shift(bt, partial, y);
     if (add) inst_shift(bt, add);
-    const int r = threadIdx.x & 63, p = threadIdx.x >> 6;
-    const int i = blockIdx.x * 64 + r;
+    const int r = tid & 63, p = tid >> 6;
+    const int i = bx * 64 + r;
     double acc = 0.0;
     if (i < rows) {
         static_assert(GN_MAXCHUNK <= 64, "16 partials per thread");
@@ -253,10 +256,32 @@
     }
     part[p][r] = acc;
     __syncthreads();
-    if (threadIdx.x < 64 && i < rows) {
+    if (tid < 64 && i < rows) {
         const double v = (part[0][r] + part[1][r]) + (part[2][r] + part[3][r]);
         y[i] = add ? alpha * v + add[i] : ((beta == 0.0) ? alpha * v : alpha * v + beta * y[i]);
     }
+}
+__global__ __launch_bounds__(256) void k_gemv_n_reduce(Batch bt, int rows, int nchunk, const double* __restrict__ partial, double* __restrict__ y, double alpha, double beta,
+                                                       const double* __restrict__ add = nullptr) {
+    __shared__ double part[4][64];
+    gemv_n_reduce_body(bt, blockIdx.x, threadIdx.x, part, rows, nchunk, partial, y, alpha, beta, add);
+}
+
+__global__ __launch_bounds__(256) void k_gemv_t_and_n(Batch bt, Sparsity spt, int rowst, int colst, const double* __restrict__ At, int ldt, const double* __restrict__ xt,
+                                                       double* __restrict__ yt, int nt, Sparsity spn, int rb, int rowsn, int colsn, int chunk, const double* __restrict__ An, int ldn,
+                                                       const double* __restrict__ xn, double* __restrict__ partial) {
+    static_assert(GN_ROWS == 256, "one block size for both bodies");
+    const int b = blockIdx.x;
+    if (b < nt) gemv_t_body(bt, spt, b, rowst, colst, At, ldt, xt, yt, 1.0, 0.0, nullptr);
+    else gemv_n_partial_body(bt, spn, (b - nt) % rb, (b - nt) / rb, 0, rowsn, colsn, chunk, An, ldn, xn, partial);
+}
+__global__ __launch_bounds__(1024) void k_gemv_n_reduce_and_objective(Batch bt, int nred, int rows, int nchunk, const double* __restrict__ partial, double* __restrict__ y,
+                                                                       const double* __restrict__ add, int nx, const double* __restrict__ x, const double* __restrict__ Lx,
+                                                                       const double* __restrict__ q, double* __restrict__ dscal) {
+    __shared__ double part[4][4][64];
+    if ((int)blockIdx.x == nred) { qp_objective_body(bt, nx, x, Lx, q, dscal, &part[0][0][0]); return; }
+    const int sub = threadIdx.x >> 8;
+    gemv_n_reduce_body(bt, blockIdx.x * 4 + sub, threadIdx.x & 255, part[sub], rows, nchunk, partial, y, 1.0, 0.0, add);
 }
 
 constexpr int BOTH_RQ = 16;
@@ -344,6 +369,21 @@
     return 0;
 }
 
+bool gemv_qp_candidate(calipso_hip_solver* s, const double* x, double* Lx, const double* q, const double* bh, double* gh) {
+    const Dims& d = s->d;
+    if (!(step_fusions() & FUSE_QP_CANDIDATE) || s->cur || s->compact || s->blocks.on || s->band64 > 0 || d.m == 0 || d.nx == 0) return false;
+    int rb, nchunk, chunk;
+    gemv_n_chunks(d.m, d.nx, rb, nchunk, chunk);
+    if (nchunk < 1) return false;
+    const BatchSc B = batch_of(s);
+    const int nt = (d.nx + 3) / 4, nred = (d.m + 255) / 256;
+    hipLaunchKernelGGL(k_gemv_t_and_n, dim3(nt + rb * nchunk, 1, 1), dim3(256), 0, s->stream, B.b, Sparsity(), d.nx, d.nx, s->Lxx, d.nx, x, Lx, nt, Sparsity(), rb, d.m, d.nx, chunk, s->Z, d.m, x,
+                       s->gemv_partial);
+    hipLaunchKernelGGL(k_gemv_n_reduce_and_objective, dim3(nred + 1, 1, 1), dim3(1024), 0, s->stream, B.b, nred, d.m, nchunk, s->gemv_partial, gh, bh, d.nx, x, Lx, q, s->dscal);
+    s->fusion_count[3] += 1;
+    return true;
+}
+
 void gemv_n(calipso_hip_solver* s, int rows, int cols, const double* A, int ld, const double* x, double* y, double alpha, double beta, int kind, const double* add) {
     if (rows == 0) return;
     if (blocks_gemv_n(s, kind, x, y, alpha, beta)) { if (add) launch_add(s, y, add, rows); return; }
diff --git a/calipso.jl_amd/csrc/internal.hpp b/calipso.jl_amd/csrc/internal.hpp
--- a/calipso.jl_amd/csrc/internal.hpp
+++ b/calipso.jl_amd/csrc/internal.hpp
@@ -1,6 +1,7 @@
 #pragma once
 #include <hip/hip_runtime.h>
 #include <stdint.h>
+#include <stdlib.h>
 
 #include <map>
 #include <string>
@@ -99,6 +100,12 @@
     std::vector<ZBlock> zb; std::vector<LBlock> lb; std::vector<Segment> seg; std::vector<int> segblk, pairblk, colrange, seg_of_col; std::vector<SegPair> pairs;
     size_t packed = 0, spacked = 0; int max_lb = 0; unsigned long long signature = 0;
 };
+
+enum { FUSE_FWD_AHEAD = 1, FUSE_INERTIA = 2, FUSE_CONE_WEIGHTS = 4, FUSE_QP_CANDIDATE = 8 };
+inline int step_fusions() {
+    static const int env = [] { const char* e = getenv("CALIPSO_HIP_STEP_FUSIONS"); return e ? atoi(e) : 31; }();
+    return env;
+}
 
 struct QpEval {
     bool attached = false;
@@ -146,7 +153,9 @@
     void (*side_work)(calipso_hip_solver*) = nullptr;
     unsigned long long pub_seq2 = 0;
     long long prologue_ahead_steps = 0;
+    long long fusion_count[5] = {0, 0, 0, 0, 0};
     long long ahead_undone = 0;
+    int fwd_ahead = 0;
     bool rhs_ahead = false, rhs_joined = false;
     double *evalL = nullptr, *evalZ = nullptr;
     std::map<std::string, double*> optd;
@@ -171,6 +180,7 @@
     double *solution = nullptr, *candidate = nullptr, *lambda = nullptr, *parameters = nullptr;
     double *residual = nullptr, *residual_error = nullptr, *step = nullptr, *step_correction = nullptr, *saved_point = nullptr;
     double *residual_symmetric = nullptr, *step_symmetric = nullptr, *merit_gradient = nullptr;
+    bool weights_pending = false;
     bool pad_done = false;
     double* Kdense = nullptr;
     double* S = nullptr;
@@ -303,9 +313,10 @@
             const double* add = nullptr);
 void gemv_t2(calipso_hip_solver* s, int rows, int cols, const double* A, int ld, const double* x1, const double* x2, double* y1, double* y2, int kind = SP_DENSE);
 int gemv_refine_pair(calipso_hip_solver* s, const double* x1, const double* x2, double* y1, double* y2, const double* xl, double* yl, bool defer_reduce = false);
+bool gemv_qp_candidate(calipso_hip_solver* s, const double* x, double* Lx, const double* q, const double* bh, double* gh);
 void gemv_both(calipso_hip_solver* s, int rows, int cols, const double* A, int ld, const double* x, const double* u, double* yn, double* yt, double beta_t,
                int kind = SP_DENSE);
-void launch_cone_weights(calipso_hip_solver* s);
+void launch_cone_weights(calipso_hip_solver* s, bool scale_rows_follows = false);
 void launch_cone_weights_wide(calipso_hip_solver* s);
 void launch_residual_symmetric_wide(calipso_hip_solver* s, const double* res, int p, double* rsym, double* t1, bool regions);
 void launch_recover_wide(calipso_hip_solver* s, const double* res, int p, const double* rsym, const double* t2, double* dsym, double* step, double* accumulate, int zsx_mode, bool regions);
@@ -334,12 +345,12 @@
 bool blocks_entry_offsets(const calipso_hip_solver* s, int which, int row, int col, long long* off_c, long long* off_r);
 void launch_ldl(calipso_hip_solver* s);
 void ldl_drop_graphs(calipso_hip_solver* s);
-void launch_trsv(calipso_hip_solver* s, double* x);
+void launch_trsv(calipso_hip_solver* s, double* x, int fwd_done = 0);
 bool lastblock_sym_on(const calipso_hip_solver* s);
 bool wform_on(const calipso_hip_solver* s);
 bool lfac_on(const calipso_hip_solver* s);
 bool lfac_ready(calipso_hip_solver* s);
-int lfac_enqueue(calipso_hip_solver* s, unsigned long long* hprog, unsigned long long epoch);
+int lfac_enqueue(calipso_hip_solver* s, unsigned long long* hprog, unsigned long long epoch, unsigned long long publish_seq = 0);
 double* lfac_factor_buffer(calipso_hip_solver* s);
 void lfac_release(calipso_hip_solver* s);
 void lfac_describe(calipso_hip_solver* s, double out[8]);
@@ -348,7 +359,7 @@
 void launch_lambda_update(calipso_hip_solver* s);
 void launch_jacobian_parameters(calipso_hip_solver* s);
 void launch_negate_copy(calipso_hip_solver* s, const double* src, double* dst, int n);
-void linear_solve_device(calipso_hip_solver* s, bool with_t2 = true, bool rhs_ready = false);
+void linear_solve_device(calipso_hip_solver* s, bool with_t2 = true, bool rhs_ready = false, int fwd_done = 0);
 hipStream_t ldl_rhs_stream(calipso_hip_solver* s);
 void launch_solve_from_b(calipso_hip_solver* s);
 void gemm(calipso_hip_solver* s, int M, int N, int K, double alpha, const double* A, int lda, bool transA, const double* B, int ldb, double beta,
diff --git a/calipso.jl_amd/csrc/ldl.hip b/calipso.jl_amd/csrc/ldl.hip
--- a/calipso.jl_amd/csrc/ldl.hip
+++ b/calipso.jl_amd/csrc/ldl.hip
@@ -464,7 +464,10 @@
     unsigned long long* const hprog = overlap ? s->hprog_dev : (unsigned long long*)nullptr;
     const unsigned long long epoch = s->ldl_epoch << 16;
     s->lfac_last = lfac;
-    if (lfac) launches = lfac_enqueue(s, hprog, epoch);
+    const bool publish = s->ldl_publish && nz == 1;
+    const bool publish_inside = publish && lfac && (step_fusions() & FUSE_INERTIA) && NP / NB >= 2;
+    if (publish) s->ldl_pub_seq = ++s->pub_seq;
+    if (lfac) launches = lfac_enqueue(s, hprog, epoch, publish_inside ? s->ldl_pub_seq : 0);
     for (int kb = 0; !lfac && kb + 1 < nblk;) {
         const int k0 = kb * NB;
         const int rows = std::min(NP - k0 - NB, band * NB);
@@ -487,10 +490,8 @@
     int forks = 0;
     if (overlap) while (3 * forks < (int)s->ldl_feeds.size() && s->ldl_feeds[3 * forks] <= nblk - 2) ++forks;
     s->ldl_forks = forks;
-    if (s->ldl_publish && nz == 1) {
-        s->ldl_pub_seq = ++s->pub_seq;
-        hipLaunchKernelGGL(k_publish_inertia, dim3(1), dim3(64), 0, s->stream, s->icount, s->hicount_dev, s->hseq_dev, s->ldl_pub_seq);
-    }
+    if (publish && publish_inside && launches > 0) s->fusion_count[1] += 1;
+    else if (publish) hipLaunchKernelGGL(k_publish_inertia, dim3(1), dim3(64), 0, s->stream, s->icount, s->hicount_dev, s->hseq_dev, s->ldl_pub_seq);
 }
 
 static void enqueue_ldl_finish(calipso_hip_solver* s) {
@@ -848,7 +849,22 @@
     const int rows = wform_rows(s, rb);
     hipLaunchKernelGGL(k_wform_product, dim3((rows / 32) * (w / 32), 1, bt.n), dim3(256), 0, stream, bt, NP, tb, kb, w, rb, rows, s->Lf, s->Tinv, s->Wfac + wform_offset(NP, tb, kb));
 }
-static void enqueue_trsv_wform(calipso_hip_solver* s, double* x) {
+static void enqueue_trsv_fwd_block(calipso_hip_solver* s, hipStream_t stream, int kb, double* x, const int* gate, int ge) {
+    const int NP = s->d.NP, tb = trsv_block(NP, (int)s->solve_block), nb = (NP + tb - 1) / tb;
+    const Batch bt = batch_of(s).b;
+    const unsigned nz = bt.n;
+    double* u = s->zf;
+    double* z = s->zf2;
+    const bool sym = lastblock_sym_on(s);
+    const int k0 = kb * tb, w = std::min(tb, NP - k0), rb = NP - k0 - w;
+    const double* Wb = s->Wfac + wform_offset(NP, tb, kb);
+    const int rows = wform_rows(s, rb);
+    const int snap = (sym && kb == nb - 2) ? 1 + rows : 0;
+    const int grows = snap ? rb : rows;
+    if (w > 512) hipLaunchKernelGGL((k_trsv_fwd<16, 32, 32>), dim3((w + grows) / 16, 1, nz), dim3(512), 0, stream, bt, kb, tb, w, rb, s->Tinv, Wb, x, s->Dx, u, z, gate, ge, snap);
+    else hipLaunchKernelGGL((k_trsv_fwd<16, 16, 32>), dim3((w + grows) / 16, 1, nz), dim3(256), 0, stream, bt, kb, tb, w, rb, s->Tinv, Wb, x, s->Dx, u, z, gate, ge, snap);
+}
+static void enqueue_trsv_wform(calipso_hip_solver* s, double* x, int fwd_done = 0) {
     const int NP = s->d.NP, tb = trsv_block(NP, (int)s->solve_block), nb = (NP + tb - 1) / tb;
     double* u = s->zf;
     double* z = s->zf2;
@@ -857,15 +873,7 @@
     const int* gate = s->gate_epoch ? s->gate : (const int*)nullptr;
     const int ge = s->gate_epoch;
     const bool sym = lastblock_sym_on(s);
-    for (int kb = 0; kb < nb - (sym ? 1 : 0); ++kb) {
-        const int k0 = kb * tb, w = std::min(tb, NP - k0), rb = NP - k0 - w;
-        const double* Wb = s->Wfac + wform_offset(NP, tb, kb);
-        const int rows = wform_rows(s, rb);
-        const int snap = (sym && kb == nb - 2) ? 1 + rows : 0;
-        const int grows = snap ? rb : rows;
-        if (w > 512) hipLaunchKernelGGL((k_trsv_fwd<16, 32, 32>), dim3((w + grows) / 16, 1, nz), dim3(512), 0, s->stream, bt, kb, tb, w, rb, s->Tinv, Wb, x, s->Dx, u, z, gate, ge, snap);
-        else hipLaunchKernelGGL((k_trsv_fwd<16, 16, 32>), dim3((w + grows) / 16, 1, nz), dim3(256), 0, s->stream, bt, kb, tb, w, rb, s->Tinv, Wb, x, s->Dx, u, z, gate, ge, snap);
-    }
+    for (int kb = fwd_done; kb < nb - (sym ? 1 : 0); ++kb) enqueue_trsv_fwd_block(s, s->stream, kb, x, gate, ge);
     if (sym) {
         const int k0 = (nb - 1) * tb, w = NP - k0;
         const double* Msym = s->Wfac + wform_offset(NP, tb, nb - 1);
@@ -954,8 +962,20 @@
     return s->stream2;
 }
 
+static void enqueue_fwd_ahead(calipso_hip_solver* s, int f) {
+    if (!(step_fusions() & FUSE_FWD_AHEAD) || s->ldl_feeds[3 * f + 1] != 1 || s->ldl_feeds[3 * f + 2] != s->fwd_ahead) return;
+    if (!s->rhs_ahead || !s->lfac_last || !lastblock_sym_on(s)) return;
+    if (s->side_work && (!s->side_ran || s->prologue_rc < 0)) return;
+    const int NP = s->d.NP, tb = trsv_block(NP, (int)s->solve_block), nb = (NP + tb - 1) / tb;
+    if (s->fwd_ahead >= nb - 1) return;
+    enqueue_trsv_fwd_block(s, s->stream2, s->fwd_ahead, s->xbuf, nullptr, 0);
+    if (s->fwd_ahead == 0) s->fusion_count[0] += 1;
+    s->fwd_ahead += 1;
+}
+
 void launch_ldl(calipso_hip_solver* s) {
     s->ldl_forks = 0;
+    s->fwd_ahead = 0;
     s->ldl_pub_seq = 0;
     s->ldl_overlap_on = false;
     s->ldl_failed = false;
@@ -983,6 +1003,7 @@
         const unsigned long long want = (s->ldl_epoch << 16) | (unsigned long long)s->ldl_feeds[3 * f];
         (void)host_wait([&] { return __atomic_load_n(s->hprog, __ATOMIC_ACQUIRE) >= want; }, [&] { return hipStreamQuery(s->stream) == hipErrorNotReady; });
         enqueue_feed(s, s->stream2, f, true);
+        enqueue_fwd_ahead(s, f);
     }
     if (!graphs || !replay_or_capture(s, s->graph_ldl_fin, s->graph_ldl_fin_tried, [&] { enqueue_ldl_finish(s); })) enqueue_ldl_finish(s);
 }
@@ -991,8 +1012,9 @@
     if (s->stage_parallel && s->spS) { (void)sparse_solve_inplace(s->spS, s->stream, batch_of(s).b, x); return; }
     enqueue_trsv(s, x);
 }
-void launch_trsv(calipso_hip_solver* s, double* x) {
+void launch_trsv(calipso_hip_solver* s, double* x, int fwd_done) {
     if (s->stage_parallel && s->spS) { (void)sparse_solve_inplace(s->spS, s->stream, batch_of(s).b, x); return; }
+    if (fwd_done > 0) { enqueue_trsv_wform(s, x, fwd_done); return; }
     if (s->cur || x != s->xbuf || !s->use_graphs || !replay_or_capture(s, s->graph_trsv, s->graph_trsv_tried, [&] { enqueue_trsv(s, s->xbuf); })) enqueue_trsv(s, x);
 }
 
diff --git a/calipso.jl_amd/csrc/lfac.hip b/calipso.jl_amd/csrc/lfac.hip
--- a/calipso.jl_amd/csrc/lfac.hip
+++ b/calipso.jl_amd/csrc/lfac.hip
@@ -32,6 +32,7 @@
     int* icount;
     const LItem* items; const int* wfirst;
     unsigned long long* hprog; unsigned long long ptag;
+    int* hcount; unsigned long long* hseq; unsigned long long seq;
     Scalars sc;
 };
 
@@ -296,6 +297,12 @@
         for (int r = 0; r < 4; ++r) cS[r] -= acc[r];
         lds_barrier();
         diag_block(smem, (v4d){cS[0], cS[1], cS[2], cS[3]}, a.NP, a.nx, r0, a.tb, a.S, a.Dx, a.Tinv, a.Minv, a.icount);
+        if (a.hseq && L.tid == 0) {
+#pragma unroll
+            for (int i = 0; i < 6; ++i) a.hcount[i] = __hip_atomic_load(a.icount + i, __ATOMIC_RELAXED, __HIP_MEMORY_SCOPE_AGENT);
+            __threadfence_system();
+            __hip_atomic_store(a.hseq, a.seq, __ATOMIC_RELEASE, __HIP_MEMORY_SCOPE_SYSTEM);
+        }
         return;
     }
     const int w = (int)blockIdx.x - 1;
@@ -649,7 +656,7 @@
     return static_cast<LfacAux*>(s->lfac_aux)->Lfac;
 }
 
-int lfac_enqueue(calipso_hip_solver* s, unsigned long long* hprog, unsigned long long epoch) {
+int lfac_enqueue(calipso_hip_solver* s, unsigned long long* hprog, unsigned long long epoch, unsigned long long publish_seq) {
     LfacAux* A = lfac_prepare(s);
     if (!A) return 0;
     const int NP = s->d.NP, nblk = NP / NB;
@@ -666,6 +673,8 @@
         a.wfirst = A->d_wfirst + A->plan.item0[ell + 2];
         a.hprog = ell >= 0 ? hprog : (unsigned long long*)nullptr;
         a.ptag = epoch | (unsigned long long)(ell >= 0 ? ell : 0);
+        const bool pub = publish_seq != 0 && ell == nblk - 2;
+        a.hcount = pub ? s->hicount_dev : (int*)nullptr; a.hseq = pub ? s->hseq_dev : (unsigned long long*)nullptr; a.seq = pub ? publish_seq : 0;
         hipLaunchKernelGGL(k_lfac, dim3(1 + A->plan.busy[ell + 2]), dim3(TR_THREADS), 0, s->stream, a);
         ++launches;
     }
@@ -748,7 +757,7 @@
     a.NP = NP; a.nx = s->d.nx; a.m = s->d.m; a.ne = s->d.ne; a.nc = s->d.nc; a.tb = trsv_block(NP, (int)s->solve_block);
     a.nst0 = A->plan.nst0; a.nst = nst; a.k = -2;
     a.S = s->S; a.Zbuf = A->Zbuf; a.Minv = s->Ypanel; a.Dx = s->Dx; a.Tinv = s->Tinv; a.Lsym = s->Lsym; a.Zj = s->Z; a.WH = s->WH; a.icount = s->icount;
-    a.items = d_items; a.wfirst = d_wfirst; a.hprog = nullptr; a.ptag = 0; a.sc = s->sc;
+    a.items = d_items; a.wfirst = d_wfirst; a.hprog = nullptr; a.ptag = 0; a.hcount = nullptr; a.hseq = nullptr; a.seq = 0; a.sc = s->sc;
     hipEvent_t e0, e1;
     (void)hipEventCreate(&e0); (void)hipEventCreate(&e1);
     hipLaunchKernelGGL(k_lfac, dim3(1 + W), dim3(TR_THREADS), 0, s->stream, a);
diff --git a/calipso.jl_amd/csrc/qp.hip b/calipso.jl_amd/csrc/qp.hip
--- a/calipso.jl_amd/csrc/qp.hip
+++ b/calipso.jl_amd/csrc/qp.hip
@@ -6,18 +6,7 @@
 __global__ __launch_bounds__(1024) void k_qp_objective(Batch bt, int nx, const double* __restrict__ x, const double* __restrict__ Lx,
                                                         const double* __restrict__ q, double* __restrict__ dscal) {
     __shared__ double sm[16];
-    inst_shift(bt, x, Lx, q, dscal);
-    double a = 0.0, b = 0.0;
-    for (int i0 = threadIdx.x; i0 < nx; i0 += 4 * 1024) {
-        double xv[4], lv[4], qv[4];
-#pragma unroll
-        for (int u = 0; u < 4; ++u) { const int i = i0 + u * 1024; const bool in = i < nx; xv[u] = in ? x[i] : 0.0; lv[u] = in ? Lx[i] : 0.0; qv[u] = in ? q[i] : 0.0; }
-#pragma unroll
-        for (int u = 0; u < 4; ++u) if (i0 + u * 1024 < nx) { a += xv[u] * lv[u]; b += qv[u] * xv[u]; }
-    }
-    const double ra = block_sum(a, sm);
-    const double rb = block_sum(b, sm);
-    if (threadIdx.x == 0) dscal[0] = 0.5 * ra + rb;
+    qp_objective_body(bt, nx, x, Lx, q, dscal, sm);
 }
 
 __global__ void k_vec_add(Batch bt, int n, const double* __restrict__ a, const double* __restrict__ b, double sign, double* __restrict__ out) {
@@ -34,6 +23,9 @@
     double* Lx = s->vtmp + 3 * (size_t)d.N;
     const Batch bt = batch_of(s).b;
     const unsigned nz = bt.n;
+    if ((flags & ~(uint32_t)(CALIPSO_EVAL_EQUALITY | CALIPSO_EVAL_CONE)) == CALIPSO_EVAL_OBJECTIVE && (!d.ne || (flags & CALIPSO_EVAL_EQUALITY)) && (!d.nc || (flags & CALIPSO_EVAL_CONE)) &&
+        gemv_qp_candidate(s, x, Lx, s->qp.q, s->qp.bh, s->gh))
+        return;
     if (flags & (CALIPSO_EVAL_OBJECTIVE | CALIPSO_EVAL_OBJECTIVE_GRADIENT)) {
         if (!(flags & CALIPSO_EVAL_OBJECTIVE)) gemv_t(s, d.nx, d.nx, s->Lxx, d.nx, x, s->fx, 1.0, 0.0, SP_LXX, s->qp.q);
         else {
diff --git a/calipso.jl_amd/csrc/schur.hip b/calipso.jl_amd/csrc/schur.hip
--- a/calipso.jl_amd/csrc/schur.hip
+++ b/calipso.jl_amd/csrc/schur.hip
@@ -6,93 +6,101 @@
 
 namespace calipso {
 
-__global__ __launch_bounds__(1024) void k_cone_weights(BatchSc bt, Dims d, ConeDev cd, const double* __restrict__ w,
-                                                        double* __restrict__ kzz, double* __restrict__ wz, double* __restrict__ Bsoc,
-                                                        double* __restrict__ Wsoc, double* __restrict__ work, int* __restrict__ icount) {
-    __shared__ int smi[3][16];
-    inst_shift(bt.b, w, kzz, wz, Bsoc, Wsoc, work);
+__device__ __forceinline__ double nonneg_kzz(const double* __restrict__ sl, const double* __restrict__ t, const Scalars& sc, double Hss, int i) {
+    const double Sb = sl[i] - sc.ed, Ti = t[i];
+    return -1.0 * Sb / (Ti + Sb * Hss) + (0.0 - sc.ed);
+}
+__device__ __forceinline__ void small_cone_blocks(int st, int dim, const double* __restrict__ sl, const double* __restrict__ t, const Scalars& sc, double Hss, double (&Bm)[16],
+                                                  double (&Wm)[16], int& pos, int& nonpos, int& zero) {
+    constexpr int MD = 4;
+    double ls[MD], lt[MD], u[MD], c[MD], o[MD], M[MD * MD];
+#pragma unroll
+    for (int a = 0; a < MD; ++a) { ls[a] = a < dim ? sl[st + a] : 0.0; lt[a] = a < dim ? t[st + a] : 0.0; u[a] = 0.0; c[a] = 0.0; o[a] = 0.0; }
+#pragma unroll
+    for (int e = 0; e < MD * MD; ++e) { Bm[e] = 0.0; M[e] = 0.0; Wm[e] = 0.0; }
+    const double sb1 = ls[0] - sc.ed;
+    u[0] = lt[0] + sb1 * Hss;
+#pragma unroll
+    for (int k = 1; k < MD; ++k) if (k < dim) u[k] = lt[k] + ls[k] * Hss;
+#pragma unroll
+    for (int col = 0; col < MD; ++col) if (col < dim) {
+#pragma unroll
+        for (int a = 0; a < MD; ++a) if (a < dim) c[a] = (a == col) ? sb1 : (col == 0 ? ls[a] : (a == 0 ? ls[col] : 0.0));
+        arrow_inverse_small<MD>(dim, u, c, o);
+#pragma unroll
+        for (int a = 0; a < MD; ++a) if (a < dim) Bm[a + col * MD] = 0.0 - o[a];
+    }
+#pragma unroll
+    for (int a = 0; a < MD; ++a) if (a < dim) Bm[a + a * MD] += (0.0 - sc.ed);
+#pragma unroll
+    for (int b = 0; b < MD; ++b)
+#pragma unroll
+        for (int a = 0; a < MD; ++a) if (a < dim && b < dim) M[a + b * MD] = (a <= b) ? Bm[a + b * MD] : Bm[b + a * MD];
+#pragma unroll
+    for (int jj = 0; jj < MD; ++jj) if (jj < dim) {
+        const double dj = M[jj + jj * MD];
+        pos += dj > 0.0; nonpos += dj <= 0.0; zero += dj == 0.0;
+#pragma unroll
+        for (int i = jj + 1; i < MD; ++i) if (i < dim) {
+            const double yij = M[i + jj * MD];
+            const double l = yij / dj;
+#pragma unroll
+            for (int k = jj + 1; k < MD; ++k) if (k <= i) M[i + k * MD] -= l * (k == i ? yij : M[jj + k * MD]);
+            M[i + jj * MD] = l;
+            M[jj + i * MD] = yij;
+        }
+    }
+#pragma unroll
+    for (int col = 0; col < MD; ++col) if (col < dim) {
+#pragma unroll
+        for (int a = 0; a < MD; ++a) o[a] = (a == col) ? 1.0 : 0.0;
+#pragma unroll
+        for (int a = 0; a < MD; ++a) if (a < dim) {
+            double x = o[a];
+#pragma unroll
+            for (int k = 0; k < MD; ++k) if (k < a) x -= M[a + k * MD] * o[k];
+            o[a] = x;
+        }
+#pragma unroll
+        for (int a = 0; a < MD; ++a) if (a < dim) o[a] /= M[a + a * MD];
+#pragma unroll
+        for (int a = MD - 1; a >= 0; --a) if (a < dim) {
+            double x = o[a];
+#pragma unroll
+            for (int k = 0; k < MD; ++k) if (k > a && k < dim) x -= M[k + a * MD] * o[k];
+            o[a] = x;
+        }
+#pragma unroll
+        for (int a = 0; a < MD; ++a) if (a < dim) Wm[a + col * MD] = -o[a];
+    }
+}
+__device__ __forceinline__ void cone_weights_body(const BatchSc& bt, const Dims& d, const ConeDev& cd, const double* __restrict__ w, double* __restrict__ kzz, double* __restrict__ wz,
+                                                  double* __restrict__ Bsoc, double* __restrict__ Wsoc, int* __restrict__ icount, int (*smi)[16]) {
+    inst_shift(bt.b, w, kzz, wz, Bsoc, Wsoc);
     inst_shift_i(bt.b, icount);
     const Scalars sc = bt.scal(blockIdx.z);
-    const int tid = threadIdx.x;
+    const int tid = threadIdx.x, nthr = blockDim.x;
     const double* sl = w + d.os();
     const double* t = w + d.ot();
     const double Hss = 0.0 + sc.ep;
     int pos = 0, nonpos = 0, zero = 0;
-    for (int i = tid; i < d.q; i += 1024) {
-        const double Sb = sl[i] - sc.ed, Ti = t[i];
-        const double k = -1.0 * Sb / (Ti + Sb * Hss) + (0.0 - sc.ed);
+    for (int i = tid; i < d.q; i += nthr) {
+        const double k = nonneg_kzz(sl, t, sc, Hss, i);
         kzz[i] = k;
         wz[i] = -1.0 / k;
         pos += k > 0.0; nonpos += k <= 0.0; zero += k == 0.0;
     }
-    for (int j = tid; j < d.n_soc; j += 1024) {
+    for (int j = tid; j < d.n_soc; j += nthr) {
         const int st = cd.soc_start[j], dim = cd.soc_dim[j], off = cd.soc_woff[j];
         double* B = Bsoc + off;
         double* W = Wsoc + off;
         if (dim > 4) continue;
-        {
-            constexpr int MD = 4;
-            double ls[MD], lt[MD], u[MD], c[MD], o[MD], Bm[MD * MD], M[MD * MD];
-#pragma unroll
-            for (int a = 0; a < MD; ++a) { ls[a] = a < dim ? sl[st + a] : 0.0; lt[a] = a < dim ? t[st + a] : 0.0; u[a] = 0.0; c[a] = 0.0; o[a] = 0.0; }
-#pragma unroll
-            for (int e = 0; e < MD * MD; ++e) { Bm[e] = 0.0; M[e] = 0.0; }
-            const double sb1 = ls[0] - sc.ed;
-            u[0] = lt[0] + sb1 * Hss;
-#pragma unroll
-            for (int k = 1; k < MD; ++k) if (k < dim) u[k] = lt[k] + ls[k] * Hss;
-#pragma unroll
-            for (int col = 0; col < MD; ++col) if (col < dim) {
-#pragma unroll
-                for (int a = 0; a < MD; ++a) if (a < dim) c[a] = (a == col) ? sb1 : (col == 0 ? ls[a] : (a == 0 ? ls[col] : 0.0));
-                arrow_inverse_small<MD>(dim, u, c, o);
-#pragma unroll
-                for (int a = 0; a < MD; ++a) if (a < dim) Bm[a + col * MD] = 0.0 - o[a];
-            }
-#pragma unroll
-            for (int a = 0; a < MD; ++a) if (a < dim) Bm[a + a * MD] += (0.0 - sc.ed);
-#pragma unroll
-            for (int b = 0; b < MD; ++b)
-#pragma unroll
-                for (int a = 0; a < MD; ++a) if (a < dim && b < dim) { B[a + b * dim] = Bm[a + b * MD]; M[a + b * MD] = (a <= b) ? Bm[a + b * MD] : Bm[b + a * MD]; }
-#pragma unroll
-            for (int jj = 0; jj < MD; ++jj) if (jj < dim) {
-                const double dj = M[jj + jj * MD];
-                pos += dj > 0.0; nonpos += dj <= 0.0; zero += dj == 0.0;
-#pragma unroll
-                for (int i = jj + 1; i < MD; ++i) if (i < dim) {
-                    const double yij = M[i + jj * MD];
-                    const double l = yij / dj;
-#pragma unroll
-                    for (int k = jj + 1; k < MD; ++k) if (k <= i) M[i + k * MD] -= l * (k == i ? yij : M[jj + k * MD]);
-                    M[i + jj * MD] = l;
-                    M[jj + i * MD] = yij;
-                }
-            }
-#pragma unroll
-            for (int col = 0; col < MD; ++col) if (col < dim) {
-#pragma unroll
-                for (int a = 0; a < MD; ++a) o[a] = (a == col) ? 1.0 : 0.0;
-#pragma unroll
-                for (int a = 0; a < MD; ++a) if (a < dim) {
-                    double x = o[a];
-#pragma unroll
-                    for (int k = 0; k < MD; ++k) if (k < a) x -= M[a + k * MD] * o[k];
-                    o[a] = x;
-                }
-#pragma unroll
-                for (int a = 0; a < MD; ++a) if (a < dim) o[a] /= M[a + a * MD];
-#pragma unroll
-                for (int a = MD - 1; a >= 0; --a) if (a < dim) {
-                    double x = o[a];
-#pragma unroll
-                    for (int k = 0; k < MD; ++k) if (k > a && k < dim) x -= M[k + a * MD] * o[k];
-                    o[a] = x;
-                }
-#pragma unroll
-                for (int a = 0; a < MD; ++a) if (a < dim) W[a + col * dim] = -o[a];
-            }
-        }
+        double Bm[16], Wm[16];
+        small_cone_blocks(st, dim, sl, t, sc, Hss, Bm, Wm, pos, nonpos, zero);
+#pragma unroll
+        for (int b = 0; b < 4; ++b)
+#pragma unroll
+            for (int a = 0; a < 4; ++a) if (a < dim && b < dim) { B[a + b * dim] = Bm[a + b * 4]; W[a + b * dim] = Wm[a + b * 4]; }
     }
     if (tid == 0 && d.ne > 0) {
         const double ky = -1.0 / (sc.rho + sc.ep) + (0.0 - sc.ed);
@@ -105,13 +113,26 @@
     __syncthreads();
     if (tid < 3) {
         int a = 0;
-        for (int k = 0; k < 16; ++k) a += smi[tid][k];
+        for (int k = 0; k < (nthr >> 6); ++k) a += smi[tid][k];
         icount[tid] = a;
         icount[3 + tid] = 0;
     }
 }
-
-void launch_cone_weights(calipso_hip_solver* s) {
+__global__ __launch_bounds__(1024) void k_cone_weights(BatchSc bt, Dims d, ConeDev cd, const double* __restrict__ w,
+                                                        double* __restrict__ kzz, double* __restrict__ wz, double* __restrict__ Bsoc,
+                                                        double* __restrict__ Wsoc, double* __restrict__ work, int* __restrict__ icount) {
+    __shared__ int smi[3][16];
+    (void)work;
+    cone_weights_body(bt, d, cd, w, kzz, wz, Bsoc, Wsoc, icount, smi);
+}
+
+void launch_cone_weights(calipso_hip_solver* s, bool scale_rows_follows) {
+    s->weights_pending = false;
+    if (scale_rows_follows && (step_fusions() & FUSE_CONE_WEIGHTS) && !s->cur && !s->compact && !s->blocks.on && s->band64 == 0 && !(s->stage_parallel && s->spS) && s->d.nc > 0 &&
+        s->d.n_wide == 0) {
+        s->weights_pending = true;
+        return;
+    }
     const BatchSc B = batch_of(s);
     hipLaunchKernelGGL(k_cone_weights, dim3(1, 1, B.b.n), dim3(1024), 0, s->stream, B, s->d, s->cone, s->solution, s->kzz, s->wz, s->Bsoc,
                        s->Wsoc, s->socwork, s->icount);
@@ -119,14 +140,15 @@
 }
 
 constexpr int SCALE_COLS = 16;
-__global__ void k_scale_rows(Batch bt, Dims d, ConeDev cd, const double* __restrict__ hx, const double* __restrict__ wz,
-                             const double* __restrict__ Wsoc, double* __restrict__ WH, const int* __restrict__ zrow, double* __restrict__ Spad) {
+template <bool FUSED>
+__device__ __forceinline__ void scale_rows_body(Batch bt, const Scalars& sc, Dims d, ConeDev cd, const double* __restrict__ hx, const double* __restrict__ wz, const double* __restrict__ Wsoc,
+                                                double* __restrict__ WH, const int* __restrict__ zrow, double* __restrict__ Spad, const double* __restrict__ pt, int by, int ny) {
     inst_shift(bt, hx, wz, Wsoc, WH);
     if (zrow) inst_shift_i(bt, zrow);
     if (Spad) {
         inst_shift(bt, Spad);
-        const long long total = (long long)gridDim.x * gridDim.y * blockDim.x, count = (long long)(d.NP - d.nx) * d.NP;
-        for (long long e = ((long long)blockIdx.y * gridDim.x + blockIdx.x) * blockDim.x + threadIdx.x; e < count; e += total) {
+        const long long total = (long long)gridDim.x * ny * blockDim.x, count = (long long)(d.NP - d.nx) * d.NP;
+        for (long long e = ((long long)by * gridDim.x + blockIdx.x) * blockDim.x + threadIdx.x; e < count; e += total) {
             const int i = d.nx + (int)(e / d.NP), j = (int)(e % d.NP);
             if (j <= i) Spad[i + (size_t)j * d.NP] = (i == j) ? 1.0 : 0.0;
         }
@@ -136,14 +158,38 @@
     int st = 0, dim = 0;
     const double* W = nullptr;
     double w0 = 0.0;
-    if (c < d.q) w0 = wz[c];
-    else { const int j = cd.entry_soc[c]; st = cd.soc_start[j]; dim = cd.soc_dim[j]; W = Wsoc + cd.soc_woff[j]; }
-    int col0 = blockIdx.y * SCALE_COLS, col1 = min(d.nx, col0 + SCALE_COLS);
+    double wr[4] = {0.0, 0.0, 0.0, 0.0};
+    if (FUSED) {
+        inst_shift(bt, pt);
+        const double* sl = pt + d.os();
+        const double* t = pt + d.ot();
+        const double Hss = 0.0 + sc.ep;
+        if (c < d.q) w0 = -1.0 / nonneg_kzz(sl, t, sc, Hss, c);
+        else {
+            const int j = cd.entry_soc[c];
+            st = cd.soc_start[j]; dim = cd.soc_dim[j];
+            double Bm[16], Wm[16];
+            int pos = 0, nonpos = 0, zero = 0;
+            small_cone_blocks(st, dim, sl, t, sc, Hss, Bm, Wm, pos, nonpos, zero);
+#pragma unroll
+            for (int b = 0; b < 4; ++b)
+#pragma unroll
+                for (int a = 0; a < 4; ++a) if (a == c - st) wr[b] = Wm[a + b * 4];
+        }
+    } else if (c < d.q) w0 = wz[c];
+    else {
+        const int j = cd.entry_soc[c]; st = cd.soc_start[j]; dim = cd.soc_dim[j]; W = Wsoc + cd.soc_woff[j];
+        if (dim <= 4) {
+#pragma unroll
+            for (int b = 0; b < 4; ++b) wr[b] = b < dim ? W[(c - st) + b * dim] : 0.0;
+        }
+    }
+    int col0 = by * SCALE_COLS, col1 = min(d.nx, col0 + SCALE_COLS);
     if (zrow) {
         const int k = d.ne + c;
         col0 = max(col0, zrow[2 * k]); col1 = min(col1, zrow[2 * k + 1]);
     }
-    const int cbase = blockIdx.y * SCALE_COLS;
+    const int cbase = by * SCALE_COLS;
     if (c < d.q) {
         double hv[SCALE_COLS];
 #pragma unroll
@@ -153,9 +199,6 @@
         return;
     }
     if (dim <= 4) {
-        double wr[4];
-#pragma unroll
-        for (int b = 0; b < 4; ++b) wr[b] = b < dim ? W[(c - st) + b * dim] : 0.0;
         for (int k0 = 0; k0 < SCALE_COLS; k0 += 8) {
             double hv[8][4];
 #pragma unroll
@@ -184,6 +227,20 @@
         for (int b = 0; b < dim; ++b) v += W[(c - st) + b * dim] * h[st + b];
         WH[c + (size_t)col * d.nc] = v;
     }
+}
+__global__ void k_scale_rows(Batch bt, Dims d, ConeDev cd, const double* __restrict__ hx, const double* __restrict__ wz,
+                             const double* __restrict__ Wsoc, double* __restrict__ WH, const int* __restrict__ zrow, double* __restrict__ Spad) {
+    scale_rows_body<false>(bt, Scalars(), d, cd, hx, wz, Wsoc, WH, zrow, Spad, nullptr, blockIdx.y, gridDim.y);
+}
+__global__ __launch_bounds__(256) void k_cone_weights_scale_rows(BatchSc bt, Dims d, ConeDev cd, const double* __restrict__ pt, double* __restrict__ kzz, double* __restrict__ wz,
+                                                                  double* __restrict__ Bsoc, double* __restrict__ Wsoc, int* __restrict__ icount, const double* __restrict__ hx,
+                                                                  double* __restrict__ WH, double* __restrict__ Spad) {
+    __shared__ int smi[3][16];
+    if (blockIdx.y == 0) {
+        if (blockIdx.x == 0) cone_weights_body(bt, d, cd, pt, kzz, wz, Bsoc, Wsoc, icount, smi);
+        return;
+    }
+    scale_rows_body<true>(bt.b, bt.scal(blockIdx.z), d, cd, hx, nullptr, nullptr, WH, nullptr, Spad, pt, (int)blockIdx.y - 1, (int)gridDim.y - 1);
 }
 
 void launch_scale_rows(calipso_hip_solver* s) {
@@ -193,6 +250,13 @@
     const BatchSc B = batch_of(s);
     const bool pad = s->d.NP > s->d.nx && !(s->stage_parallel && s->spS);
     s->pad_done = pad;
+    if (s->weights_pending) {
+        s->weights_pending = false;
+        hipLaunchKernelGGL(k_cone_weights_scale_rows, dim3((s->d.nc + 255) / 256, 1 + (s->d.nx + SCALE_COLS - 1) / SCALE_COLS, 1), dim3(256), 0, s->stream, B, s->d, s->cone, s->solution, s->kzz,
+                           s->wz, s->Bsoc, s->Wsoc, s->icount, s->hx, s->WH, pad ? s->S : (double*)nullptr);
+        s->fusion_count[2] += 1;
+        return;
+    }
     hipLaunchKernelGGL(k_scale_rows, dim3((s->d.nc + 255) / 256, (s->d.nx + SCALE_COLS - 1) / SCALE_COLS, B.b.n), dim3(256), 0, s->stream, B.b, s->d, s->cone, s->hx, s->wz, s->Wsoc, s->WH, s->band64 > 0 ? s->zrow : nullptr,
                        pad ? s->S : (double*)nullptr);
 }
diff --git a/calipso.jl_amd/csrc/solvek.hip b/calipso.jl_amd/csrc/solvek.hip
--- a/calipso.jl_amd/csrc/solvek.hip
+++ b/calipso.jl_amd/csrc/solvek.hip
@@ -19,10 +19,10 @@
     hipLaunchKernelGGL(k_negate_copy, dim3((n + 255) / 256), dim3(256), 0, s->stream, src, dst, n);
 }
 
-void linear_solve_device(calipso_hip_solver* s, bool with_t2, bool rhs_ready) {
+void linear_solve_device(calipso_hip_solver* s, bool with_t2, bool rhs_ready, int fwd_done) {
     const Dims& d = s->d;
     if (d.m && !rhs_ready) gemv_t(s, d.m, d.nx, s->Z, d.m, s->t1, s->xbuf, 1.0, 1.0, SP_Z);
-    launch_trsv(s, s->xbuf);
+    launch_trsv(s, s->xbuf, rhs_ready ? fwd_done : 0);
     if (d.m && with_t2) gemv_n(s, d.m, d.nx, s->Z, d.m, s->xbuf, s->t2, 1.0, 0.0, SP_Z);
 }
 
diff --git a/include/calipso_hip.h b/include/calipso_hip.h
--- a/include/calipso_hip.h
+++ b/include/calipso_hip.h
@@ -269,7 +269,7 @@
 int32_t calipso_hip_phase_times(calipso_hip_solver*, double out[9]);
 int32_t calipso_hip_kernel_times(calipso_hip_solver*, double out[8]);
 int32_t calipso_hip_structure_work(calipso_hip_solver*, double out[8]);
-int32_t calipso_hip_schedule_info(calipso_hip_solver*, double out[4]);
+int32_t calipso_hip_schedule_info(calipso_hip_solver*, double out[9]);
 int32_t calipso_hip_synchronize(calipso_hip_solver*);
 int32_t calipso_hip_streams_concurrent(calipso_hip_solver* a, calipso_hip_solver* b, double out[6]);
 int32_t calipso_hip_rebind_stream(calipso_hip_solver*, int32_t priority_class);
```

Measured after the change: 563.8 Newton steps/s, median of 4. About the same (+1.5%).
